# tangjiapeng/DiffuScene

Measured on AMD Instinct MI355X. Metric: denoiser steps/sec (train + 1000-step sample) at B=256, N=80 objects, higher is better.
Workload: dtype f32 (operands split 3xbf16, 6 products, f32 accumulate); 1 GPU; uncond living/dining rooms (config/uncond/diffusion_livingrooms_instancond_lat32_v.yaml scaled to N=80), B=256 scenes per GPU, N=80, C=65, T=1000, mode=both; global_batch=256, parallelism=single

## Files before the change

__graft_entry__.py:

```python
import os
import subprocess
import sys

ROOT = os.path.dirname(os.path.abspath(__file__))
CSRC = os.path.join(ROOT, "diffuscene_amd", "csrc")
LIB = os.path.join(ROOT, "diffuscene_amd", "libdiffuscene_hip.so")

SOURCES = [
    ("gemm_mfma.hip", []),
    ("gemm_split.hip", ["-fno-slp-vectorize"]),
    ("gemm_tn_split.hip", ["-fno-slp-vectorize"]),
    ("blocks.hip", []),
    ("diffusion.hip", ["-ffp-contract=off"]),
    ("train.hip", []),
    ("retrieval.hip", ["-ffp-contract=off"]),
    ("dataset.hip", ["-ffp-contract=off"]),
    ("chamfer.hip", ["-ffp-contract=off"]),
    ("optim.hip", ["-ffp-contract=off"]),
    ("foldingnet.hip", []),
]


def _hipcc():
    for c in (os.environ.get("HIPCC"), "/opt/rocm/bin/hipcc", "hipcc"):
        if c and (os.path.isabs(c) and os.path.exists(c) or not os.path.isabs(c)):
            return c
    raise RuntimeError("hipcc not found")


def _stale(target, deps):
    if not os.path.exists(target):
        return True
    t = os.path.getmtime(target)
    return any(os.path.getmtime(d) > t for d in deps)


def _stamp_git_head():
    try:
        head = subprocess.check_output(["git", "rev-parse", "--short", "HEAD"], cwd=ROOT, stderr=subprocess.DEVNULL, text=True).strip()
        dirty = subprocess.check_output(["git", "status", "--porcelain", "-uno"], cwd=ROOT, stderr=subprocess.DEVNULL, text=True).strip()
        with open(os.path.join(ROOT, "GIT_HEAD"), "w") as f:
            f.write(head + ("+" if dirty else "") + "\n")
    except Exception:
        pass


def build(force=False):
    hipcc = _hipcc()
    headers = [os.path.join(CSRC, "dsc_common.h"), os.path.join(CSRC, "gemm_core.h"), os.path.join(CSRC, "gemm_tn_split.h"),
               os.path.join(ROOT, "include", "diffuscene_hip.h")]
    objs = []
    for src, extra in SOURCES:
        s = os.path.join(CSRC, src)
        if not os.path.exists(s):
            continue
        o = os.path.join(CSRC, src.replace(".hip", ".o"))
        if force or _stale(o, [s] + headers):
            cmd = [hipcc, "--offload-arch=gfx950", "-O3", "-std=c++17", "-fPIC", "-c", s, "-o", o] + extra
            subprocess.check_call(cmd)
        objs.append(o)
    if force or _stale(LIB, objs):
        subprocess.check_call([hipcc, "--offload-arch=gfx950", "-shared", "-fPIC", "-o", LIB] + objs)
    gsrc = os.path.join(ROOT, "tools", "guard_alloc.cpp")
    gso = os.path.join(ROOT, "tools", "_build", "libdsc_guard_alloc.so")
    if os.path.exists(gsrc) and (force or _stale(gso, [gsrc])):
        os.makedirs(os.path.dirname(gso), exist_ok=True)
        try:
            subprocess.check_call([hipcc, "-O2", "-std=c++17", "-fPIC", "-shared", gsrc, "-o", gso])
        except (subprocess.CalledProcessError, OSError) as e:
            print("warning: guard allocator (tools/guard_alloc.cpp) not built: %s -- tests/test_gpu_guard.py will skip its allocator runs" % e,
                  file=sys.stderr)
    _stamp_git_head()
    if ROOT not in sys.path:
        sys.path.insert(0, ROOT)
    import diffuscene_amd
    from diffuscene_amd import _lib
    _lib.load()
    import oracle.ref_torch


def build_asan():
    hipcc = _hipcc()
    out = os.path.join(ROOT, "diffuscene_amd", "libdiffuscene_hip_asan.so")
    objs = []
    for src, extra in SOURCES:
        s = os.path.join(CSRC, src)
        o = os.path.join(CSRC, src.replace(".hip", ".asan.o"))
        subprocess.check_call([hipcc, "--offload-arch=gfx950", "-O1", "-g", "-std=c++17", "-fPIC", "-fsanitize=address", "-fno-gpu-sanitize",
                               "-shared-libsan", "-Wno-option-ignored", "-c", s, "-o", o] + extra)
        objs.append(o)
    subprocess.check_call([hipcc, "--offload-arch=gfx950", "-shared", "-fPIC", "-fsanitize=address", "-fno-gpu-sanitize", "-shared-libsan",
                           "-Wno-option-ignored", "-o", out] + objs)
    return out


def smoke():
    if ROOT not in sys.path:
        sys.path.insert(0, ROOT)
    import torch
    assert torch.cuda.is_available(), "smoke() needs a GPU"
    from diffuscene_amd.networks.denoise_net import Unet1D
    from diffuscene_amd.networks.diffusion_ddpm import DiffusionPoint
    from oracle import ref_torch as R
    from oracle import weights as W

    kw = dict(W.UNCOND_BEDROOM)
    B, N = 4, 12
    dev = torch.device("cuda:0")
    net = Unet1D(**kw)
    sd = W.synth_state_dict(kw)
    net.load_state_dict(sd)
    net.to(dev)
    cfg = dict(objectness_dim=0, class_dim=22, angle_dim=2, objfeat_dim=32)
    diff = DiffusionPoint(net, cfg, time_num=1000, model_mean_type="v")
    x = W.synth_scene_batch(B, N, 22, 32, 0)
    t = torch.tensor([3, 250, 600, 999], dtype=torch.int64)
    cond = W.synth_condition(B, N, 128, 0).contiguous()
    noise = W.synth_noise((B, N, 62), 7)
    with torch.no_grad():
        out = net(x.to(dev), t.to(dev), cond.to(dev), None).cpu()
        ref = R.unet1d_forward(sd, kw, x, t, cond, None)
        rel = float((out - ref).abs().max() / ref.abs().max())
        assert rel < 1e-4, "Unet1D forward mismatch vs oracle: %g" % rel
        tb = R.schedule_tables(1e-4, 0.02, 1000, "v")
        step = diff.diffusion.p_sample(diff._denoise, x.to(dev), t.to(dev), cond.to(dev), None,
                                       noise_fn=lambda size, dtype, device: noise.to(device), clip_denoised=True).cpu()
        ref_step = R.p_sample_step(tb, x, t, ref, noise, True, "v")
        rel2 = float((step - ref_step).abs().max() / ref_step.abs().max())
        assert rel2 < 1e-4, "p_sample mismatch vs oracle: %g" % rel2
    print("smoke ok: forward rel err %.3g, p_sample rel err %.3g" % (rel, rel2))


if __name__ == "__main__":
# ... 7 lines not shown
```

diffuscene_amd/_lib.py:

```python
import ctypes as C
import os

_HERE = os.path.dirname(os.path.abspath(__file__))
LIB_PATH = os.path.join(_HERE, "libdiffuscene_hip.so")
if os.environ.get("DSC_HIP_LIB"):
    LIB_PATH = os.path.abspath(os.environ["DSC_HIP_LIB"])

ACT_NONE, ACT_GELU, ACT_SILU, ACT_LEAKY01 = 0, 1, 2, 3
SS_NONE, SS_PER_TOKEN, SS_PER_SCENE, SS_PER_SLOT, SS_BY_INDEX = 0, 1, 2, 3, 4
MEAN_EPS, MEAN_X0, MEAN_V = 0, 1, 2
TILE_GN_80_W8, TILE_GN_80_W4, TILE_160x256, TILE_160x128_W4 = 1, 2, 5, 8
TILE_WAVE_GN, TILE_WAVE_DENSE, TILE_WAVE_GN_64 = 10, 11, 12
F32_TILE_160x256, F32_TILE_160x128, F32_TILE_128x128, F32_TILE_96x128, F32_TILE_64x64 = 0, 1, 2, 3, 4
DSC_PLANES_NONE = -100
GEMM_ROW_INVARIANT = 1
WS_MAX = 64
MAX_TOKENS_PER_SCENE = 160
STATS_MAX_OBJECTS, STATS_ONE_WAVE_MAX = 160, 32

_ERR = {-1: "DSC_EINVAL (bad shape / null pointer)", -2: "DSC_EALIGN (16-byte alignment required)",
        -3: "DSC_ERANGE (size outside kernel limits)"}

c_f32p = C.c_void_p
c_i64p = C.c_void_p


class GemmArgs(C.Structure):
    _fields_ = [
        ("a1", C.c_void_p), ("lda1", C.c_int64), ("k1", C.c_int32),
        ("a2", C.c_void_p), ("lda2", C.c_int64), ("k2", C.c_int32),
        ("w", C.c_void_p), ("ldw", C.c_int64),
        ("bias", C.c_void_p),
        ("residual", C.c_void_p), ("ldr", C.c_int64),
        ("y", C.c_void_p), ("ldy", C.c_int64),
        ("m", C.c_int32), ("n", C.c_int32),
        ("act_in", C.c_int32), ("act_out", C.c_int32),
        ("batch", C.c_int32),
        ("sa1", C.c_int64), ("sa2", C.c_int64), ("sw", C.c_int64), ("sbias", C.c_int64),
        ("sres", C.c_int64), ("sy", C.c_int64),
        ("gamma", C.c_void_p), ("beta", C.c_void_p), ("eps", C.c_float),
        ("tokens_per_scene", C.c_int32),
        ("scale_shift", C.c_void_p), ("ld_ss", C.c_int64), ("ss_mode", C.c_int32),
        ("preact", C.c_void_p), ("ld_preact", C.c_int64),
        ("ss_index", C.c_void_p),
        ("w_planes", C.c_void_p),
        ("actgrad_x", C.c_void_p), ("ld_actgrad", C.c_int64),
        ("ss_rows", C.c_int32),
        ("w_planes_layout", C.c_int32),
        ("gnb_z", C.c_void_p), ("ld_gnb_z", C.c_int64),
        ("gnb_dgamma", C.c_void_p), ("gnb_dbeta", C.c_void_p), ("gnb_dbias", C.c_void_p), ("gnb_pstride", C.c_int64),
        ("gnb_dss", C.c_void_p), ("ld_gnb_dss", C.c_int64),
        ("flags", C.c_int32),
    ]


class SplitItem(C.Structure):
    _fields_ = [("w", C.c_void_p), ("ldw", C.c_int64), ("rows", C.c_int32), ("cols", C.c_int32), ("planes", C.c_void_p),
                ("transpose", C.c_int32)]


class SmallKItem(C.Structure):
    _fields_ = [("x", C.c_void_p), ("ldx", C.c_int64), ("k_in", C.c_int32), ("w", C.c_void_p), ("ldw", C.c_int64), ("bias", C.c_void_p),
                ("y", C.c_void_p), ("ldy", C.c_int64)]


class ColSpan(C.Structure):
    _fields_ = [("src_col", C.c_int32), ("dst_col", C.c_int32), ("width", C.c_int32)]


SMALLK_MAX = 4


class WsItem(C.Structure):
    _fields_ = [("w", C.c_void_p), ("out", C.c_void_p), ("rows", C.c_int32), ("cols", C.c_int32)]


class TnGroup(C.Structure):
    _fields_ = [("a1", C.c_void_p), ("lda1", C.c_int64), ("k1", C.c_int32),
                ("a2", C.c_void_p), ("lda2", C.c_int64), ("k2", C.c_int32),
                ("dy", C.c_void_p), ("ldd", C.c_int64),
                ("out", C.c_void_p), ("ldo", C.c_int64),
                ("dbias", C.c_void_p),
                ("m", C.c_int32), ("n", C.c_int32), ("kvalid", C.c_int32),
                ("tile0", C.c_int32),
                ("ws_offset", C.c_int64),
                ("tile0s", C.c_int32)]


class ColsumItem(C.Structure):
    _fields_ = [("x", C.c_void_p), ("ldx", C.c_int64), ("m", C.c_int32), ("n", C.c_int32), ("out", C.c_void_p)]


class WsBwdItem(C.Structure):
    _fields_ = [("w", C.c_void_p), ("dw_std", C.c_void_p), ("dw", C.c_void_p), ("rows", C.c_int32), ("cols", C.c_int32)]


SIGNATURES = {
    "dsc_version": (C.c_int, []),
    "dsc_gemm_f32": (C.c_int, [C.POINTER(GemmArgs), C.c_void_p]),
    "dsc_gemm_gn_silu_f32": (C.c_int, [C.POINTER(GemmArgs), C.c_void_p]),
    "dsc_split_bf16x3_f32": (C.c_int, [C.POINTER(SplitItem), C.c_int32, C.c_void_p]),
    "dsc_gemm_arithmetic": (C.c_int, [C.POINTER(GemmArgs), C.c_int32]),
    "dsc_gemm_split_tile": (C.c_int, [C.POINTER(GemmArgs), C.c_int32]),
    "dsc_gemm_f32_tile": (C.c_int, [C.POINTER(GemmArgs)]),
    "dsc_gemm_planes_layout": (C.c_int, [C.POINTER(GemmArgs), C.c_int32]),
    "dsc_get_split_wave": (C.c_int, []),
    "dsc_set_split_wave": (C.c_int, [C.c_int32]),
    "dsc_gemm_skinny": (C.c_int, [C.POINTER(GemmArgs), C.c_int32]),
    "dsc_get_skinny": (C.c_int, []),
    "dsc_set_skinny": (C.c_int, [C.c_int32]),
    "dsc_get_gemm_arithmetic": (C.c_int, []),
    "dsc_set_gemm_arithmetic": (C.c_int, [C.c_int32]),
    "dsc_gemm_layernorm_f32": (C.c_int, [C.POINTER(GemmArgs), C.c_void_p]),
    "dsc_gemm_splitk_f32": (C.c_int, [C.POINTER(GemmArgs), C.c_int32, c_f32p, C.c_int64, C.c_void_p]),
    "dsc_linear_smallk_f32": (C.c_int, [c_f32p, C.c_int64, C.c_int32, c_f32p, C.c_int64, c_f32p, c_f32p, C.c_int64,
                                        C.c_int32, C.c_int32, C.c_int32, C.c_void_p]),
    "dsc_linear_smallk_grouped_f32": (C.c_int, [C.POINTER(SmallKItem), C.c_int32, C.c_int32, C.c_int32, C.c_int32, C.c_void_p]),
    "dsc_gather_columns_f32": (C.c_int, [c_f32p, C.c_int64, c_f32p, C.c_int64, C.c_int32, C.POINTER(ColSpan), C.c_int32, C.c_void_p]),
    "dsc_weight_standardize_f32": (C.c_int, [C.POINTER(WsItem), C.c_int32, C.c_float, C.c_void_p]),
    "dsc_layernorm_f32": (C.c_int, [c_f32p, C.c_int64, c_f32p, c_f32p, C.c_int64, c_f32p, C.c_int64, C.c_int32,
                                    C.c_int32, C.c_float, C.c_void_p]),
    "dsc_linear_attention_f32": (C.c_int, [c_f32p, C.c_int64, c_f32p, C.c_int64, c_f32p, C.c_int64, c_f32p, C.c_int64,
                                           C.c_int32, C.c_int32, C.c_int32, C.c_float, C.c_void_p]),
    "dsc_attention_f32": (C.c_int, [c_f32p, C.c_int64, c_f32p, C.c_int64, c_f32p, C.c_int64, c_f32p, C.c_int64,
                                    C.c_int32, C.c_int32, C.c_float, C.c_void_p]),
    "dsc_time_embedding_f32": (C.c_int, [c_i64p, C.c_int32, C.c_int32, c_f32p, C.c_int32, c_f32p, c_f32p, C.c_void_p]),
    "dsc_activation_f32": (C.c_int, [c_f32p, c_f32p, C.c_int64, C.c_int32, C.c_void_p]),
    "dsc_q_sample_f32": (C.c_int, [c_f32p, c_f32p, c_i64p, c_f32p, c_f32p, c_f32p, c_f32p, C.c_int32, C.c_int64, C.c_int32,
                                   C.c_void_p]),
    "dsc_p_sample_f32": (C.c_int, [c_f32p, c_f32p, c_f32p, c_i64p, c_f32p, c_f32p, c_f32p, c_f32p, c_f32p, c_f32p,
                                   c_f32p, C.c_int32, C.c_int32, C.c_int32, C.c_int64, C.c_int32, C.c_void_p]),
    "dsc_device_error_count": (C.c_int64, [C.c_int32]),
    "dsc_add_scalar_i64": (C.c_int, [c_i64p, C.c_int32, C.c_int64, C.c_void_p]),
    "dsc_ddim_step_f32": (C.c_int, [c_f32p, c_f32p, c_f32p, c_i64p, c_i64p, c_i64p, c_f32p, c_f32p, c_f32p, c_f32p, c_f32p,
                                    c_f32p, c_f32p, c_f32p, c_f32p, C.c_int32, C.c_int32, C.c_int64, C.c_int32, C.c_int32,
                                    C.c_void_p]),
    "dsc_ddim_advance_i64": (C.c_int, [c_i64p, c_i64p, c_i64p, C.c_int32, C.c_int32, C.c_void_p]),
    "dsc_knn16_f32": (C.c_int, [c_f32p, C.c_int64, C.c_int32, c_f32p, c_f32p, C.c_int32, C.c_int32, C.c_void_p, C.c_void_p]),
    "dsc_rowsq_f32": (C.c_int, [c_f32p, C.c_int64, C.c_int32, C.c_int64, c_f32p, C.c_void_p]),
    "dsc_knn_cov_f32": (C.c_int, [c_f32p, C.c_int64, C.c_void_p, C.c_int32, C.c_int32, c_f32p, C.c_int64, C.c_void_p]),
    "dsc_gather_max_f32": (C.c_int, [c_f32p, C.c_int64, C.c_void_p, C.c_int32, C.c_int32, C.c_int32, c_f32p, C.c_int64,
                                     C.c_void_p, C.c_void_p]),
    "dsc_gather_max_bwd_f32": (C.c_int, [c_f32p, C.c_int64, C.c_void_p, C.c_void_p, C.c_int32, C.c_int32, C.c_int32, c_f32p,
                                         C.c_int64, C.c_void_p]),
    "dsc_bn_workspace_floats": (C.c_int64, [C.c_int64, C.c_int32]),
    "dsc_batchnorm_fwd_f32": (C.c_int, [c_f32p, C.c_int64, c_f32p, c_f32p, C.c_int64, C.c_int32, C.c_float, C.c_float,
                                        C.c_int32, c_f32p, c_f32p, c_f32p, c_f32p, c_f32p, c_f32p, c_f32p, C.c_int64,
                                        C.c_void_p]),
    "dsc_batchnorm_eval_f32": (C.c_int, [c_f32p, C.c_int64, c_f32p, c_f32p, c_f32p, c_f32p, C.c_int64, C.c_int32, C.c_int32,
                                         c_f32p, C.c_void_p]),
    "dsc_batchnorm_bwd_f32": (C.c_int, [c_f32p, c_f32p, c_f32p, c_f32p, c_f32p, C.c_int64, C.c_int32, C.c_int32, c_f32p,
                                        c_f32p, c_f32p, c_f32p, C.c_int64, C.c_void_p]),
    "dsc_rowmax_f32": (C.c_int, [c_f32p, C.c_int64, C.c_int32, C.c_int32, C.c_int32, c_f32p, C.c_void_p, C.c_void_p]),
    "dsc_rowmax_bwd_f32": (C.c_int, [c_f32p, C.c_void_p, C.c_int32, C.c_int32, C.c_int32, c_f32p, C.c_void_p]),
    "dsc_point_affine_f32": (C.c_int, [c_f32p, C.c_int64, C.c_int32, c_f32p, C.c_int64, c_f32p, C.c_int32, C.c_int32,
                                       C.c_int32, C.c_int32, c_f32p, C.c_void_p]),
    "dsc_point_affine_bwd_f32": (C.c_int, [c_f32p, c_f32p, C.c_int64, C.c_int32, c_f32p, C.c_int64, C.c_int32, C.c_int32,
                                           C.c_int32, C.c_int32, c_f32p, C.c_int64, c_f32p, C.c_int64, c_f32p, c_f32p,
                                           C.c_int64, C.c_void_p]),
    "dsc_postfilter_compact_f32": (C.c_int, [c_f32p, C.c_int32, C.c_int32, C.c_int32, C.c_int32, C.c_int32, C.c_int32, c_f32p,
                                             C.c_void_p, C.c_void_p]),
    "dsc_gemm_tn_f32": (C.c_int, [c_f32p, C.c_int64, C.c_int32, c_f32p, C.c_int64, C.c_int32, c_f32p, C.c_int64, c_f32p,
                                  C.c_int64, c_f32p, C.c_int32, C.c_int32, C.c_int32, c_f32p, C.c_int64, C.c_void_p]),
    "dsc_gemm_tn_workspace_floats": (C.c_int64, [C.c_int32, C.c_int32, C.c_int32]),
    "dsc_gemm_tn_grouped_f32": (C.c_int, [C.c_void_p, C.c_int32, C.c_int32, C.c_int32, c_f32p, C.c_int64, C.c_int64,
                                          C.c_void_p]),
    "dsc_gemm_tn_grouped_split_f32": (C.c_int, [C.c_void_p, C.c_int32, C.c_int32, C.c_void_p, C.c_int32, C.c_int32, c_f32p, C.c_int64,
                                                C.c_int64, C.c_int32, C.c_void_p]),
    "dsc_set_tn_split_form": (C.c_int, [C.c_int32]),
    "dsc_get_tn_split_form": (C.c_int, []),
    "dsc_colsum_f32": (C.c_int, [c_f32p, C.c_int64, C.c_int32, C.c_int32, c_f32p, c_f32p, C.c_int64, C.c_void_p]),
    "dsc_colsum_grouped_f32": (C.c_int, [C.c_void_p, C.c_int32, C.c_int32, C.c_void_p]),
    "dsc_gn_silu_bwd_f32": (C.c_int, [c_f32p, C.c_int64, c_f32p, C.c_int64, c_f32p, c_f32p, c_f32p, C.c_int64, C.c_int32,
                                      c_f32p, C.c_int64, c_f32p, c_f32p, c_f32p, C.c_int64, c_f32p, C.c_int64, C.c_int32,
                                      C.c_int32, C.c_int32, C.c_float, C.c_void_p]),
    "dsc_weight_standardize_bwd_f32": (C.c_int, [C.POINTER(WsBwdItem), C.c_int32, C.c_float, C.c_void_p]),
    "dsc_layernorm_bwd_f32": (C.c_int, [c_f32p, C.c_int64, c_f32p, c_f32p, C.c_int64, c_f32p, C.c_int64, c_f32p, C.c_int64, c_f32p,
                                        C.c_int32, C.c_int32, C.c_int32, C.c_float, C.c_void_p]),
    "dsc_linear_attention_bwd_f32": (C.c_int, [c_f32p, C.c_int64] * 7 + [C.c_int32, C.c_int32, C.c_int32, C.c_float,
                                                                          C.c_void_p]),
    "dsc_attention_bwd_f32": (C.c_int, [c_f32p, C.c_int64] * 7 + [C.c_int32, C.c_int32, C.c_float, C.c_void_p]),
    "dsc_retrieve_nearest_f32": (C.c_int, [c_f32p, C.c_void_p, C.c_void_p, c_f32p, C.c_void_p, C.c_void_p, C.c_int32,
                                           C.c_int32, C.c_int32, C.c_void_p, c_f32p, C.c_void_p]),
    "dsc_box_bounds_f32": (C.c_int, [c_f32p, c_f32p, c_f32p, C.c_void_p, C.c_int32, C.c_int32, c_f32p, C.c_void_p]),
    "dsc_scene_stats_f32": (C.c_int, [c_f32p, c_f32p, C.c_void_p, C.c_void_p, C.c_int32, C.c_int32, C.c_int32, C.c_int32,
                                      C.c_void_p, C.c_void_p, C.c_void_p, C.c_void_p, C.c_void_p, C.c_void_p, c_f32p, C.c_void_p]),
    "dsc_encode_scene_batch_f32": (C.c_int, [c_i64p, c_f32p, c_f32p, c_f32p, c_f32p, c_f32p, C.c_int32, C.c_int32, c_i64p,
                                             C.c_void_p, C.c_void_p, C.c_void_p, C.c_int32, C.POINTER(C.c_double), c_f32p,
                                             C.c_int64, c_i64p, C.c_int32, C.c_int32, C.c_void_p]),
    "dsc_chamfer3d_forward_f32": (C.c_int, [c_f32p, c_f32p, c_f32p, c_f32p, C.c_void_p, C.c_void_p, C.c_int32, C.c_int32,
                                            C.c_int32, C.c_void_p]),
    "dsc_chamfer3d_backward_f32": (C.c_int, [c_f32p, c_f32p, c_f32p, c_f32p, C.c_void_p, C.c_void_p, c_f32p, c_f32p,
                                             C.c_int32, C.c_int32, C.c_int32, C.c_void_p]),
    "dsc_grad_sumsq_f32": (C.c_int, [C.c_void_p, C.c_int32, C.c_void_p, C.c_void_p]),
    "dsc_clip_coef_f32": (C.c_int, [C.c_void_p, C.c_int32, C.c_float, c_f32p, c_f32p, C.c_void_p]),
    "dsc_adam_step_f32": (C.c_int, [C.c_void_p, C.c_int32, C.c_float, C.c_float, C.c_float, C.c_float, C.c_float, C.c_float,
                                    c_f32p, C.c_void_p]),
    "dsc_ddpm_loss_f32": (C.c_int, [c_f32p, c_f32p, c_f32p, c_i64p, c_f32p, c_f32p, c_f32p, c_f32p, C.POINTER(C.c_float),
                                    c_f32p, c_f32p, c_f32p] + [C.c_int32] * 12 + [C.c_float, C.c_int32, C.c_void_p]),
    "dsc_copy2d_f32": (C.c_int, [c_f32p, C.c_int64, c_f32p, C.c_int64, C.c_int32, C.c_int32, C.c_void_p]),
    "dsc_add2d_f32": (C.c_int, [c_f32p, C.c_int64, c_f32p, C.c_int64, C.c_int32, C.c_int32, C.c_void_p]),
    "dsc_activation_bwd_f32": (C.c_int, [c_f32p, c_f32p, c_f32p, C.c_int64, C.c_int32, C.c_void_p]),
    "dsc_transpose_batched_f32": (C.c_int, [C.POINTER(WsItem), C.c_int32, C.c_void_p]),
    "dsc_transpose_f32": (C.c_int, [c_f32p, C.c_int64, c_f32p, C.c_int64, C.c_int32, C.c_int32, C.c_void_p]),
    "dsc_complete_overwrite_f32": (C.c_int, [c_f32p, c_f32p, c_f32p, c_i64p, c_f32p, c_f32p, C.c_int32, C.c_int32,
                                             C.c_int32, C.c_int32, C.c_int32, C.c_void_p]),
    "dsc_complete_overwrite_ragged_f32": (C.c_int, [c_f32p, c_f32p, c_f32p, c_i64p, c_i64p, c_f32p, c_f32p, C.c_int32, C.c_int32,
                                                    C.c_int32, C.c_int32, C.c_int32, C.c_void_p]),
    "dsc_p_sample_inpaint_f32": (C.c_int, [c_f32p, c_f32p, c_f32p, c_f32p, c_f32p, c_i64p, c_i64p, c_f32p, c_f32p, c_f32p, c_f32p,
                                           c_f32p, c_f32p, c_f32p, c_f32p] + [C.c_int32] * 7 + [C.c_void_p]),
    "dsc_ddim_inpaint_step_f32": (C.c_int, [c_f32p] * 5 + [c_i64p] * 4 + [c_f32p] * 10 + [C.c_int32] * 7 + [C.c_void_p]),
    "dsc_masked_overwrite_f32": (C.c_int, [c_f32p, c_f32p, c_f32p, C.c_void_p, c_i64p, c_f32p, c_f32p, C.c_int32, C.c_int64, C.c_int32,
                                           C.c_void_p]),
    "dsc_p_sample_masked_f32": (C.c_int, [c_f32p] * 5 + [C.c_void_p, c_i64p] + [c_f32p] * 8 + [C.c_int32] * 3 + [C.c_int64, C.c_int32,
                                                                                                                  C.c_void_p]),
    "dsc_ddim_masked_step_f32": (C.c_int, [c_f32p] * 5 + [C.c_void_p] + [c_i64p] * 3 + [c_f32p] * 10 + [C.c_int32] * 2 +
                                 [C.c_int64, C.c_int32, C.c_int32, C.c_void_p]),
    "dsc_cfg_combine_f32": (C.c_int, [c_f32p, c_f32p, c_f32p, C.c_int32, C.c_int64, C.c_void_p]),
    "dsc_scene_randn_f32": (C.c_int, [c_f32p, c_i64p, c_i64p, C.c_int64, C.c_int64, C.c_int64, C.c_void_p]),
    "dsc_scene_philox_u32": (C.c_int, [C.c_void_p, c_i64p, c_i64p, C.c_int64, C.c_int64, C.c_int64, C.c_void_p]),
    "dsc_p_sample_cfg_f32": (C.c_int, [c_f32p] * 4 + [c_i64p] + [c_f32p] * 8 + [C.c_int32] * 3 + [C.c_int64, C.c_int32, C.c_void_p]),
    "dsc_ddim_cfg_step_f32": (C.c_int, [c_f32p] * 4 + [c_i64p] * 3 + [c_f32p] * 10 + [C.c_int32] * 2 +
                              [C.c_int64, C.c_int32, C.c_int32, C.c_void_p]),
    "dsc_p_sample_masked_cfg_f32": (C.c_int, [c_f32p] * 6 + [C.c_void_p, c_i64p] + [c_f32p] * 9 + [C.c_int32] * 3 +
                                    [C.c_int64, C.c_int32, C.c_void_p]),
    "dsc_ddim_masked_cfg_step_f32": (C.c_int, [c_f32p] * 6 + [C.c_void_p] + [c_i64p] * 3 + [c_f32p] * 11 + [C.c_int32] * 2 +
                                     [C.c_int64, C.c_int32, C.c_int32, C.c_void_p]),
    "dsc_scene_gate_f32": (C.c_int, [c_f32p, C.c_void_p, c_f32p, C.c_int32, C.c_int64, C.c_void_p]),
}

_lib = None


class HipLibraryMissing(RuntimeError):
    pass


def load():
    global _lib
    if _lib is not None:
        return _lib
    if not os.path.exists(LIB_PATH):
        raise HipLibraryMissing(
            "%s not found: build it with `python __graft_entry__.py` (hipcc --offload-arch=gfx950). "
            "diffuscene_amd has no CPU or PyTorch fallback." % LIB_PATH)
    import torch
    lib = C.CDLL(LIB_PATH)
    for name, (res, args) in SIGNATURES.items():
        try:
            fn = getattr(lib, name)
        except AttributeError as e:
            raise HipLibraryMissing("symbol %s missing from %s" % (name, LIB_PATH)) from e
        fn.restype = res
        fn.argtypes = args
    if lib.dsc_get_gemm_arithmetic() < 0:
        raise ValueError("DSC_GEMM=%r: must be 'split' (default) or 'f32'" % os.environ.get("DSC_GEMM"))
    if lib.dsc_get_tn_split_form() < 0:
        raise ValueError("DSC_TN_FORM=%r: must be '2' (default), '1' or '0'" % os.environ.get("DSC_TN_FORM"))
    if lib.dsc_get_split_wave() < 0:
        raise ValueError("DSC_WAVE=%r: must be '1' / 'auto' (default) or '0'" % os.environ.get("DSC_WAVE"))
    _lib = lib
    return lib


def split_enabled():
    return load().dsc_get_gemm_arithmetic() == 1


def gemm_mode():
    lib = load()
    if lib.dsc_get_gemm_arithmetic() != 1:
        return 0
    return (2 if lib.dsc_get_split_wave() == 1 else 1) + 10 * lib.dsc_get_tn_split_form()


def set_split_wave(on):
    prev = load().dsc_get_split_wave() == 1
    check(load().dsc_set_split_wave(1 if on else 0), "dsc_set_split_wave")
    return prev


def set_gemm_arithmetic(name):
    if name not in ("split", "f32"):
        raise ValueError("gemm arithmetic must be 'split' or 'f32', got %r" % (name,))
    prev = "split" if split_enabled() else "f32"
    check(load().dsc_set_gemm_arithmetic(1 if name == "split" else 0), "dsc_set_gemm_arithmetic")
    return prev


def device_error_count(reset=False):
    n = load().dsc_device_error_count(1 if reset else 0)
    if n < 0:
        raise RuntimeError("dsc_device_error_count failed (HIP error)")
    return int(n)


def check_indices(where):
    if os.environ.get("DSC_CHECK_INDICES", "0") == "1":
        n = device_error_count(reset=True)
        if n:
            raise IndexError("%s: %d out-of-range device timestep(s) were clamped into the schedule tables" % (where, n))


def check(rc, what):
    if rc != 0:
        raise RuntimeError("%s failed: %s" % (what, _ERR.get(rc, "hipError_t %d" % rc)))


def fn(name):
    return getattr(load(), name)
```

diffuscene_amd/csrc/blocks.hip:

```cpp
#include "dsc_common.h"

namespace {

struct WsBatch { dsc_ws_item it[DSC_WS_MAX]; };

__device__ __forceinline__ float block_sum_256(float v, float* red) {
    v = wave_sum(v);
    const int lane = threadIdx.x & 63, wave = threadIdx.x >> 6;
    __syncthreads();
    if (lane == 0) red[wave] = v;
    __syncthreads();
    return red[0] + red[1] + red[2] + red[3];
}

__global__ __launch_bounds__(256) void ws_kernel(const WsBatch b, const float eps) {
    __shared__ float red[4];
    const dsc_ws_item it = b.it[blockIdx.y];
    const int row = blockIdx.x;
    if (row >= it.rows) return;
    const float* w = it.w + (int64_t)row * it.cols;
    float* o = it.out + (int64_t)row * it.cols;
    constexpr int MAXE = 8;
    float v[MAXE];
    float s = 0.f;
#pragma unroll
    for (int i = 0; i < MAXE; ++i) {
        const int c = threadIdx.x + 256 * i;
        v[i] = (c < it.cols) ? w[c] : 0.f;
        s += v[i];
    }
    const float mean = block_sum_256(s, red) / (float)it.cols;
    float s2 = 0.f;
#pragma unroll
    for (int i = 0; i < MAXE; ++i) {
        const int c = threadIdx.x + 256 * i;
        const float d = (c < it.cols) ? v[i] - mean : 0.f;
        s2 += d * d;
    }
    const float var = block_sum_256(s2, red) / (float)it.cols;
    const float rs = 1.0f / sqrtf(var + eps);
#pragma unroll
    for (int i = 0; i < MAXE; ++i) {
        const int c = threadIdx.x + 256 * i;
        if (c < it.cols) o[c] = (v[i] - mean) * rs;
    }
}

__global__ __launch_bounds__(256) void layernorm512_kernel(const float* __restrict__ x, int64_t ldx,
                                                          const float* __restrict__ g,
                                                          const float* __restrict__ res, int64_t ldr,
                                                          float* __restrict__ y, int64_t ldy, int m, float eps) {
    const int lane = threadIdx.x & 63;
    const int row = blockIdx.x * 4 + (threadIdx.x >> 6);
    if (row >= m) return;
    const float* xr = x + (int64_t)row * ldx;
    const f32x4 a = *reinterpret_cast<const f32x4*>(xr + lane * 4);
    const f32x4 b = *reinterpret_cast<const f32x4*>(xr + 256 + lane * 4);
    float s = (a[0] + a[1]) + (a[2] + a[3]) + (b[0] + b[1]) + (b[2] + b[3]);
    const float mean = wave_sum(s) * (1.0f / 512.0f);
    float s2 = 0.f;
#pragma unroll
    for (int e = 0; e < 4; ++e) {
        const float da = a[e] - mean, db = b[e] - mean;
        s2 += da * da + db * db;
    }
    const float var = wave_sum(s2) * (1.0f / 512.0f);
    const float rs = 1.0f / sqrtf(var + eps);
    const f32x4 ga = *reinterpret_cast<const f32x4*>(g + lane * 4);
    const f32x4 gb = *reinterpret_cast<const f32x4*>(g + 256 + lane * 4);
    f32x4 oa, ob;
#pragma unroll
    for (int e = 0; e < 4; ++e) {
        oa[e] = (a[e] - mean) * rs * ga[e];
        ob[e] = (b[e] - mean) * rs * gb[e];
    }
    if (res) {
        const float* rr = res + (int64_t)row * ldr;
        const f32x4 ra = *reinterpret_cast<const f32x4*>(rr + lane * 4);
        const f32x4 rb = *reinterpret_cast<const f32x4*>(rr + 256 + lane * 4);
#pragma unroll
        for (int e = 0; e < 4; ++e) { oa[e] += ra[e]; ob[e] += rb[e]; }
    }
    float* yr = y + (int64_t)row * ldy;
    *reinterpret_cast<f32x4*>(yr + lane * 4) = oa;
    *reinterpret_cast<f32x4*>(yr + 256 + lane * 4) = ob;
}

constexpr int MAXTOK = 160;
constexpr int HP = 33;
constexpr int LP = 36;

__global__ __launch_bounds__(256) void linear_attention_kernel(const float* __restrict__ q, int64_t ldq,
                                                               const float* __restrict__ k, int64_t ldk,
                                                               const float* __restrict__ v, int64_t ldv,
                                                               float* __restrict__ out, int64_t ldo,
                                                               int nq, int nk, float scale) {
    extern __shared__ __attribute__((aligned(16))) float lds[];
    float* Ks = lds;
    float* Vs = Ks + nk * LP;
    float* Qs = Vs + nk * LP;
    float* ctx = Qs + nq * LP;
    const int b = blockIdx.x >> 2, h = blockIdx.x & 3;
    const int tid = threadIdx.x;
    const float* kb = k + (int64_t)b * nk * ldk + h * 32;
    const float* vb = v + (int64_t)b * nk * ldv + h * 32;
    const float* qb = q + (int64_t)b * nq * ldq + h * 32;
    for (int f = tid; f < nk * 8; f += 256) {
        const int j = f >> 3, c4 = (f & 7) * 4;
        *reinterpret_cast<f32x4*>(Ks + j * LP + c4) = *reinterpret_cast<const f32x4*>(kb + (int64_t)j * ldk + c4);
        *reinterpret_cast<f32x4*>(Vs + j * LP + c4) = *reinterpret_cast<const f32x4*>(vb + (int64_t)j * ldv + c4);
    }
    for (int f = tid; f < nq * 8; f += 256) {
        const int i = f >> 3, c4 = (f & 7) * 4;
        *reinterpret_cast<f32x4*>(Qs + i * LP + c4) = *reinterpret_cast<const f32x4*>(qb + (int64_t)i * ldq + c4);
    }
    __syncthreads();
    {
        const int d = tid >> 3, part = tid & 7;
        float mx = -INFINITY;
        for (int j = part; j < nk; j += 8) mx = fmaxf(mx, Ks[j * LP + d]);
        mx = fmaxf(mx, __shfl_xor(mx, 1, 64));
        mx = fmaxf(mx, __shfl_xor(mx, 2, 64));
        mx = fmaxf(mx, __shfl_xor(mx, 4, 64));
        float sm = 0.f;
        for (int j = part; j < nk; j += 8) {
            const float e = expf(Ks[j * LP + d] - mx);
            Ks[j * LP + d] = e;
            sm += e;
        }
        sm += __shfl_xor(sm, 1, 64);
        sm += __shfl_xor(sm, 2, 64);
        sm += __shfl_xor(sm, 4, 64);
        const float inv = 1.0f / sm;
        for (int j = part; j < nk; j += 8) Ks[j * LP + d] *= inv;
    }
    __syncthreads();
    {
        const int d = tid >> 3, e0 = (tid & 7) * 4;
        f32x4 a = {0.f, 0.f, 0.f, 0.f};
        for (int j = 0; j < nk; ++j) {
            const float kd = Ks[j * LP + d];
            const f32x4 vv = *reinterpret_cast<const f32x4*>(Vs + j * LP + e0);
#pragma unroll
            for (int e = 0; e < 4; ++e) a[e] += kd * vv[e];
        }
        *reinterpret_cast<f32x4*>(ctx + d * LP + e0) = a;
    }
    __syncthreads();
    for (int i0 = 0; i0 < nq; i0 += 64) {
        const int i = i0 + (tid >> 2), part = tid & 3;
        const bool ok = i < nq;
        float qv[8];
        float mx = -INFINITY;
        if (ok) {
            const f32x4 a = *reinterpret_cast<const f32x4*>(Qs + i * LP + part * 8);
            const f32x4 c = *reinterpret_cast<const f32x4*>(Qs + i * LP + part * 8 + 4);
#pragma unroll
            for (int e = 0; e < 4; ++e) { qv[e] = a[e]; qv[4 + e] = c[e]; }
#pragma unroll
            for (int e = 0; e < 8; ++e) mx = fmaxf(mx, qv[e]);
        }
        mx = fmaxf(mx, __shfl_xor(mx, 1, 64));
        mx = fmaxf(mx, __shfl_xor(mx, 2, 64));
        float sm = 0.f;
        if (ok) {
#pragma unroll
            for (int e = 0; e < 8; ++e) { qv[e] = expf(qv[e] - mx); sm += qv[e]; }
        }
        sm += __shfl_xor(sm, 1, 64);
        sm += __shfl_xor(sm, 2, 64);
        if (ok) {
            const float inv = scale / sm;
            f32x4 a, c;
#pragma unroll
            for (int e = 0; e < 4; ++e) { a[e] = qv[e] * inv; c[e] = qv[4 + e] * inv; }
            *reinterpret_cast<f32x4*>(Qs + i * LP + part * 8) = a;
            *reinterpret_cast<f32x4*>(Qs + i * LP + part * 8 + 4) = c;
        }
        __builtin_amdgcn_wave_barrier();
        if (ok) {
            f32x4 o0 = {0.f, 0.f, 0.f, 0.f}, o1 = {0.f, 0.f, 0.f, 0.f};
#pragma unroll 8
            for (int d = 0; d < 32; ++d) {
                const float qd = Qs[i * LP + d];
                const f32x4 c0 = *reinterpret_cast<const f32x4*>(ctx + d * LP + part * 8);
                const f32x4 c1 = *reinterpret_cast<const f32x4*>(ctx + d * LP + part * 8 + 4);
#pragma unroll
                for (int e = 0; e < 4; ++e) { o0[e] += c0[e] * qd; o1[e] += c1[e] * qd; }
            }
            float* orow = out + ((int64_t)b * nq + i) * ldo + h * 32 + part * 8;
            *reinterpret_cast<f32x4*>(orow) = o0;
            *reinterpret_cast<f32x4*>(orow + 4) = o1;
        }
    }
}

__global__ __launch_bounds__(512) void attention_kernel(const float* __restrict__ q, int64_t ldq,
                                                        const float* __restrict__ k, int64_t ldk,
                                                        const float* __restrict__ v, int64_t ldv,
                                                        float* __restrict__ out, int64_t ldo, int n, float scale) {
    extern __shared__ __attribute__((aligned(16))) float att_lds[];
    float* Ks = att_lds;
    float* Vs = Ks + n * LP;
    const int b = blockIdx.x >> 2, h = blockIdx.x & 3;
    const int tid = threadIdx.x;
    const float* kb = k + (int64_t)b * n * ldk + h * 32;
    const float* vb = v + (int64_t)b * n * ldv + h * 32;
    const int nthr = blockDim.x, rows = nthr >> 2;
    for (int f = tid; f < n * 8; f += nthr) {
        const int j = f >> 3, c4 = (f & 7) * 4;
        *reinterpret_cast<f32x4*>(Ks + j * LP + c4) = *reinterpret_cast<const f32x4*>(kb + (int64_t)j * ldk + c4);
        *reinterpret_cast<f32x4*>(Vs + j * LP + c4) = *reinterpret_cast<const f32x4*>(vb + (int64_t)j * ldv + c4);
    }
    __syncthreads();
    const int part = tid & 3;
    for (int i0 = 0; i0 < n; i0 += rows) {
        const int i = i0 + (tid >> 2);
        const bool ok = i < n;
        const float* qr = q + ((int64_t)b * n + (ok ? i : 0)) * ldq + h * 32 + part * 8;
        const f32x4 qa = *reinterpret_cast<const f32x4*>(qr), qc = *reinterpret_cast<const f32x4*>(qr + 4);
        float qv[8];
#pragma unroll
        for (int e = 0; e < 4; ++e) { qv[e] = qa[e] * scale; qv[4 + e] = qc[e] * scale; }
        auto score = [&](int j) {
            const f32x4 ka = *reinterpret_cast<const f32x4*>(Ks + j * LP + part * 8);
            const f32x4 kc = *reinterpret_cast<const f32x4*>(Ks + j * LP + part * 8 + 4);
            float s = 0.f;
#pragma unroll
            for (int e = 0; e < 4; ++e) s += qv[e] * ka[e];
#pragma unroll
            for (int e = 0; e < 4; ++e) s += qv[4 + e] * kc[e];
            s += __shfl_xor(s, 1, 64);
            s += __shfl_xor(s, 2, 64);
            return s;
        };
        float mx = -INFINITY;
        for (int j = 0; j < n; ++j) mx = fmaxf(mx, score(j));
        float o[8] = {0.f, 0.f, 0.f, 0.f, 0.f, 0.f, 0.f, 0.f};
        float sm = 0.f;
        for (int j = 0; j < n; ++j) {
            const float pj = expf(score(j) - mx);
            sm += pj;
            const f32x4 va = *reinterpret_cast<const f32x4*>(Vs + j * LP + part * 8);
            const f32x4 vc = *reinterpret_cast<const f32x4*>(Vs + j * LP + part * 8 + 4);
#pragma unroll
            for (int e = 0; e < 4; ++e) { o[e] += pj * va[e]; o[4 + e] += pj * vc[e]; }
        }
        if (ok) {
            const float inv = 1.0f / sm;
            float* orow = out + ((int64_t)b * n + i) * ldo + h * 32 + part * 8;
            f32x4 t0, t1;
#pragma unroll
            for (int e = 0; e < 4; ++e) { t0[e] = o[e] * inv; t1[e] = o[4 + e] * inv; }
            *reinterpret_cast<f32x4*>(orow) = t0;
            *reinterpret_cast<f32x4*>(orow + 4) = t1;
        }
    }
}

constexpr int SK_TOK = 32;
constexpr int SK_MAXK = 64;

__device__ __forceinline__ void linear_smallk_block(const float* __restrict__ x, int64_t ldx, int kin,
                                                    const float* __restrict__ w, int64_t ldw,
                                                    const float* __restrict__ bias,
                                                    float* __restrict__ y, int64_t ldy, int m, int n, int act, float* xs) {
    const int tok0 = blockIdx.x * SK_TOK;
    const int ntok = (m - tok0) < SK_TOK ? (m - tok0) : SK_TOK;
    for (int f = threadIdx.x; f < SK_TOK * kin; f += 256) {
        const int t = f / kin, kk = f - t * kin;
        xs[kk * SK_TOK + t] = (t < ntok) ? x[(int64_t)(tok0 + t) * ldx + kk] : 0.f;
    }
    __syncthreads();
    for (int c = threadIdx.x; c < n; c += 256) {
        float acc[SK_TOK];
        const float b = bias ? bias[c] : 0.f;
// ... 219 lines not shown
```

diffuscene_amd/csrc/gemm_split.hip:

```cpp
#include "dsc_common.h"
#include "gemm_split_wave.h"
#include <atomic>
#include <cstring>

#ifndef DSC_SPLIT_DSPREAD
#define DSC_SPLIT_DSPREAD true
#endif

namespace dsc_split {

typedef unsigned u32x4 __attribute__((ext_vector_type(4)));
typedef __bf16 bf16x8 __attribute__((ext_vector_type(8)));
typedef __bf16 bf16x2 __attribute__((ext_vector_type(2)));

constexpr int BK = 32;

__device__ __forceinline__ unsigned cvt_pk_bf16(float a, float b) {
    f32x2 v = {a, b};
    return __builtin_bit_cast(unsigned, __builtin_convertvector(v, bf16x2));
}
__device__ __forceinline__ float bf_lo(unsigned p) { return __builtin_bit_cast(float, p << 16); }
__device__ __forceinline__ float bf_hi(unsigned p) { return __builtin_bit_cast(float, p & 0xffff0000u); }

__device__ __forceinline__ void split8(const f32x4 lo, const f32x4 hi, bf16x8& p1, bf16x8& p2, bf16x8& p3) {
// ... 316 lines not shown
            }
        }
        if (p.preact) {
            float* const pb = p.preact + (int64_t)(row0 + srow + l15) * p.ld_preact + cbase;
#pragma unroll
            for (int i = 0; i < RB; ++i)
                if (valid[i]) {
#pragma unroll
                    for (int j = 0; j < 4; ++j) *reinterpret_cast<f32x4*>(pb + (int64_t)i * 16 * p.ld_preact + j * 16) = acc[i][j];
                }
        }
        const float inv_cnt = 1.f / (float)(ntok * 64);
        float s0 = 0.f;
#pragma unroll
        for (int i = 0; i < RB; ++i)
#pragma unroll
            for (int j = 0; j < 4; ++j)
                s0 += valid[i] ? (acc[i][j][0] + acc[i][j][1]) + (acc[i][j][2] + acc[i][j][3]) : 0.f;
        const float mean = wave_sum_dpp(s0) * inv_cnt;
        float q0 = 0.f;
#pragma unroll
        for (int i = 0; i < RB; ++i)
#pragma unroll
            for (int j = 0; j < 4; ++j)
#pragma unroll
                for (int e = 0; e < 4; ++e) {
                    const float d = valid[i] ? acc[i][j][e] - mean : 0.f;
                    q0 = fmaf(d, d, q0);
                }
        const float rstd = 1.f / sqrtf(wave_sum_dpp(q0) * inv_cnt + p.eps);
#pragma unroll
        for (int j = 0; j < 4; ++j)
#pragma unroll
            for (int e = 0; e < 4; ++e) {
                const float a = rstd * ga[j][e], sp1 = sc[j][e] + 1.f;
                ga[j][e] = a * sp1;
                be[j][e] = fmaf(be[j][e] - mean * a, sp1, sh[j][e]);
            }
#pragma unroll
        for (int i = 0; i < RB; ++i) {
            if (valid[i]) {
#pragma unroll
                for (int j = 0; j < 4; ++j) {
                    f32x4 y, s1 = {1.f, 1.f, 1.f, 1.f}, s2 = {0.f, 0.f, 0.f, 0.f};
                    if (per_row) {
                        const int64_t row = p.ss_mode == DSC_SS_PER_TOKEN ? (int64_t)row0 + srow + i * 16 + l15 : (int64_t)i * 16 + l15;
                        const float* ssr = p.scale_shift + row * p.ld_ss + cbase + j * 16;
                        s1 = *reinterpret_cast<const f32x4*>(ssr) + 1.f;
                        s2 = *reinterpret_cast<const f32x4*>(ssr + p.n);
                    }
#pragma unroll
                    for (int e = 0; e < 4; ++e) {
                        float t = fmaf(acc[i][j][e], ga[j][e], be[j][e]);
                        if (per_row) t = fmaf(t, s1[e], s2[e]);
                        y[e] = dsc_silu_fast(t);
                    }
                    if (rbp) y += *reinterpret_cast<const f32x4*>(rbp + (int64_t)i * 16 * p.ldr + j * 16);
                    *reinterpret_cast<f32x4*>(ob + (int64_t)i * 16 * p.ldy + j * 16) = y;
                }
            }
        }
    }
}

template <bool GN, int WM, int WN, int RB, bool DSPREAD = DSC_SPLIT_DSPREAD>
__global__ __launch_bounds__(64 * WM * WN, 1) void gemm_split_kernel(const dsc_gemm_args p, const int ntok) {
    __shared__ __attribute__((aligned(16))) char smem[split_smem_bytes<WM, WN, RB>()];
    gemm_split_tile<GN, WM, WN, RB, DSPREAD>(p, ntok, blockIdx.x, blockIdx.y, smem);
}

template <bool GN, int WM, int WN, int RB>
int launch(const dsc_gemm_args* a, int ntok, hipStream_t s) {
    constexpr int BN = 64 * WN;
    const int scenes = (a->m + ntok - 1) / ntok;
    const unsigned grid = (unsigned)(((scenes + WM - 1) / WM) * (a->n / BN));
    DSC_CLEAR_STALE_ERROR();
    hipLaunchKernelGGL((gemm_split_kernel<GN, WM, WN, RB>), dim3(grid, (unsigned)a->batch), dim3(64 * WM * WN), 0, s, *a, ntok);
    DSC_LAUNCH_CHECK();
    return 0;
}

}

enum { T_GN_32 = 0, T_GN_80_W8, T_GN_80_W4, T_GN_48, T_GN_64, T_160x256, T_256x128, T_128x128, T_160x128_W4, T_64x256, T_WAVE_GN, T_WAVE_DENSE, T_WAVE_GN_64 };

static std::atomic<int> g_gemm_arith{-1000};

extern "C" int dsc_get_gemm_arithmetic(void) {
    int m = g_gemm_arith.load(std::memory_order_relaxed);
    if (m == -1000) {
        const char* e = getenv("DSC_GEMM");
        m = (!e || !e[0] || !strcmp(e, "split")) ? 1 : !strcmp(e, "f32") ? 0 : DSC_EINVAL;
        g_gemm_arith.store(m, std::memory_order_relaxed);
    }
    return m;
}

extern "C" int dsc_set_gemm_arithmetic(int32_t mode) {
    if (mode != 0 && mode != 1) return DSC_EINVAL;
    g_gemm_arith.store(mode, std::memory_order_relaxed);
    return 0;
}

static std::atomic<int> g_split_wave{-1000};

extern "C" int dsc_get_split_wave(void) {
    int m = g_split_wave.load(std::memory_order_relaxed);
    if (m == -1000) {
        const char* e = getenv("DSC_WAVE");
        m = (!e || !e[0] || !strcmp(e, "1") || !strcmp(e, "auto")) ? 1 : !strcmp(e, "0") ? 0 : DSC_EINVAL;
        g_split_wave.store(m, std::memory_order_relaxed);
    }
    return m;
}

extern "C" int dsc_set_split_wave(int32_t mode) {
    if (mode != 0 && mode != 1) return DSC_EINVAL;
    g_split_wave.store(mode, std::memory_order_relaxed);
    return 0;
}

static int select_wave(const dsc_gemm_args* a, bool gn) {
    if (dsc_get_split_wave() != 1) return -1;
    const int K = a->k1 + a->k2;
    if ((a->n % 128) || (a->k1 % 64) || (a->k2 % 64) || K < 256) return -1;
    if (a->batch != 1 && (gn || a->sw != (int64_t)a->n * K || a->ldw != K || (a->sy & 3) || (a->sres & 3) || (a->sbias & 3))) return -1;
    if (!dsc_aligned16(a->y) || (a->ldy & 3) || a->ldy < a->n) return -1;
    if (a->bias && !dsc_aligned16(a->bias)) return -1;
    if (a->residual && (!dsc_aligned16(a->residual) || (a->ldr & 3) || a->ldr < a->n)) return -1;
    if (a->preact && (!dsc_aligned16(a->preact) || (a->ld_preact & 3) || a->ld_preact < a->n || a->batch != 1)) return -1;
    if (a->actgrad_x && (gn || !dsc_aligned16(a->actgrad_x) || (a->ld_actgrad & 3) || a->ld_actgrad < a->n || a->batch != 1)) return -1;
    if (3LL * a->batch * a->n * K * 2 >= 0x7fffffffLL) return -1;
    const int64_t ld_max = a->lda1 > a->lda2 ? a->lda1 : a->lda2;
    if (ld_max * 4 * 96 >= 0x7fffffffLL) return -1;
    long waves;
    if (a->gnb_z) {
        const int N = a->tokens_per_scene;
        if (gn || a->batch != 1 || N <= 64 || N > 80 || (a->m % N) || a->bias || a->residual || a->preact || a->actgrad_x || a->act_out != DSC_ACT_NONE) return -1;
        if (!a->gamma || !a->beta || !a->gnb_dgamma || !a->gnb_dbeta || !a->gnb_dbias || (a->ss_mode != DSC_SS_NONE && a->ss_mode != DSC_SS_PER_SCENE)) return -1;
        if (!dsc_aligned16(a->gnb_z) || (a->ld_gnb_z & 3) || a->ld_gnb_z < a->n || !dsc_aligned16(a->gamma) || !dsc_aligned16(a->beta)) return -1;
        if (!dsc_aligned16(a->gnb_dgamma) || !dsc_aligned16(a->gnb_dbeta) || !dsc_aligned16(a->gnb_dbias) || (a->gnb_pstride & 3)) return -1;
        if (a->ss_mode == DSC_SS_PER_SCENE && (!a->scale_shift || !dsc_aligned16(a->scale_shift) || (a->ld_ss & 3))) return -1;
        if (a->gnb_dss && (!dsc_aligned16(a->gnb_dss) || (a->ld_gnb_dss & 3))) return -1;
        waves = (long)(a->m / N) * (a->n / 128);
        const long r = (waves + 1023) / 1024;
        return waves * 5 >= r * 1024 * 4 ? T_WAVE_DENSE : -1;
    }
    if (gn) {
        const int N = a->tokens_per_scene;
        if (N <= 16 || N > 80) return -1;
        const bool perrow = a->ss_mode == DSC_SS_PER_TOKEN || a->ss_mode == DSC_SS_PER_SLOT;
        if (perrow && a->ld_ss < 2 * (int64_t)a->n) return -1;
        waves = (long)(a->m / N) * (a->n / 128);
    } else {
        waves = (long)((a->m + 79) / 80) * (a->n / 128) * a->batch;
    }
    const long rounds = (waves + 1023) / 1024;
    if (waves * 5 >= rounds * 1024 * 4) return gn ? T_WAVE_GN : T_WAVE_DENSE;
    if (gn && a->tokens_per_scene > 64) {
        const long w4 = 2 * waves, r4 = (w4 + 1023) / 1024;
        if (r4 == 1 && w4 * 5 >= 1024 * 4) return T_WAVE_GN_64;
    }
    return -1;
}

static int select_block_tile(const dsc_gemm_args* a, bool gn);

static int select_tile(const dsc_gemm_args* a, bool gn, bool assume_planes = false) {
    if (dsc_get_gemm_arithmetic() != 1 || (!assume_planes && !a->w_planes)) return -1;
    if (a->flags & DSC_GEMM_ROW_INVARIANT) return -1;
    const int w = select_wave(a, gn);
    return w >= 0 ? w : select_block_tile(a, gn);
}

static int select_block_tile(const dsc_gemm_args* a, bool gn) {
    if (a->gnb_z) return -1;
    const int K = a->k1 + a->k2;
    if (a->batch != 1 && (gn || a->sw != (int64_t)a->n * K || a->ldw != K || (a->sy & 3) || (a->sres & 3) || (a->sbias & 3))) return -1;
    if ((a->n % 128) || (K % 32)) return -1;
    if (!dsc_aligned16(a->w_planes) || !dsc_aligned16(a->y) || (a->ldy & 3)) return -1;
    if (a->bias && !dsc_aligned16(a->bias)) return -1;
    if (a->residual && (!dsc_aligned16(a->residual) || (a->ldr & 3))) return -1;
    if (!gn && a->preact && (!dsc_aligned16(a->preact) || (a->ld_preact & 3) || a->batch != 1)) return -1;
    if (a->actgrad_x && (gn || !dsc_aligned16(a->actgrad_x) || (a->ld_actgrad & 3) || a->batch != 1)) return -1;
    if (3LL * a->batch * a->n * K * 2 >= 0x7fffffffLL) return -1;
    const int64_t ld_max = a->lda1 > a->lda2 ? a->lda1 : a->lda2;
    if (ld_max * 4 * 320 >= 0x7fffffffLL) return -1;
    const bool wide = (a->n % 256) == 0;
    constexpr long MIN_BLOCKS = 160;
    if (gn) {
        const int N = a->tokens_per_scene;
        if (N <= 16 || N > 80) return -1;
        const long S = a->m / N;
        if (N <= 32) return ((S + 3) / 4) * (a->n / 128) >= MIN_BLOCKS ? T_GN_32 : -1;
        const long b8 = wide ? ((S + 1) / 2) * (a->n / 256) : 0, b4 = ((S + 1) / 2) * (a->n / 128);
        if (N > 64) return b8 >= MIN_BLOCKS + 32 ? T_GN_80_W8 : b4 >= MIN_BLOCKS ? T_GN_80_W4 : -1;
        if (b8 < MIN_BLOCKS) return -1;
        return N <= 48 ? T_GN_48 : T_GN_64;
    }
    struct Cand { int bm, bn, id; };
    const Cand cands[5] = {{160, 256, T_160x256}, {256, 128, T_256x128}, {160, 128, T_160x128_W4}, {128, 128, T_128x128}, {64, 256, T_64x256}};
    int best = -1;
    long best_cost = 0, best_blk = 0;
    for (int i = 0; i < 5; ++i) {
        if (cands[i].bn == 256 && !wide) continue;
        const long nblk = (long)((a->m + cands[i].bm - 1) / cands[i].bm) * (a->n / cands[i].bn) * a->batch;
        const long c = ((nblk + 255) / 256) * (long)cands[i].bm * cands[i].bn;
        if (best < 0 || c < best_cost) { best = cands[i].id; best_cost = c; best_blk = nblk; }
    }
    return best_blk >= MIN_BLOCKS ? best : -1;
}

int dsc_gemm_try_split(const dsc_gemm_args* a, bool gn, hipStream_t s) {
    using namespace dsc_split;
    if (dsc_get_gemm_arithmetic() < 0 || dsc_get_split_wave() < 0) return DSC_EINVAL;
    const int N = a->tokens_per_scene;
    const int tile = select_tile(a, gn);
    if (tile < 0) return DSC_SPLIT_NOT_TAKEN;
    const int want = (tile == T_WAVE_GN || tile == T_WAVE_DENSE || tile == T_WAVE_GN_64) ? DSC_PLANES_FRAGMENT : DSC_PLANES_ROWMAJOR;
    if (a->w_planes_layout != want) return DSC_EINVAL;
    switch (tile) {
        case T_GN_32: return launch<true, 4, 2, 2>(a, N, s);
        case T_GN_80_W8: return launch<true, 2, 4, 5>(a, N, s);
        case T_GN_80_W4: return launch<true, 2, 2, 5>(a, N, s);
        case T_GN_48: return launch<true, 2, 4, 3>(a, N, s);
        case T_GN_64: return launch<true, 2, 4, 4>(a, N, s);
        case T_160x256: return launch<false, 2, 4, 5>(a, 80, s);
        case T_256x128: return launch<false, 4, 2, 4>(a, 64, s);
        case T_128x128: return launch<false, 4, 2, 2>(a, 32, s);
        case T_160x128_W4: return launch<false, 2, 2, 5>(a, 80, s);
        case T_64x256: return launch<false, 2, 4, 2>(a, 32, s);
        case T_WAVE_DENSE:
            if (a->gnb_z) return dsc_wave::launch<false, 5, false, 8, true>(a, a->w_planes, N, s);
            return dsc_wave::launch<false, 5>(a, a->w_planes, 80, s);
        case T_WAVE_GN_64:
            return (a->ss_mode == DSC_SS_PER_TOKEN || a->ss_mode == DSC_SS_PER_SLOT) ? dsc_wave::launch<true, 5, true, 4>(a, a->w_planes, N, s)
                                                                                     : dsc_wave::launch<true, 5, false, 4>(a, a->w_planes, N, s);
        case T_WAVE_GN: {
            const bool perrow = a->ss_mode == DSC_SS_PER_TOKEN || a->ss_mode == DSC_SS_PER_SLOT;
            const int rb = (N + 15) / 16;
            if (perrow) {
                return rb == 5 ? dsc_wave::launch<true, 5, true>(a, a->w_planes, N, s) : rb == 4 ? dsc_wave::launch<true, 4, true>(a, a->w_planes, N, s)
                     : rb == 3 ? dsc_wave::launch<true, 3, true>(a, a->w_planes, N, s) : dsc_wave::launch<true, 2, true>(a, a->w_planes, N, s);
            }
            return rb == 5 ? dsc_wave::launch<true, 5>(a, a->w_planes, N, s) : rb == 4 ? dsc_wave::launch<true, 4>(a, a->w_planes, N, s)
                 : rb == 3 ? dsc_wave::launch<true, 3>(a, a->w_planes, N, s) : dsc_wave::launch<true, 2>(a, a->w_planes, N, s);
        }
        default: return DSC_SPLIT_NOT_TAKEN;
    }
}

extern "C" int dsc_gemm_arithmetic(const dsc_gemm_args* a, int32_t gn) {
    if (!a || a->m <= 0 || a->n <= 0 || a->k1 <= 0) return DSC_EINVAL;
    return select_tile(a, gn != 0) >= 0 ? 1 : 0;
}

extern "C" int dsc_gemm_split_tile(const dsc_gemm_args* a, int32_t gn) {
    if (!a || a->m <= 0 || a->n <= 0 || a->k1 <= 0) return DSC_EINVAL;
    return select_tile(a, gn != 0);
}

extern "C" int dsc_gemm_planes_layout(const dsc_gemm_args* a, int32_t gn) {
    if (!a || a->m <= 0 || a->n <= 0 || a->k1 <= 0) return DSC_EINVAL;
    const int tile = select_tile(a, gn != 0, true);
    return tile < 0 ? DSC_PLANES_NONE : (tile == T_WAVE_GN || tile == T_WAVE_DENSE || tile == T_WAVE_GN_64) ? DSC_PLANES_FRAGMENT : DSC_PLANES_ROWMAJOR;
}

extern "C" int dsc_split_bf16x3_f32(const dsc_split_item* items, int32_t count, dsc_stream_t stream) {
    using namespace dsc_split;
    if (!items || count < 1 || count > DSC_WS_MAX) return DSC_EINVAL;
    SplitBatch b;
    long max_items = 0;
    for (int i = 0; i < count; ++i) {
        const dsc_split_item& it = items[i];
        if (!it.w || !it.planes || it.rows <= 0 || it.cols <= 0) return DSC_EINVAL;
        if (it.transpose & ~(DSC_SPLIT_TRANSPOSE | DSC_SPLIT_FRAGMENT)) return DSC_EINVAL;
        const bool tr = (it.transpose & DSC_SPLIT_TRANSPOSE) != 0;
        const int co = tr ? it.rows : it.cols, ro = tr ? it.cols : it.rows;
        if (co % 8) return DSC_EINVAL;
        if ((it.transpose & DSC_SPLIT_FRAGMENT) && ((ro % 16) || (co % 32))) return DSC_EINVAL;
        if (!dsc_aligned16(it.planes) || (!tr && (!dsc_aligned16(it.w) || (it.ldw & 3)))) return DSC_EALIGN;
        b.it[i] = it;
        const long n = (long)it.rows * it.cols / 8;
        if (n > max_items) max_items = n;
    }
    long bx = (max_items + 255) / 256;
    if (bx > 1024) bx = 1024;
    DSC_CLEAR_STALE_ERROR();
    hipLaunchKernelGGL(split_planes_kernel, dim3((unsigned)bx, (unsigned)count), dim3(256), 0, static_cast<hipStream_t>(stream), b);
    DSC_LAUNCH_CHECK();
    return 0;
}
```

diffuscene_amd/csrc/gemm_split_wave.h:

```cpp
#pragma once
#include "dsc_common.h"
#include <utility>

#ifndef DSC_WAVE_STAMP_ARGS
#define DSC_WAVE_STAMP_ARGS
#define DSC_WAVE_STAMP_PASS
#define DSC_WAVE_STAMP_DECL
#define DSC_WAVE_STAMP_KERNEL(id)
#define DSC_WAVE_STAMP_TILE(id)
#define DSC_WAVE_STAMP_FLUSH(kt)
#define DSC_WAVE_STAMP_END
#endif

namespace dsc_wave {

typedef unsigned u32x4 __attribute__((ext_vector_type(4)));
typedef __bf16 bf16x8 __attribute__((ext_vector_type(8)));
typedef __bf16 bf16x2 __attribute__((ext_vector_type(2)));

constexpr int BK = 32;
constexpr int WAVES = 4;

__device__ __forceinline__ unsigned cvt_pk_bf16(float a, float b) {
    f32x2 v = {a, b};
    return __builtin_bit_cast(unsigned, __builtin_convertvector(v, bf16x2));
}
__device__ __forceinline__ float bf_lo(unsigned p) { return __builtin_bit_cast(float, p << 16); }
__device__ __forceinline__ float bf_hi(unsigned p) { return __builtin_bit_cast(float, p & 0xffff0000u); }

__device__ __forceinline__ void split8(const f32x4 lo, const f32x4 hi, bf16x8& p1, bf16x8& p2, bf16x8& p3) {
    u32x4 a, b, c;
#pragma unroll
    for (int q = 0; q < 4; ++q) {
        const float x0 = q < 2 ? lo[2 * q] : hi[2 * q - 4], x1 = q < 2 ? lo[2 * q + 1] : hi[2 * q - 3];
        const unsigned u1 = cvt_pk_bf16(x0, x1);
        const float r0 = x0 - bf_lo(u1), r1 = x1 - bf_hi(u1);
        const unsigned u2 = cvt_pk_bf16(r0, r1);
        const float s0 = r0 - bf_lo(u2), s1 = r1 - bf_hi(u2);
        a[q] = u1;
        b[q] = u2;
        c[q] = cvt_pk_bf16(s0, s1);
    }
    p1 = __builtin_bit_cast(bf16x8, a);
    p2 = __builtin_bit_cast(bf16x8, b);
    p3 = __builtin_bit_cast(bf16x8, c);
}

template <int RB>
constexpr int wave_smem_bytes() { return WAVES * 2 * 3 * (16 * RB) * 64; }

template <bool GN, int RB, bool PERROW = false, int J = 8, bool GB = false>
__global__ __launch_bounds__(64 * WAVES, 1) void gemm_split_wave_kernel(const dsc_gemm_args p, const uint16_t* const planes_f, const int ntok DSC_WAVE_STAMP_ARGS) {
    static_assert(J == 8 || J == 4, "wave tile: 128 or 64 channels");
    static_assert(!GB || (!GN && J == 8), "the GroupNorm-backward epilogue rides on the dense 80 x 128 form");
    constexpr int NWF = 3 * J;
    constexpr int CW = 16 * J;
    constexpr int ROWS = 16 * RB, XP = ROWS * 64, STAGE = 3 * XP;
    constexpr int NWB = RB > 4 ? RB - 2 : RB > 3 ? RB - 1 : RB;
    constexpr int PERW = (NWF + NWB - 1) / NWB;
    __shared__ __attribute__((aligned(16))) char smem[wave_smem_bytes<RB>()];
    const int lane = threadIdx.x & 63;
    const int wave = __builtin_amdgcn_readfirstlane(threadIdx.x >> 6);
    const int K = p.k1 + p.k2, KT = K / BK;
    const int scenes = (p.m + ntok - 1) / ntok;
    const int sgs = (scenes + WAVES - 1) / WAVES, chunks = p.n / CW;
    const int bid = blockIdx.x;
    int sg, ch;
    if ((sgs & 7) == 0) {
        const int xcd = bid & 7, idx = bid >> 3;
        sg = xcd * (sgs >> 3) + idx / chunks;
        ch = idx % chunks;
    } else {
        sg = bid / chunks;
        ch = bid % chunks;
    }
    const int scene = sg * WAVES + wave;
    if (scene >= scenes) return;
    DSC_WAVE_STAMP_DECL
    DSC_WAVE_STAMP_KERNEL(0)
    const int z = blockIdx.y;
    const int row0 = scene * ntok, col0 = ch * CW;
    const int rows_here = min(ntok, p.m - row0);
    const float* const xb1 = p.a1 + (int64_t)z * p.sa1 + (int64_t)row0 * p.lda1;
    const float* const xb2 = p.a2 ? p.a2 + (int64_t)z * p.sa2 + (int64_t)row0 * p.lda2 : xb1;
    const float* const bias = p.bias ? p.bias + (int64_t)z * p.sbias : nullptr;
    const int64_t rec1 = ((int64_t)(p.m - row0 - 1) * p.lda1 + p.k1) * 4;
    const int64_t rec2 = p.a2 ? ((int64_t)(p.m - row0 - 1) * p.lda2 + p.k2) * 4 : rec1;
    const int64_t recw = (int64_t)3 * p.batch * p.n * K * 2;
    const int64_t rec1c = rec1 < 0x7fffffffLL ? rec1 : 0x7fffffffLL, rec2c = rec2 < 0x7fffffffLL ? rec2 : 0x7fffffffLL;
#if defined(__HIP_DEVICE_COMPILE__)
    const __amdgpu_buffer_rsrc_t r1 = __builtin_amdgcn_make_buffer_rsrc(const_cast<float*>(xb1), 0, (int)rec1c, 0x00020000);
    const __amdgpu_buffer_rsrc_t r2 = __builtin_amdgcn_make_buffer_rsrc(const_cast<float*>(xb2), 0, (int)rec2c, 0x00020000);
#endif
#if defined(__HIP_DEVICE_COMPILE__)
    const __amdgpu_buffer_rsrc_t rw = __builtin_amdgcn_make_buffer_rsrc(const_cast<uint16_t*>(planes_f), 0, (int)recw, 0x00020000);
#endif
    const int plane_bytes = p.batch * p.n * K * 2;
    const int nb0 = (z * p.n + col0) / 16;

    const int q4 = lane & 3, r16 = lane >> 2, g = lane >> 4, l15 = lane & 15;
    const int tvo1 = (r16 * (int)p.lda1 + q4 * 8) * 4, tvo2 = (r16 * (int)p.lda2 + q4 * 8) * 4;
    const int ildso = r16 * 64 + ((q4 ^ ((r16 >> 1) & 3)) << 4);
    const int xoff = l15 * 64 + ((g ^ ((l15 >> 1) & 3)) << 4);
    const int wvo = lane * 16;
    char* const wl = smem + wave * (2 * STAGE);

    f32x4 acc[RB][J];
#pragma unroll
    for (int j = 0; j < J; ++j) {
        f32x4 b4 = {0.f, 0.f, 0.f, 0.f};
        if (bias) b4 = *reinterpret_cast<const f32x4*>(bias + col0 + j * 16 + 4 * g);
#pragma unroll
        for (int i = 0; i < RB; ++i) acc[i][j] = b4;
    }

    f32x4 ld[RB][2];
    bf16x8 wf[2][J][3], xf[2][3];
    const int lda2e = p.a2 ? (int)p.lda2 : (int)p.lda1, kshift = p.a2 ? p.k1 : 0;
    const int tvo2e = p.a2 ? tvo2 : tvo1;
    auto load_tok = [&](int kt, int u, auto segc) {
#if defined(__HIP_DEVICE_COMPILE__)
        constexpr int SEG = decltype(segc)::value;
        const int k0 = kt * BK;
        if constexpr (SEG == 0) {
            const int so = (u * 16 * (int)p.lda1 + k0) * 4;
            ld[u][0] = __builtin_bit_cast(f32x4, __builtin_amdgcn_raw_buffer_load_b128(r1, tvo1, so, 0));
            ld[u][1] = __builtin_bit_cast(f32x4, __builtin_amdgcn_raw_buffer_load_b128(r1, tvo1 + 16, so, 0));
        } else {
            const int so = (u * 16 * lda2e + k0 - kshift) * 4;
            ld[u][0] = __builtin_bit_cast(f32x4, __builtin_amdgcn_raw_buffer_load_b128(r2, tvo2e, so, 0));
            ld[u][1] = __builtin_bit_cast(f32x4, __builtin_amdgcn_raw_buffer_load_b128(r2, tvo2e + 16, so, 0));
        }
#else
        (void)kt; (void)u;
#endif
    };
    auto load_w = [&](int kt, int j, int pl) -> bf16x8 {
#if defined(__HIP_DEVICE_COMPILE__)
        return __builtin_bit_cast(bf16x8, __builtin_amdgcn_raw_buffer_load_b128(rw, wvo, pl * plane_bytes + ((nb0 + j) * KT + kt) * 1024, 0));
#else
        (void)kt; (void)j; (void)pl;
        return bf16x8{};
#endif
    };
    constexpr int NMMA = 6 * J;

    auto tile = [&](const int kt, auto curc, auto segc) {
        constexpr int CUR = decltype(curc)::value, NXT = CUR ^ 1;
        char* const cur = wl + CUR * STAGE;
        char* const nxt = wl + NXT * STAGE;
        const int kn1 = min(kt + 1, KT - 1), kn2 = min(kt + 2, KT - 1);
        constexpr int X0 = CUR ? (RB & 1) : 0;
        DSC_WAVE_STAMP_TILE(0)
        auto block = [&](auto ic) {
            constexpr int i = decltype(ic)::value;
            constexpr int NR = 3;
            constexpr int W0 = i * PERW < NWF ? i * PERW : NWF, W1 = (i + 1) * PERW < NWF ? (i + 1) * PERW : NWF;
            constexpr int VPS = J == 8 ? 2 : 4, NVS = 44 / VPS;
            constexpr int S0 = NR + (W1 - W0), S1 = S0 + NVS, S2 = S1 + 3, S3 = S2 + 1;
            static_assert(S3 <= NMMA, "one MFMA per filler slot");
            unsigned su1[4], su2[4], su3[4];
            float sr0[4], sr1[4], st0[4], st1[4];
            auto xin = [&](int q, int h) -> float { return q < 2 ? ld[i][0][2 * q + h] : ld[i][1][2 * q - 4 + h]; };
            auto split_op = [&](auto nc) {
                constexpr int n = decltype(nc)::value;
                constexpr int q = 2 * (n / 22) + (n & 1), o = (n % 22) >> 1;
                if constexpr (o == 0) su1[q] = cvt_pk_bf16(xin(q, 0), xin(q, 1));
                if constexpr (o == 1) st0[q] = bf_lo(su1[q]);
                if constexpr (o == 2) st1[q] = bf_hi(su1[q]);
                if constexpr (o == 3) sr0[q] = xin(q, 0) - st0[q];
                if constexpr (o == 4) sr1[q] = xin(q, 1) - st1[q];
                if constexpr (o == 5) su2[q] = cvt_pk_bf16(sr0[q], sr1[q]);
                if constexpr (o == 6) st0[q] = bf_lo(su2[q]);
                if constexpr (o == 7) st1[q] = bf_hi(su2[q]);
                if constexpr (o == 8) sr0[q] = sr0[q] - st0[q];
                if constexpr (o == 9) sr1[q] = sr1[q] - st1[q];
                if constexpr (o == 10) su3[q] = cvt_pk_bf16(sr0[q], sr1[q]);
            };
            char* const d0 = nxt + i * 1024 + ildso;
            auto filler = [&](auto kc) {
                constexpr int k = decltype(kc)::value;
                if constexpr (k < NR) {
                    if constexpr (i + 1 < RB) xf[(X0 + i + 1) & 1][k] = *reinterpret_cast<const bf16x8*>(cur + k * XP + (i + 1) * 1024 + xoff);
                    else xf[(X0 + i + 1) & 1][k] = *reinterpret_cast<const bf16x8*>(nxt + k * XP + xoff);
                } else if constexpr (k < S0) {
                    constexpr int w = W0 + (k - NR);
                    wf[NXT][w / 3][w % 3] = load_w(kn1, w / 3, w % 3);
                } else if constexpr (k < S1) {
                    dsc_static_for<VPS>([&](auto vc) { split_op(std::integral_constant<int, VPS * (k - S0) + decltype(vc)::value>{}); });
                } else if constexpr (k < S2) {
                    constexpr int pl = k - S1;
                    const u32x4 v = pl == 0 ? u32x4{su1[0], su1[1], su1[2], su1[3]} : pl == 1 ? u32x4{su2[0], su2[1], su2[2], su2[3]}
                                                                                              : u32x4{su3[0], su3[1], su3[2], su3[3]};
                    *reinterpret_cast<u32x4*>(d0 + pl * XP) = v;
                } else if constexpr (k == S2) {
                    load_tok(kn2, i, segc);
                }
            };
            auto product = [&](auto pc) {
                constexpr int pr = decltype(pc)::value;
                constexpr int wp = pr == 0 ? 2 : (pr == 1 || pr >= 4) ? 0 : 1;
                constexpr int xp = pr == 0 ? 0 : pr == 1 ? 2 : pr == 2 ? 1 : pr == 3 ? 0 : pr == 4 ? 1 : 0;
                dsc_static_for<J>([&](auto jc) {
                    constexpr int j = decltype(jc)::value;
                    acc[i][j] = __builtin_amdgcn_mfma_f32_16x16x32_bf16(wf[CUR][j][wp], xf[(X0 + i) & 1][xp], acc[i][j], 0, 0, 0);
                    filler(std::integral_constant<int, pr * J + j>{});
                    __builtin_amdgcn_sched_barrier(0);
                });
            };
            dsc_static_for<6>(product);
            DSC_WAVE_STAMP_TILE(1 + i)
        };
        dsc_static_for<RB>(block);
        DSC_WAVE_STAMP_FLUSH(kt)
    };

    using std::integral_constant;
#pragma unroll
    for (int u = 0; u < RB; ++u) load_tok(0, u, integral_constant<int, 0>{});
#pragma unroll
    for (int w = 0; w < NWF; ++w) wf[0][w / 3][w % 3] = load_w(0, w / 3, w % 3);
#pragma unroll
    for (int u = 0; u < RB; ++u) {
        bf16x8 a, b, c;
        split8(ld[u][0], ld[u][1], a, b, c);
        char* d0 = wl + u * 1024 + ildso;
        *reinterpret_cast<bf16x8*>(d0) = a;
        *reinterpret_cast<bf16x8*>(d0 + XP) = b;
        *reinterpret_cast<bf16x8*>(d0 + 2 * XP) = c;
        load_tok(1, u, integral_constant<int, 0>{});
    }
#pragma unroll
    for (int pl = 0; pl < 3; ++pl) xf[0][pl] = *reinterpret_cast<const bf16x8*>(wl + pl * XP + xoff);
    const int KT1 = p.k1 / BK;
    int kt = 0;
    DSC_WAVE_STAMP_KERNEL(1)
    for (; kt + 2 < KT1; kt += 2) {
        tile(kt, integral_constant<int, 0>{}, integral_constant<int, 0>{});
        tile(kt + 1, integral_constant<int, 1>{}, integral_constant<int, 0>{});
    }
    f32x4 ep_ga[2], ep_be[2], ep_sc[2], ep_sh[2];
    if constexpr (GN) {
        const bool per_scene_e = p.ss_mode == DSC_SS_PER_SCENE || p.ss_mode == DSC_SS_BY_INDEX;
        int64_t ssrow_e = scene;
        if (p.ss_mode == DSC_SS_BY_INDEX) ssrow_e = dsc_clamp_index(p.ss_index[scene], p.ss_rows);
#pragma unroll
        for (int c2 = 0; c2 < J / 4; ++c2) {
            const int ch = col0 + 64 * c2 + 4 * (lane & 15);
            ep_ga[c2] = *reinterpret_cast<const f32x4*>(p.gamma + ch);
            ep_be[c2] = *reinterpret_cast<const f32x4*>(p.beta + ch);
            ep_sc[c2] = f32x4{0.f, 0.f, 0.f, 0.f};
            ep_sh[c2] = ep_sc[c2];
            if (per_scene_e) {
                const float* ssr = p.scale_shift + ssrow_e * p.ld_ss + ch;
                ep_sc[c2] = *reinterpret_cast<const f32x4*>(ssr);
                ep_sh[c2] = *reinterpret_cast<const f32x4*>(ssr + p.n);
            }
        }
    }
    for (; kt < KT; kt += 2) {
        tile(kt, integral_constant<int, 0>{}, integral_constant<int, 1>{});
        tile(kt + 1, integral_constant<int, 1>{}, integral_constant<int, 1>{});
    }

    DSC_WAVE_STAMP_KERNEL(2)
    constexpr int ERS = 64 * 4 + 16;
    static_assert(ROWS * ERS <= 2 * STAGE, "the transposed cell fits the wave's LDS image");
    const int er = lane >> 4, ec = lane & 15;
#if defined(__HIP_DEVICE_COMPILE__)
    auto row_rsrc = [&](const float* base, int64_t ld, int rows, int cols) {
        return __builtin_amdgcn_make_buffer_rsrc(const_cast<float*>(base), 0, rows > 0 ? (int)(((int64_t)(rows - 1) * ld + cols) * 4) : 0, 0x00020000);
    };
    const __amdgpu_buffer_rsrc_t ry = row_rsrc(p.y + (int64_t)z * p.sy + (int64_t)row0 * p.ldy, p.ldy, rows_here, p.n);
    const __amdgpu_buffer_rsrc_t rr = row_rsrc(p.residual ? p.residual + (int64_t)z * p.sres + (int64_t)row0 * p.ldr : p.y, p.ldr, p.residual ? rows_here : 0, p.n);
    const __amdgpu_buffer_rsrc_t rpa = row_rsrc(p.preact ? p.preact + (int64_t)z * p.sy + (int64_t)row0 * p.ld_preact : p.y, p.ld_preact, p.preact ? rows_here : 0, p.n);
    auto ld4 = [&](const __amdgpu_buffer_rsrc_t& r, int voff, int soff) { return __builtin_bit_cast(f32x4, __builtin_amdgcn_raw_buffer_load_b128(r, voff, soff, 0)); };
    auto st4 = [&](const f32x4 v, const __amdgpu_buffer_rsrc_t& r, int voff, int soff) { __builtin_amdgcn_raw_buffer_store_b128(__builtin_bit_cast(u32x4, v), r, voff, soff, 0); };
#else
    const int ry = 0, rr = 0, rpa = 0;
    auto ld4 = [&](int, int, int) { return f32x4{}; };
    auto st4 = [&](const f32x4, int, int, int) {};
#endif
    const bool has_res = p.residual != nullptr, has_pre = p.preact != nullptr;
    auto to_lds = [&](const int c2) {
#pragma unroll
        for (int i = 0; i < RB; ++i)
#pragma unroll
            for (int j = 0; j < 4; ++j) *reinterpret_cast<f32x4*>(wl + (i * 16 + l15) * ERS + (j * 16 + 4 * g) * 4) = acc[i][4 * c2 + j];
    };
    constexpr int NQ = ROWS / 4, QH = NQ % 10 == 0 ? 10 : NQ % 8 == 0 ? 8 : NQ % 6 == 0 ? 6 : 4;
    static_assert(NQ % QH == 0, "row groups per pass");
    if constexpr (GB) {
        const float inv_cnt = 1.f / (float)(ntok * 64);
        const bool per_scene = p.ss_mode == DSC_SS_PER_SCENE && p.scale_shift;
#if defined(__HIP_DEVICE_COMPILE__)
        const __amdgpu_buffer_rsrc_t rz = row_rsrc(p.gnb_z + (int64_t)row0 * p.ld_gnb_z, p.ld_gnb_z, rows_here, p.n);
#else
        const int rz = 0;
#endif
        dsc_static_for<2>([&](auto c2c) {
            constexpr int c2 = decltype(c2c)::value;
            const int ch = col0 + 64 * c2 + 4 * ec, cc = ch * 4;
            const int vy = er * (int)p.ldy * 4 + cc, vz = er * (int)p.ld_gnb_z * 4 + cc;
            f32x4 zv[NQ], dv[NQ];
#pragma unroll
            for (int q = 0; q < NQ; ++q) zv[q] = ld4(rz, vz, 4 * q * (int)p.ld_gnb_z * 4);
            const f32x4 ga = *reinterpret_cast<const f32x4*>(p.gamma + ch), be = *reinterpret_cast<const f32x4*>(p.beta + ch);
            f32x4 s1 = {1.f, 1.f, 1.f, 1.f}, sh = {0.f, 0.f, 0.f, 0.f};
            if (per_scene) {
                const float* ssr = p.scale_shift + (int64_t)scene * p.ld_ss + ch;
                s1 = *reinterpret_cast<const f32x4*>(ssr) + 1.f;
                sh = *reinterpret_cast<const f32x4*>(ssr + p.n);
            }
            to_lds(c2);
            float s = 0.f;
#pragma unroll
            for (int q = 0; q < NQ; ++q) {
                dv[q] = *reinterpret_cast<const f32x4*>(wl + (4 * q + er) * ERS + ec * 16);
                const bool ok = 4 * q + er < rows_here;
                if (!ok) dv[q] = f32x4{0.f, 0.f, 0.f, 0.f};
                s += ok ? (zv[q][0] + zv[q][1]) + (zv[q][2] + zv[q][3]) : 0.f;
            }
            const float mu = wave_sum_dpp(s) * inv_cnt;
            s = 0.f;
#pragma unroll
            for (int q = 0; q < NQ; ++q) {
                const bool ok = 4 * q + er < rows_here;
#pragma unroll
                for (int e = 0; e < 4; ++e) { const float d = ok ? zv[q][e] - mu : 0.f; s = fmaf(d, d, s); }
            }
            const float rs = 1.0f / sqrtf(wave_sum_dpp(s) * inv_cnt + p.eps);
            float S1 = 0.f, S2 = 0.f;
            f32x4 Gg = {0.f, 0.f, 0.f, 0.f}, Gb = Gg, Gsc = Gg, Gsh = Gg, Gz = Gg;
#pragma unroll
            for (int q = 0; q < NQ; ++q) {
#pragma unroll
                for (int e = 0; e < 4; ++e) {
                    const float xh = (zv[q][e] - mu) * rs;
                    const float gh = ga[e] * xh + be[e];
                    const float u = gh * s1[e] + sh[e];
                    const float sig = __builtin_amdgcn_rcpf(1.0f + __expf(-u));
                    const float du = dv[q][e] * (sig * (1.0f + u * (1.0f - sig)));
                    const float dgh = du * s1[e];
                    const float dxh = dgh * ga[e];
                    S1 += dxh; S2 += dxh * xh;
                    Gg[e] += dgh * xh; Gb[e] += dgh; Gsc[e] += du * gh; Gsh[e] += du;
                    zv[q][e] = xh;
                    dv[q][e] = dxh;
                }
            }
            const float m1 = wave_sum_dpp(S1) * inv_cnt, m2 = wave_sum_dpp(S2) * inv_cnt;
#pragma unroll
            for (int q = 0; q < NQ; ++q) {
                const bool ok = 4 * q + er < rows_here;
                f32x4 dzv;
#pragma unroll
                for (int e = 0; e < 4; ++e) { dzv[e] = rs * (dv[q][e] - m1 - zv[q][e] * m2); Gz[e] += ok ? dzv[e] : 0.f; }
                st4(dzv, ry, vy, 4 * q * (int)p.ldy * 4);
            }
            auto fold = [&](f32x4 v) {
#pragma unroll
                for (int e = 0; e < 4; ++e) { v[e] += __shfl_xor(v[e], 16, 64); v[e] += __shfl_xor(v[e], 32, 64); }
                return v;
            };
            Gg = fold(Gg); Gb = fold(Gb); Gz = fold(Gz);
            if (per_scene && p.gnb_dss) { Gsc = fold(Gsc); Gsh = fold(Gsh); }
            if (lane < 16) {
                const int64_t o = (int64_t)scene * p.gnb_pstride + ch;
                *reinterpret_cast<f32x4*>(p.gnb_dgamma + o) = Gg;
                *reinterpret_cast<f32x4*>(p.gnb_dbeta + o) = Gb;
                *reinterpret_cast<f32x4*>(p.gnb_dbias + o) = Gz;
                if (per_scene && p.gnb_dss) {
                    *reinterpret_cast<f32x4*>(p.gnb_dss + (int64_t)scene * p.ld_gnb_dss + ch) = Gsc;
                    *reinterpret_cast<f32x4*>(p.gnb_dss + (int64_t)scene * p.ld_gnb_dss + p.n + ch) = Gsh;
                }
// ... 55 lines not shown
    } else {
#if defined(__HIP_DEVICE_COMPILE__)
        const __amdgpu_buffer_rsrc_t rs = row_rsrc(PERROW ? p.scale_shift + (p.ss_mode == DSC_SS_PER_TOKEN ? (int64_t)row0 * p.ld_ss : 0) : p.y, p.ld_ss,
                                                   PERROW ? rows_here : 0, 2 * p.n);
#else
        const int rs = 0;
#endif
        const float inv_cnt = 1.f / (float)(ntok * 64);
        const bool vlast = (RB - 1) * 16 + l15 < rows_here;
#pragma unroll
        for (int c2 = 0; c2 < J / 4; ++c2) {
            const int ch = col0 + 64 * c2 + 4 * ec;
            const f32x4 ga = ep_ga[c2], be = ep_be[c2], sc = ep_sc[c2], sh = ep_sh[c2];
            to_lds(c2);
            float s0 = 0.f;
#pragma unroll
            for (int i = 0; i < RB; ++i)
#pragma unroll
                for (int j = 0; j < 4; ++j) {
                    const f32x4 a = acc[i][4 * c2 + j];
                    const float t = (a[0] + a[1]) + (a[2] + a[3]);
                    s0 += (i < RB - 1 || vlast) ? t : 0.f;
                }
            const float mean = wave_sum_dpp(s0) * inv_cnt;
            float q0 = 0.f;
#pragma unroll
            for (int i = 0; i < RB; ++i)
#pragma unroll
                for (int j = 0; j < 4; ++j)
#pragma unroll
                    for (int e = 0; e < 4; ++e) {
                        const float d = (i < RB - 1 || vlast) ? acc[i][4 * c2 + j][e] - mean : 0.f;
                        q0 = fmaf(d, d, q0);
                    }
            const float rstd = 1.f / sqrtf(wave_sum_dpp(q0) * inv_cnt + p.eps);
            if (c2 == 0) { DSC_WAVE_STAMP_KERNEL(3) }
            f32x4 A, B;
#pragma unroll
            for (int e = 0; e < 4; ++e) {
                const float a = rstd * ga[e], sp1 = sc[e] + 1.f;
                A[e] = a * sp1;
                B[e] = fmaf(be[e] - mean * a, sp1, sh[e]);
            }
            const int cc = ch * 4;
            const int vy = er * (int)p.ldy * 4 + cc, vr = er * (int)p.ldr * 4 + cc, vp = er * (int)p.ld_preact * 4 + cc, vs = er * (int)p.ld_ss * 4 + cc;
            if (c2 == 0) { DSC_WAVE_STAMP_KERNEL(4) }
#pragma unroll
            for (int h = 0; h < NQ; h += QH) {
                f32x4 rres[QH], s1[QH], s2[QH];
                if (has_res) {
#pragma unroll
                    for (int qq = 0; qq < QH; ++qq) rres[qq] = ld4(rr, vr, 4 * (h + qq) * (int)p.ldr * 4);
                }
                if constexpr (PERROW) {
#pragma unroll
                    for (int qq = 0; qq < QH; ++qq) {
                        s1[qq] = ld4(rs, vs, 4 * (h + qq) * (int)p.ld_ss * 4);
                        s2[qq] = ld4(rs, vs + p.n * 4, 4 * (h + qq) * (int)p.ld_ss * 4);
                    }
                }
#pragma unroll
                for (int qq = 0; qq < QH; ++qq) {
                    const f32x4 zv = *reinterpret_cast<const f32x4*>(wl + (4 * (h + qq) + er) * ERS + ec * 16);
                    if (has_pre) st4(zv, rpa, vp, 4 * (h + qq) * (int)p.ld_preact * 4);
                    f32x4 y;
#pragma unroll
                    for (int e = 0; e < 4; ++e) {
                        float t = fmaf(zv[e], A[e], B[e]);
                        if constexpr (PERROW) t = fmaf(t, s1[qq][e] + 1.f, s2[qq][e]);
                        y[e] = dsc_silu_fast(t);
                    }
                    if (has_res) y += rres[qq];
                    st4(y, ry, vy, 4 * (h + qq) * (int)p.ldy * 4);
                }
            }
            if (c2 == 0) { DSC_WAVE_STAMP_KERNEL(5) }
        }
    }
    DSC_WAVE_STAMP_END
}

template <bool GN, int RB, bool PERROW = false, int J = 8, bool GB = false>
int launch(const dsc_gemm_args* a, const uint16_t* planes_f, int ntok, hipStream_t s) {
    const int scenes = (a->m + ntok - 1) / ntok;
    const unsigned grid = (unsigned)(((scenes + WAVES - 1) / WAVES) * (a->n / (16 * J)));
    DSC_CLEAR_STALE_ERROR();
    hipLaunchKernelGGL((gemm_split_wave_kernel<GN, RB, PERROW, J, GB>), dim3(grid, (unsigned)a->batch), dim3(64 * WAVES), 0, s, *a, planes_f, ntok DSC_WAVE_STAMP_PASS);
    DSC_LAUNCH_CHECK();
    return 0;
}

}
```

diffuscene_amd/engine.py:

```python
import ctypes as C

import torch

from . import _lib, ops
from ._lib import ACT_GELU, ACT_NONE, ACT_SILU, SS_BY_INDEX, SS_NONE, SS_PER_SCENE, SS_PER_SLOT, SS_PER_TOKEN

D = 512
HID = 128
DEC_PAD = 32


def _own(t):
    if isinstance(t, torch.nn.Parameter):
        return t.detach()
    if isinstance(t, (tuple, list)):
        return tuple(_own(u) for u in t)
    return t


class StalePlanError(RuntimeError):
    pass


class _Pool:
    def __init__(self, device):
        self.device = device
        self.free_list = {}
        self.all = []
        self.bytes = 0

    def get(self, rows, cols):
        key = (rows, cols)
        lst = self.free_list.get(key)
        if lst:
            return lst.pop()
        t = torch.empty((rows, cols), device=self.device, dtype=torch.float32)
        self.all.append(t)
        self.bytes += t.numel() * 4
        return t

    def put(self, t):
        self.free_list.setdefault((t.shape[0], t.shape[1]), []).append(t)


class Plan:

    def __init__(self, eng, B, N, ctx_mode, ctx_dim, L, text_dim, time_table=False):
        self.eng, self.B, self.N, self.M = eng, B, N, B * N
        self.generation = eng.generation
        dev = eng.device
        self.pool = _Pool(dev)
        self.keep = []
        self.steps = []
        self.pre_steps = []
        net = eng.net
        C_in = net.channels
        self.x_in = torch.empty((self.M, C_in), device=dev, dtype=torch.float32)
        self.t_in = torch.empty((B,), device=dev, dtype=torch.int64)
        ctx_rows = {SS_NONE: 0, SS_PER_SLOT: N, SS_PER_TOKEN: self.M}[ctx_mode]
        self.ctx_in = torch.empty((ctx_rows, ctx_dim), device=dev, dtype=torch.float32) if ctx_rows else None
        self.cross_in = torch.empty((B * L, text_dim), device=dev, dtype=torch.float32) if L else None
        self.ctx_mode = ctx_mode
        self.L = L
        self.time_table = time_table
        self.out = torch.empty((self.M, net.out_dim), device=dev, dtype=torch.float32)
        self._build()
        self.tiled_steps = self.steps

    def gemm_args(self):
        kinds = {id(_lib.fn("dsc_gemm_gn_silu_f32")): "gn", id(_lib.fn("dsc_gemm_f32")): "plain"}
        out = []
        for f, a in self.steps:
            k = kinds.get(id(f))
            if k is not None:
                out.append((k, a[0]._obj))
        return out

    def gemm(self, a, w, out, bias=None, a2=None, residual=None, act_in=ACT_NONE, act_out=ACT_NONE, row_invariant=False):
        g = ops.make_gemm_args(a, w, out, bias, a2, residual, act_in, act_out, row_invariant=row_invariant)
        lay = ops.planes_layout(g)
        pl = self.eng.planes_of(w, lay) if lay >= 0 else None
        if pl is not None:
            ops.attach_planes(g, pl, layout=lay)
        self.keep.append(_own((g, a, w, out, bias, a2, residual, pl)))
        self.steps.append((_lib.fn("dsc_gemm_f32"), (C.byref(g),)))
        return out

    def gemm_batched(self, a, w, out, bias, batch, sa, sw, sy, sbias, act_out=ACT_NONE):
        stacked = w._base if w._base is not None else w
        g = ops.make_gemm_args(a, w, out, bias, None, None, ACT_NONE, act_out)
        g.batch, g.sa1, g.sw, g.sy, g.sbias = batch, sa, sw, sy, sbias
        whole = (stacked.dim() == 2 and stacked.is_contiguous() and w.data_ptr() == stacked.data_ptr()
                 and stacked.shape[0] == batch * w.shape[0] and stacked.shape[1] == w.shape[1] and sw == w.shape[0] * w.shape[1])
        lay = ops.planes_layout(g) if whole else -1
        pl = self.eng.planes_of(stacked, lay) if lay >= 0 else None
        if pl is not None:
            ops.attach_planes(g, pl, layout=lay)
        self.keep.append(_own((g, a, w, out, bias, pl)))
        self.steps.append((_lib.fn("dsc_gemm_f32"), (C.byref(g),)))
        return out

    def gemm_gn(self, a, w, out, bias, gamma, beta, a2=None, ss=None, ss_mode=SS_NONE, residual=None):
        g = ops.make_gemm_args(a, w, out, bias, a2, residual, gamma=gamma, beta=beta, eps=1e-5,
                               tokens_per_scene=self.N, scale_shift=ss, ss_mode=ss_mode if ss is not None else SS_NONE,
                               ss_index=self.t_in if (ss is not None and ss_mode == SS_BY_INDEX) else None)
        lay = ops.planes_layout(g, gn=True)
        pl = self.eng.planes_of(w, lay) if lay >= 0 else None
        if pl is not None:
            ops.attach_planes(g, pl, gn=True, layout=lay)
        self.keep.append(_own((g, a, w, out, bias, a2, residual, gamma, beta, ss, pl)))
        self.steps.append((_lib.fn("dsc_gemm_gn_silu_f32"), (C.byref(g),)))
        return out

    def call(self, name, *args, keep=()):
        self.keep.append(_own(keep))
        self.steps.append((_lib.fn(name), args))

    def hoist(self, first):
        if self.time_table:
            self.pre_steps += self.steps[first:]
            del self.steps[first:]
            return True
        return False

    def check_current(self):
        if self.generation != self.eng.generation:
            raise StalePlanError("diffuscene_amd: this launch plan was built for parameter storages the model no longer uses (flat storage "
                                 "of the first training step, module.to(), load into new tensors): rebuild it -- DenoiserEngine.prepare() / "
                                 "graph_sample_loop() do -- instead of running or replaying it")

    def run_pre(self):
        self.check_current()
        s = ops.stream_ptr()
        for f, a in self.pre_steps:
            rc = f(*a, s)
            if rc:
                _lib.check(rc, f.__name__)

    def layernorm(self, x, g, out, residual=None):
        self.call("dsc_layernorm_f32", x.data_ptr(), x.stride(0), g.data_ptr(),
                  residual.data_ptr() if residual is not None else None,
                  residual.stride(0) if residual is not None else 0,
                  out.data_ptr(), out.stride(0), x.shape[0], x.shape[1], 1e-5, keep=(x, g, out, residual))
        return out

    def out_proj_ln(self, a, conv, ln_gain, residual):
        M = self.M
        out = self.pool.get(M, D)
        if (M + 95) // 96 >= 160:
            g = ops.make_gemm_args(a, conv.weight, out, conv.bias, None, residual, gamma=ln_gain.view(-1), beta=ln_gain.view(-1),
                                   eps=1e-5)
            self.keep.append(_own((g, a, conv.weight, out, conv.bias, residual, ln_gain)))
            self.steps.append((_lib.fn("dsc_gemm_layernorm_f32"), (C.byref(g),)))
            return out
        o = self.gemm(a, conv.weight, self.pool.get(M, D), conv.bias)
        self.layernorm(o, ln_gain, out, residual=residual)
        self.pool.put(o)
        return out

    def resblock(self, rb, x, x2, ss, ss_mode):
        e, M = self.eng, self.M
        h = self.pool.get(M, D)
        self.gemm_gn(x, e.ws[id(rb.block1.proj)], h, rb.block1.proj.bias, rb.block1.norm.weight, rb.block1.norm.bias,
                     a2=x2, ss=ss, ss_mode=ss_mode)
        if rb.has_res_conv:
            r = self.pool.get(M, D)
            self.gemm(x, rb.res_conv.weight, r, rb.res_conv.bias, a2=x2)
        else:
            r = x
        out = self.pool.get(M, D)
        self.gemm_gn(h, e.ws[id(rb.block2.proj)], out, rb.block2.proj.bias, rb.block2.norm.weight, rb.block2.norm.bias,
                     residual=r)
        self.pool.put(h)
        if rb.has_res_conv:
            self.pool.put(r)
        return out

    def t_ss(self, rb):
        i = self.eng.t_index[id(rb)]
        return self.ss_t[:, i * 2 * D:(i + 1) * 2 * D], (SS_BY_INDEX if self.time_table else SS_PER_SCENE)

    def c_ss(self, rb):
        if self.ss_c is None:
            return None, SS_NONE
        i = self.eng.c_index[id(rb)]
        return self.ss_c[:, i * 2 * D:(i + 1) * 2 * D], self.ctx_mode

    def linattn(self, blk, x):
        M, B, N = self.M, self.B, self.N
        att = blk.fn.fn
        y = self.layernorm(x, blk.fn.norm.g, self.pool.get(M, D))
        qkv = self.gemm(y, att.to_qkv.weight, self.pool.get(M, 3 * HID))
        self.pool.put(y)
        a = self.pool.get(M, HID)
        self.call("dsc_linear_attention_f32", qkv.data_ptr(), 3 * HID, qkv.data_ptr() + 4 * HID, 3 * HID,
                  qkv.data_ptr() + 8 * HID, 3 * HID, a.data_ptr(), HID, B, N, N, float(att.scale), keep=(qkv, a))
        self.pool.put(qkv)
        out = self.out_proj_ln(a, att.to_out[0], att.to_out[1].g, x)
        self.pool.put(a)
        return out

    def crossattn(self, blk, x):
        M, B, N, L = self.M, self.B, self.N, self.L
        att = blk.fn.fn
        y = self.layernorm(x, blk.fn.norm.g, self.pool.get(M, D))
        q = self.gemm(y, att.to_q.weight, self.pool.get(M, HID))
        self.pool.put(y)
        first = len(self.steps)
        kv = self.gemm(self.cross_in, att.to_kv.weight, self.pool.get(B * L, 2 * HID))
        kv_is_invariant = self.hoist(first)
        a = self.pool.get(M, HID)
        self.call("dsc_linear_attention_f32", q.data_ptr(), HID, kv.data_ptr(), 2 * HID, kv.data_ptr() + 4 * HID,
                  2 * HID, a.data_ptr(), HID, B, N, L, float(att.scale), keep=(q, kv, a))
        self.pool.put(q)
        if not kv_is_invariant:
            self.pool.put(kv)
        out = self.out_proj_ln(a, att.to_out[0], att.to_out[1].g, x)
        self.pool.put(a)
        return out

    def fullattn(self, blk, x):
        M, B, N = self.M, self.B, self.N
        att = blk.fn.fn
        y = self.layernorm(x, blk.fn.norm.g, self.pool.get(M, D))
        qkv = self.gemm(y, att.to_qkv.weight, self.pool.get(M, 3 * HID))
        self.pool.put(y)
        a = self.pool.get(M, HID)
        self.call("dsc_attention_f32", qkv.data_ptr(), 3 * HID, qkv.data_ptr() + 4 * HID, 3 * HID,
                  qkv.data_ptr() + 8 * HID, 3 * HID, a.data_ptr(), HID, B, N, float(att.scale), keep=(qkv, a))
        self.pool.put(qkv)
        out = self.gemm(a, att.to_out.weight, self.pool.get(M, D), att.to_out.bias, residual=x)
        self.pool.put(a)
        return out

    def _build(self):
        e, net, M, B = self.eng, self.eng.net, self.M, self.B
        pool = self.pool
        if self.time_table:
            self.ss_t = e.ss_table()
        else:
            temb = pool.get(B, D)
            self.call("dsc_time_embedding_f32", self.t_in.data_ptr(), B, D, e.time_table.data_ptr(),
                      e.time_table.shape[0], e.time_freq.data_ptr(), temb.data_ptr(), keep=(temb,))
            t1 = self.gemm(temb, net.time_mlp[1].weight, pool.get(B, 4 * D), net.time_mlp[1].bias, act_out=ACT_GELU, row_invariant=True)
            t2 = self.gemm(t1, net.time_mlp[3].weight, pool.get(B, 4 * D), net.time_mlp[3].bias, act_out=ACT_SILU, row_invariant=True)
            self.ss_t = self.gemm(t2, e.t_pack_w, pool.get(B, e.t_pack_w.shape[0]), e.t_pack_b, row_invariant=True)
        if self.ctx_in is not None:
            first = len(self.steps)
            cact = pool.get(self.ctx_in.shape[0], self.ctx_in.shape[1])
            self.call("dsc_activation_f32", self.ctx_in.data_ptr(), cact.data_ptr(), self.ctx_in.numel(), ACT_SILU,
                      keep=(cact,))
            self.ss_c = self.gemm(cact, e.c_pack_w, pool.get(self.ctx_in.shape[0], e.c_pack_w.shape[0]), e.c_pack_b)
            self.hoist(first)
        else:
            self.ss_c = None
        if net.seperate_all:
            bb, nc, no, nf = net.bbox_dim, net.class_dim, net.objectness_dim, net.objfeat_dim
            emb = pool.get(M, D)
            H = len(e.enc_heads)
            h1 = pool.get(M, H * D)
            items = (_lib.SmallKItem * H)()
            for i, (seq, c0, k) in enumerate(e.enc_heads):
                xs = self.x_in[:, c0:c0 + k]
                items[i].x, items[i].ldx, items[i].k_in = xs.data_ptr(), self.x_in.stride(0), k
                items[i].w, items[i].ldw, items[i].bias = seq[0].weight.data_ptr(), k, seq[0].bias.data_ptr()
                items[i].y, items[i].ldy = h1.data_ptr() + 4 * i * D, H * D
            self.call("dsc_linear_smallk_grouped_f32", items, H, M, D, ACT_GELU,
                      keep=(items, h1, [(seq[0].weight, seq[0].bias) for seq, _, _ in e.enc_heads]))
            h2 = pool.get(M, H * 2 * D)
            self.gemm_batched(h1[:, :D], e.enc_w2[:2 * D], h2[:, :2 * D], e.enc_b2[:2 * D], H, D, 2 * D * D, 2 * D, 2 * D,
                              act_out=ACT_GELU)
            pool.put(h1)
            self.gemm(h2, e.enc_w3, emb, e.enc_b3)
            pool.put(h2)
            x = self.gemm(emb, net.init_conv.weight, pool.get(M, D), net.init_conv.bias)
            pool.put(emb)
        else:
            x = pool.get(M, D)
            k = net.channels
            self.call("dsc_linear_smallk_f32", self.x_in.data_ptr(), self.x_in.stride(0), k,
                      net.init_conv.weight.data_ptr(), k, net.init_conv.bias.data_ptr(), x.data_ptr(), D, M, D,
                      ACT_NONE, keep=(x, net.init_conv.weight, net.init_conv.bias))
        r = x
        skips = []
        text = net.text_condition

        def step(rb, xin, x2, ss_pair, free_in=True):
            out = self.resblock(rb, xin, x2, *ss_pair)
            if free_in and xin is not r and all(xin is not s for s in skips):
                pool.put(xin)
            return out

        for lvl in net.downs:
            b0, b1, ac, b2, la, down = lvl
            x = step(b0, x, None, self.c_ss(b0))
            x = step(b1, x, None, self.t_ss(b1))
            skips.append(x)
            if text:
                x = self.crossattn(ac, x)
            x = step(b2, x, None, self.t_ss(b2))
            xo = self.linattn(la, x)
            pool.put(x)
            x = xo
            skips.append(x)
            if isinstance(down, torch.nn.Conv1d):
                x = self.gemm(x, down.weight, pool.get(M, D), down.bias)
        x = step(net.mid_block0, x, None, self.c_ss(net.mid_block0))
        x = step(net.mid_block1, x, None, self.t_ss(net.mid_block1))
# ... 244 lines not shown
```

diffuscene_amd/ops.py:

```python
import ctypes as C
import numbers

import torch

from . import _lib
from ._lib import (ACT_GELU, ACT_NONE, ACT_SILU, MEAN_EPS, MEAN_V, MEAN_X0, SS_NONE, SS_PER_SCENE,
                   SS_PER_SLOT, SS_PER_TOKEN, GemmArgs, SplitItem, WsItem)


def stream_ptr():
    return torch.cuda.current_stream().cuda_stream


def _dev(t, name="tensor", dtype=torch.float32):
    if not isinstance(t, torch.Tensor) or not t.is_cuda:
        raise RuntimeError("diffuscene_amd: %s must live on a HIP device (no CPU fallback exists)" % name)
    if t.dtype != dtype:
        raise RuntimeError("diffuscene_amd: %s must be %s, got %s" % (name, dtype, t.dtype))
    return t


def _mat(t, name):
    _dev(t, name)
    if t.dim() != 2 or (t.shape[1] > 1 and t.stride(1) != 1):
        raise RuntimeError("diffuscene_amd: %s must be a 2-D tensor with contiguous rows, got shape %s strides %s"
                           % (name, tuple(t.shape), t.stride()))
    return t.data_ptr(), (t.stride(0) if t.shape[0] > 1 else t.shape[1])


def as2d(w):
    return w.view(w.shape[0], w.shape[1]) if w.dim() == 3 else w


def make_gemm_args(a, w, y, bias=None, a2=None, residual=None, act_in=ACT_NONE, act_out=ACT_NONE,
                   gamma=None, beta=None, eps=1e-5, tokens_per_scene=0, scale_shift=None, ss_mode=SS_NONE, preact=None,
                   ss_index=None, w_planes=None, actgrad_x=None, gnb=None, row_invariant=False):
    g = GemmArgs()
    g.a1, g.lda1 = _mat(a, "a")
    g.k1 = a.shape[1]
    if a2 is not None:
        g.a2, g.lda2 = _mat(a2, "a2")
        g.k2 = a2.shape[1]
        if a2.shape[0] != a.shape[0]:
            raise RuntimeError("a and a2 row mismatch")
    w2 = as2d(w)
    g.w, g.ldw = _mat(w2, "w")
    if w2.shape[1] != g.k1 + g.k2:
        raise RuntimeError("weight K (%d) != activation K (%d)" % (w2.shape[1], g.k1 + g.k2))
    g.m, g.n = a.shape[0], w2.shape[0]
    g.y, g.ldy = _mat(y, "y")
    if tuple(y.shape) != (g.m, g.n):
        raise RuntimeError("output shape %s != (%d, %d)" % (tuple(y.shape), g.m, g.n))
    if bias is not None:
        g.bias = _dev(bias, "bias").data_ptr()
    if residual is not None:
        g.residual, g.ldr = _mat(residual, "residual")
    g.act_in, g.act_out, g.batch = act_in, act_out, 1
    if row_invariant:
        g.flags |= _lib.GEMM_ROW_INVARIANT
    if gamma is not None:
        g.gamma, g.beta, g.eps = _dev(gamma).data_ptr(), _dev(beta).data_ptr(), eps
        g.tokens_per_scene = tokens_per_scene
    if scale_shift is not None:
        g.scale_shift, g.ld_ss = _mat(scale_shift, "scale_shift")
        g.ss_mode = ss_mode
    if preact is not None:
        g.preact, g.ld_preact = _mat(preact, "preact")
    if actgrad_x is not None:
        g.actgrad_x, g.ld_actgrad = _mat(actgrad_x, "actgrad_x")
        if tuple(actgrad_x.shape) != (g.m, g.n):
            raise RuntimeError("actgrad_x shape %s != (%d, %d)" % (tuple(actgrad_x.shape), g.m, g.n))
    if gnb is not None:
        g.gnb_z, g.ld_gnb_z = _mat(gnb["z"], "gnb z")
        g.gnb_dgamma, g.gnb_dbeta, g.gnb_dbias = gnb["dgamma"], gnb["dbeta"], gnb["dbias"]
        g.gnb_pstride = gnb["pstride"]
        if gnb.get("dss") is not None:
            g.gnb_dss, g.ld_gnb_dss = _mat(gnb["dss"], "gnb dss")
    if ss_index is not None:
        if scale_shift is None:
            raise RuntimeError("ss_index (DSC_SS_BY_INDEX) needs the scale_shift table it indexes")
        g.ss_index = _dev(ss_index, "ss_index", torch.int64).data_ptr()
        g.ss_rows = scale_shift.shape[0]
    if w_planes is not None:
        if (w_planes.dtype != torch.int16 or w_planes.dim() != 3 or w_planes.shape[0] != 3 or w_planes.shape[1] % g.n
                or w_planes.shape[2] != g.k1 + g.k2 or not w_planes.is_contiguous()):
            raise RuntimeError("w_planes must be a contiguous int16 tensor of shape (3, %d, %d)" % (g.n, g.k1 + g.k2))
        attach_planes(g, w_planes, gn=gamma is not None and gnb is None)
    return g


PLANES_ROWMAJOR, PLANES_FRAGMENT = 0, 1


def planes_layout(g, gn=False):
    r = _lib.fn("dsc_gemm_planes_layout")(C.byref(g), 1 if gn else 0)
    if r == _lib.DSC_PLANES_NONE:
        return -1
    if r < 0:
        _lib.check(r, "dsc_gemm_planes_layout")
    return r


def fragment_major(planes):
    _, n, k = planes.shape
    return planes.view(3, n // 16, 16, k // 32, 4, 8).permute(0, 1, 3, 4, 2, 5).contiguous().view(3, n, k)


def attach_planes(g, planes, gn=False, layout=None):
    want = planes_layout(g, gn)
    if layout is None:
        layout = getattr(planes, "_dsc_layout", PLANES_ROWMAJOR)
        if want == PLANES_FRAGMENT and layout == PLANES_ROWMAJOR:
            cached = getattr(planes, "_dsc_fragment", None)
            if cached is None or cached[0] != planes._version:
                cached = planes._dsc_fragment = (planes._version, fragment_major(planes))
            planes, layout = cached[1], PLANES_FRAGMENT
            g._planes_keep = planes
    g.w_planes = planes.data_ptr()
    g.w_planes_layout = layout
    return g


def planes_wanted(n, k):
    return n % 128 == 0 and k % 32 == 0 and 6 * n * k < 0x7fffffff


def split_planes(items, stream=None):
    out, batch = [], []
    for w, planes, tr in items:
        tr = int(tr)
        frag, tr = tr & 2, tr & 1
        w2 = as2d(_dev(w, "w"))
        ptr, ldw = _mat(w2, "w")
        r, c = w2.shape
        shape = (3, c, r) if tr else (3, r, c)
        if planes is None:
            planes = torch.empty(shape, device=w2.device, dtype=torch.int16)
        elif tuple(planes.shape) != shape or planes.dtype != torch.int16 or not planes.is_contiguous():
            raise RuntimeError("split_planes: planes must be contiguous int16 %s" % (shape,))
        planes._dsc_layout = PLANES_FRAGMENT if frag else PLANES_ROWMAJOR
        planes._dsc_fragment = None
        out.append(planes)
# ... 774 lines not shown
```

diffuscene_amd/train_plan.py:

```python
import ctypes as C
import os

import torch

from ._lib import ACT_GELU, ACT_NONE, ACT_SILU, SS_NONE, SS_PER_SCENE, SS_PER_SLOT, SS_PER_TOKEN

D = 512
HID = 128


def _as2d(w):
    return w.view(w.shape[0], w.shape[1]) if w.dim() == 3 else w


class H:
    __slots__ = ("t", "g", "ng", "act_of", "g_pre", "uses", "gn_of", "gn_part")

    def __init__(self, t, needs_grad=True):
        self.t, self.g, self.ng = t, None, needs_grad
        self.uses = 0
        self.act_of = None
        self.g_pre = None
        self.gn_of = None
        self.gn_part = None


def tn_token_slices(groups, tile_n, blocks_target, tile_k=128):
    def tiles(n, k):
        return ((n + tile_n - 1) // tile_n) * ((k + tile_k - 1) // tile_k)
    work = {}
    for m, n, k in groups:
        work[m] = work.get(m, 0) + tiles(n, k) * m
    m_ref = max(work, key=lambda m: (work[m], m))
    long_tiles = sum(tiles(n, k) for m, n, k in groups if 2 * m >= m_ref)
    return max(1, min(32, m_ref // 256, -(-blocks_target // max(long_tiles, 1)))), m_ref


def long_k_splits(K):
    return next((s for s in range(64, 1, -1) if K % (32 * s) == 0 and K // s >= 256), 0)


def tn_block_map(groups, n_xcd=8, tile_k=128):
    def tiles(n, k):
        return ((n + 255) // 256) * ((k + tile_k - 1) // tile_k)
    _, m_ref = tn_token_slices(groups, 256, 768)
    lists = [[] for _ in range(n_xcd)]
    work = [0] * n_xcd
    order = sorted(range(len(groups)), key=lambda i: (-groups[i][0], -tiles(groups[i][1], groups[i][2]), i))
    short = []
    for gi in order:
        m, n, k = groups[gi]
        nt = tiles(n, k)
        if 2 * m >= m_ref and nt <= 64:
            x = min(range(n_xcd), key=lambda j: (work[j], j))
            lists[x].extend((gi, t) for t in range(nt))
            work[x] += nt * m
        else:
            short.append(gi)
    for gi in short:
        m, n, k = groups[gi]
        for t in range(tiles(n, k)):
            x = min(range(n_xcd), key=lambda j: (len(lists[j]), j))
            lists[x].append((gi, t))
    depth = max(len(l) for l in lists)
    out = []
    for pos in range(depth):
        for x in range(n_xcd):
            out.append(lists[x][pos] if pos < len(lists[x]) else (-1, -1))
    return out


class HipBackend:

    name = "hip"

    def __init__(self, device):
        from . import _lib
        _lib.load()
        self.lib = _lib
        self.device = device
        self.keep = []
        self.scratch_floats = 0
        self.scratch = None
        self._scratch_users = []
        self.split = _lib.split_enabled()
        self._planes = {}
        self._planes_new = []
        self.plane_bytes = 0
        self.transposed_of = {}
        self.f32_reads = set()

    def planes_of(self, w, rows, layout=0):
        from . import ops
        if not self.split or rows < 256 or w.dim() != 2 or w.stride(1) != 1 or not ops.planes_wanted(w.shape[0], w.shape[1]):
            return None
        key = (w.data_ptr(), tuple(w.shape), w.stride(0), layout)
        ent = self._planes.get(key)
        if ent is None:
            planes = torch.empty((3,) + tuple(w.shape), device=self.device, dtype=torch.int16)
            self.plane_bytes += planes.numel() * 2
            src = self.transposed_of.get(w.data_ptr())
            if src is not None and (not w.is_contiguous() or tuple(src.shape) != (w.shape[1], w.shape[0])):
                src = None
            if src is None:
                self.f32_reads.add(w.untyped_storage().data_ptr())
            ent = self._planes[key] = (w, planes, src, 2 * layout)
            self._planes_new.append(ent)
        return ent[1]

    def split_steps(self):
        from . import ops
        ents, self._planes_new = self._planes_new, []
        steps = []
        for i in range(0, len(ents), self.lib.WS_MAX):
            part = ents[i:i + self.lib.WS_MAX]
            arr = (self.lib.SplitItem * len(part))()
            for j, (w, planes, src, frag) in enumerate(part):
                if src is not None:
                    ptr, ldw = ops._mat(src, "w")
                    arr[j].w, arr[j].ldw, arr[j].rows, arr[j].cols, arr[j].planes, arr[j].transpose = (
                        ptr, ldw, src.shape[0], src.shape[1], planes.data_ptr(), 1 | frag)
                    continue
                ptr, ldw = ops._mat(w, "w")
                arr[j].w, arr[j].ldw, arr[j].rows, arr[j].cols, arr[j].planes, arr[j].transpose = (
                    ptr, ldw, w.shape[0], w.shape[1], planes.data_ptr(), frag)
            steps.append(self._call("dsc_split_bf16x3_f32", arr, len(part), keep=(arr, part)))
        return steps

    def _mat(self, t):
        from .ops import _mat
        return _mat(t, "plan tensor")

    def _call(self, name, *args, keep=()):
        from .engine import _own
        self.keep.append(_own(keep))
        return (self.lib.fn(name), args, name)

    def finalize(self):
        self.scratch = torch.empty(max(self.scratch_floats, 1), device=self.device, dtype=torch.float32)
        for fix in self._scratch_users:
            fix(self.scratch)

    def _with_scratch(self, floats, build):
        self.scratch_floats = max(self.scratch_floats, int(floats))
        holder = {}

        def fix(scr):
            holder["step"] = build(scr.data_ptr(), scr.numel())
        self._scratch_users.append(fix)
        return holder

    def fuse_act_ok(self, a, w, out, a2=None, bias=None, preact=None, actgrad_x=None):
        from . import ops
        if not self.split or a.shape[0] < 256 or os.environ.get("DSC_FUSE_ACT", "1") == "0":
            return False
        g = ops.make_gemm_args(a, w, out, bias, a2, act_out=ACT_GELU if (preact is not None or actgrad_x is not None) else ACT_NONE,
                               preact=preact, actgrad_x=actgrad_x)
        lay = ops.planes_layout(g)
        return lay >= 0 and self.planes_of(w, a.shape[0], lay) is not None

    def gemm(self, a, w, out, bias=None, a2=None, residual=None, act_out=ACT_NONE, preact=None, actgrad_x=None):
        from . import ops
        m, K = a.shape
        if preact is not None or actgrad_x is not None:
            g = ops.make_gemm_args(a, w, out, bias, a2, residual, ACT_NONE, act_out, preact=preact, actgrad_x=actgrad_x)
            lay = ops.planes_layout(g)
            pl = self.planes_of(w, m, lay) if lay >= 0 else None
            if pl is None:
                raise RuntimeError("HipBackend.gemm: an activation epilogue was planned for a launch the split kernel does not take")
            ops.attach_planes(g, pl, layout=lay)
            return self._call("dsc_gemm_f32", C.byref(g), keep=(g, a, w, out, bias, a2, residual, pl, preact, actgrad_x))
        tiles = ((m + 63) // 64) * ((out.shape[1] + 63) // 64)
        if a2 is None and act_out == ACT_NONE and tiles < 256 and K >= 1024 and (m * out.shape[1]) % 4 == 0:
            splits = next((s for s in (8, 4, 2) if K % (32 * s) == 0 and K // s >= 128), 0)
            if splits:
                fn = self.lib.fn("dsc_gemm_splitk_f32")
                floats = splits * m * out.shape[1]
                g = ops.make_gemm_args(a, w, out, bias, a2, residual, ACT_NONE, act_out)
                from .engine import _own
                self.keep.append(_own((g, a, w, out, bias, residual)))
                self.f32_reads.add(w.untyped_storage().data_ptr())
                return self._with_scratch(floats, lambda wp, wn: (fn, (C.byref(g), splits, wp, wn), "dsc_gemm_splitk_f32"))
        g = ops.make_gemm_args(a, w, out, bias, a2, residual, ACT_NONE, act_out)
        lay = ops.planes_layout(g)
        pl = self.planes_of(w, m, lay) if lay >= 0 else None
        if pl is not None:
            ops.attach_planes(g, pl, layout=lay)
        else:
            self.f32_reads.add(w.untyped_storage().data_ptr())
        return self._call("dsc_gemm_f32", C.byref(g), keep=(g, a, w, out, bias, a2, residual, pl))

    def _gnbwd_args(self, dy, wt, dz, gn, part):
        from . import ops
        Cc = dz.shape[1]
        pp, ps = (part.data_ptr(), part.stride(0)) if part is not None else (0x100000, 3 * Cc)
        g = ops.make_gemm_args(dy, wt, dz, gamma=gn["gamma"], beta=gn["beta"], eps=1e-5, tokens_per_scene=gn["n_tok"],
                               scale_shift=gn["ss"], ss_mode=gn["ss_mode"] if gn["ss"] is not None else SS_NONE,
                               gnb=dict(z=gn["z"], dgamma=pp + 4 * Cc, dbeta=pp + 8 * Cc, dbias=pp, pstride=ps, dss=gn["dss"]))
        return g

    def fuse_gnbwd_ok(self, dy, wt, like, gn):
        from . import ops
        if not self.split or os.environ.get("DSC_FUSE_GNBWD", "1") == "0" or gn["ss_mode"] not in (SS_NONE, SS_PER_SCENE):
            return False
        g = self._gnbwd_args(dy, wt, like, gn, None)
        return ops.planes_layout(g) == ops.PLANES_FRAGMENT and self.planes_of(wt, dy.shape[0], ops.PLANES_FRAGMENT) is not None

    def gemm_gnbwd(self, dy, wt, dz, gn, part):
        from . import ops
        g = self._gnbwd_args(dy, wt, dz, gn, part)
        lay = ops.planes_layout(g)
        pl = self.planes_of(wt, dy.shape[0], lay) if lay >= 0 else None
        if pl is None:
            raise RuntimeError("HipBackend.gemm_gnbwd: planned for a launch the wave-autonomous kernel does not take")
        ops.attach_planes(g, pl, layout=lay)
        return self._call("dsc_gemm_f32", C.byref(g), keep=(g, dy, wt, dz, gn["z"], gn["gamma"], gn["beta"], gn["ss"], gn["dss"], part, pl))

    def gemm_long_k(self, a, w, out, residual=None):
        from . import ops
        m, K = a.shape
        n = out.shape[1]
        if (m * n) % 4 or K % 32:
            return None
        splits = long_k_splits(K)
        if not splits:
            return None
        fn = self.lib.fn("dsc_gemm_splitk_f32")
        g = ops.make_gemm_args(a, w, out, None, None, residual, ACT_NONE, ACT_NONE)
        from .engine import _own
        self.keep.append(_own((g, a, w, out, residual)))
        self.f32_reads.add(w.untyped_storage().data_ptr())
        floats = splits * m * n
        return self._with_scratch(floats, lambda wp, wn: (fn, (C.byref(g), splits, wp, wn), "dsc_gemm_splitk_f32"))

    def gemm_gn(self, a, w, out, bias, gamma, beta, n_tok, a2=None, ss=None, ss_mode=SS_NONE, residual=None, preact=None):
        from . import ops
        g = ops.make_gemm_args(a, w, out, bias, a2, residual, gamma=gamma, beta=beta, eps=1e-5, tokens_per_scene=n_tok,
                               scale_shift=ss, ss_mode=ss_mode if ss is not None else SS_NONE, preact=preact)
        lay = ops.planes_layout(g, gn=True)
        pl = self.planes_of(w, a.shape[0], lay) if lay >= 0 else None
        if pl is not None:
            ops.attach_planes(g, pl, gn=True, layout=lay)
        else:
            self.f32_reads.add(w.untyped_storage().data_ptr())
        return self._call("dsc_gemm_gn_silu_f32", C.byref(g), keep=(g, a, w, out, bias, gamma, beta, a2, ss, residual, preact, pl))

    def smallk(self, x, w, bias, out, act_out=ACT_NONE):
        xp, ldx = self._mat(x)
        wp, ldw = self._mat(w)
        yp, ldy = self._mat(out)
        return self._call("dsc_linear_smallk_f32", xp, ldx, x.shape[1], wp, ldw, bias.data_ptr() if bias is not None else None,
                          yp, ldy, x.shape[0], w.shape[0], act_out, keep=(x, w, bias, out))

    def ws(self, weights, outs):
        from . import ops
        steps = []
        for i in range(0, len(weights), self.lib.WS_MAX):
            arr = ops.make_ws_items(list(zip(weights[i:i + self.lib.WS_MAX], outs[i:i + self.lib.WS_MAX])))
            steps.append(self._call("dsc_weight_standardize_f32", arr, len(arr), 1e-5, keep=(arr, weights, outs)))
        return steps

    def time_embedding(self, t, table, freq, out):
        return self._call("dsc_time_embedding_f32", t.data_ptr(), t.shape[0], out.shape[1], table.data_ptr(), table.shape[0],
                          freq.data_ptr(), out.data_ptr(), keep=(t, table, freq, out))

    def act(self, x, out, kind):
# ... 406 lines not shown
            dst, acc = self.g_target(a)
            self._gemm_acc(dy, wt, dst, acc)
            return
        want1, want2 = a.ng, a2.ng
        if not (want1 or want2):
            return
        pair_fresh = a.g is None and a2.g is None and want1 and want2
        same_parent = (a.g is not None and a2.g is not None and a.g.stride(0) == K and a2.g.stride(0) == K
                       and a2.g.data_ptr() == a.g.data_ptr() + 4 * k1)
        if pair_fresh:
            buf = self.new(dy.shape[0], K)
            a.g, a2.g = buf[:, :k1], buf[:, k1:]
            self._gemm_acc(dy, wt, buf, False)
        elif same_parent:
            buf = torch.as_strided(a.g, (a.g.shape[0], K), (K, 1))
            self._guard(buf)
            self._gemm_acc(dy, wt, buf, True)
        else:
            tmp = self.new(dy.shape[0], K)
            self._gemm_acc(dy, wt, tmp, False)
            if want1:
                self.g_alias(a, tmp[:, :k1])
            if want2:
                self.g_alias(a2, tmp[:, k1:])

    def _gemm_acc(self, dy, wt, dst, acc):
        n = dy.shape[1]
        if n > 4096 and hasattr(self.be, "gemm_long_k"):
            step = self.be.gemm_long_k(dy, wt, dst, dst if acc else None)
            if step is not None:
                self.emit(step)
                return
        if n > 4096:
            for c0 in range(0, n, 2048):
                c1 = min(c0 + 2048, n)
                self.emit(self.be.gemm(dy[:, c0:c1], wt[:, c0:c1], dst, residual=dst if (acc or c0 > 0) else None))
        else:
            self.emit(self.be.gemm(dy, wt, dst, residual=dst if acc else None))

    def tn(self, a, dy, out, a2=None, kvalid=None, dbias=None, params=(), after=None):
        self._tn_pending.append({"a": a, "dy": dy, "out": out, "a2": a2, "kvalid": kvalid, "dbias": dbias,
                                 "params": tuple(p for p in params if p is not None), "after": after})
        if self.tn_flush_floats and sum(it["out"].numel() for it in self._tn_pending) >= self.tn_flush_floats:
            self.flush_tn()

    def colsum_later(self, x, out, params=(), after=None):
        if not hasattr(self.be, "colsum_grouped"):
            self.emit(self.be.colsum(x, out))
            if after is not None:
                after()
            self.wrote(*params)
            return
        self._cs_pending.append({"x": x, "out": out, "params": tuple(params), "after": after})

    def flush_tn(self):
        cs, self._cs_pending = self._cs_pending, []
        if cs:
            self.emit(self.be.colsum_grouped([(it["x"], it["out"]) for it in cs]))
            for it in cs:
                if it["after"] is not None:
                    it["after"]()
            self.wrote(*[p for it in cs for p in it["params"]])
        items, self._tn_pending = self._tn_pending, []
        if not items:
            return
        self.emit(self.be.gemm_tn_grouped(items))
        for it in items:
            if it["after"] is not None:
                it["after"]()
        self.wrote(*[p for it in items for p in it["params"]])

    def wT(self, w2d, npad=None):
        n, K = w2d.shape
        if npad is None or npad == n:
            buf = self.new(K, n)
            self._transposes.append((w2d, buf))
            if hasattr(self.be, "transposed_of"):
                self.be.transposed_of[buf.data_ptr()] = w2d
            return buf
        buf = self.zeros(K, npad)
        self._transposes.append((w2d, buf[:, :n]))
        return buf

    def linear(self, a, weight, bias, a2=None, residual=None, out=None, act_out=ACT_NONE, wt=None, act=None):
        w2 = _as2d(weight)
        n, K = w2.shape
        rows = a.t.shape[0]
        y = H(out if out is not None else self.new(rows, n))
        self._use(a, a2, residual)
        assert act_out == ACT_NONE, "training keeps the pre-activation (its backward needs it): use act="
        fused = (act is not None and residual is None and out is None and hasattr(self.be, "fuse_act_ok")
                 and self.be.fuse_act_ok(a.t, w2, y.t, a2.t if a2 is not None else None, bias=bias, preact=y.t))
        if fused:
            ya_t = self.new(rows, n)
            self.emit(self.be.gemm(a.t, w2, ya_t, bias, a2.t if a2 is not None else None, None, act, preact=y.t))
        else:
            self.emit(self.be.gemm(a.t, w2, y.t, bias, a2.t if a2 is not None else None,
                                   residual.t if residual is not None else None, act_out))

        def bw():
            dy = y.g
            if dy is None:
                return
            npad = (n + 31) // 32 * 32
            if npad != n:
                dyp = self.zeros(rows, npad)
                self.emit(self.be.copy(dyp[:, :n], dy))
            elif not self._dense_ok(dy):
                dyp = self.new(rows, n)
                self.emit(self.be.copy(dyp, dy))
            else:
                dyp = dy
            if a.ng or (a2 is not None and a2.ng):
                self.g_gemm(a, a2, dyp, wt if wt is not None else self.wT(w2, npad))
            gw = self.gview(weight)
            gb = self.flat.grad_view(bias) if bias is not None else None
            if npad != n:
                tw = self.new(npad, K)
                tb = self.new(1, npad) if bias is not None else None

                def unpad():
                    self.emit(self.be.copy(gw, tw[:n]))
                    if bias is not None:
                        self.emit(self.be.copy(gb.view(1, n), tb[:, :n]))
                self.tn(a.t, dyp, tw, a2.t if a2 is not None else None, dbias=tb.view(-1) if tb is not None else None,
                        params=(weight, bias), after=unpad)
            else:
                self.tn(a.t, dyp, gw, a2.t if a2 is not None else None, dbias=gb, params=(weight, bias))
            if residual is not None:
                self.g_alias(residual, dy)
        self._tape.append(bw)
        if act is None:
            return y
        return self.act(y, act, out=ya_t if fused else None)

    def smallk(self, x_slice, weight, bias):
        w2 = _as2d(weight)
        n, k = w2.shape
        rows = x_slice.shape[0]
        y = H(self.new(rows, n))
        self.emit(self.be.smallk(x_slice, w2, bias, y.t))
        xpad = self.zeros(rows, 32 if k <= 32 else 64)
        self.emit(self.be.copy(xpad[:, :k], x_slice))

        def bw():
            if y.g is None:
                return
            self.tn(xpad, y.g, self.gview(weight), kvalid=k, dbias=self.flat.grad_view(bias), params=(weight, bias))
        self._tape.append(bw)
        return y

    def act(self, x, kind, out=None):
        y = H(out if out is not None else self.new(*x.t.shape))
        if out is None:
            self.emit(self.be.act(x.t, y.t, kind))
        y.act_of = (x.t, kind)

        def bw():
            if y.g_pre is not None:
                self.g_alias(x, y.g_pre)
                if y.g is None:
                    return
            if y.g is None or not x.ng:
                return
            dy = y.g
            if not dy.is_contiguous():
                d = self.new(*dy.shape)
                self.emit(self.be.copy(d, dy))
                dy = d
            self.g_write(x, lambda dst: self.emit(self.be.act_bwd(x.t, dy, dst, kind)))
        self._tape.append(bw)
        return y

    def conv_gn(self, a, blk, a2=None, ss=None, ss_mode=SS_NONE, dss=None, residual=None):
        conv, norm = blk.proj, blk.norm
        w_std = self.ws_std[id(conv)]
        rows = a.t.shape[0]
        y, z = H(self.new(rows, D)), self.new(rows, D)
        self._use(a, a2, residual)
        self.emit(self.be.gemm_gn(a.t, w_std, y.t, conv.bias, norm.weight, norm.bias, self.N, a2.t if a2 is not None else None,
                                  ss, ss_mode, residual.t if residual is not None else None, z))

        if residual is None:
            y.gn_of = dict(z=z, gamma=norm.weight, beta=norm.bias, ss=ss, ss_mode=ss_mode if ss is not None else SS_NONE,
                           dss=dss if (ss is not None and ss_mode == SS_PER_SCENE) else None, n_tok=self.N)

        def bw():
            dy = y.g
            if dy is None and y.g_pre is None:
                return
            scenes = rows // self.N
            slot_tmp = None
            if y.g_pre is not None:
                dz, part = y.g_pre, y.gn_part
            else:
                dz = self.new(rows, D)
                part = self.new(scenes, 3 * D)
                dss_arg = dss
                if ss is not None and ss_mode == SS_PER_SLOT:
                    slot_tmp = self.new(rows, 2 * D)
                    dss_arg = slot_tmp
                self.emit(self.be.gn_bwd(z, dy, norm.weight, norm.bias, ss, ss_mode, dz, part, dss_arg, scenes, self.N))
            o_b, o_g, o_be = (self.flat.grad_range(p)[0] for p in (conv.bias, norm.weight, norm.bias))
            if o_g == o_b + D and o_be == o_g + D:
                self.colsum_later(part, self.flat.G[o_b:o_b + 3 * D], params=(conv.bias, norm.weight, norm.bias))
            else:
                tmp = self.new(1, 3 * D)

                def scatter(tmp=tmp):
                    for i, p in enumerate((conv.bias, norm.weight, norm.bias)):
                        self.emit(self.be.copy(self.flat.grad_view(p).view(1, D), tmp[:, i * D:(i + 1) * D]))
                self.colsum_later(part, tmp.view(-1), params=(conv.bias, norm.weight, norm.bias), after=scatter)
            if slot_tmp is not None:
                red = self.new(self.N, 2 * D)
                self.emit(self.be.colsum(slot_tmp.view(scenes, self.N * 2 * D), red.view(-1)))
                self.emit(self.be.copy(dss, red))
            self.g_gemm(a, a2, dz, self.ws_t[id(conv)])
            self.tn(a.t, dz, self.dws[id(conv)], a2.t if a2 is not None else None)
            self._ws_pending.append(conv)
            if residual is not None:
                self.g_alias(residual, dy)
        self._tape.append(bw)
        return y

    def resblock(self, rb, a, a2, ss_pair, post=None):
        if post is not None:
            self._tape.append(post)
        ss, mode, dss = ss_pair
        h = self.conv_gn(a, rb.block1, a2=a2, ss=ss, ss_mode=mode, dss=dss)
        r = self.linear(a, rb.res_conv.weight, rb.res_conv.bias, a2=a2) if rb.has_res_conv else a
        return self.conv_gn(h, rb.block2, residual=r)

    def layernorm(self, x, gain, residual=None):
        g = gain.view(-1)
        y = H(self.new(*x.t.shape))
        self._use(x, residual)
        self.emit(self.be.layernorm(x.t, g, y.t, residual.t if residual is not None else None))

        def bw():
            dy = y.g
            if dy is None:
                return
            M_ = x.t.shape[0]
            nblk = min((M_ + 3) // 4, 512)
            part = self.new(nblk, x.t.shape[1])
            self.g_write_add(x, lambda dst, addend: self.emit(self.be.layernorm_bwd(x.t, g, dy, dst, part, addend)))
            self.colsum_later(part, self.flat.grad_view(gain).view(-1), params=(gain,))
            if residual is not None:
                self.g_alias(residual, dy)
        self._tape.append(bw)
        return y

    def linattn(self, blk, a):
        att = blk.fn.fn
        B, N = self.B, self.N
        y = self.layernorm(a, blk.fn.norm.g)
        qkv = self.linear(y, att.to_qkv.weight, None)
        o = H(self.new(self.M, HID))
        q, k, v = qkv.t[:, :HID], qkv.t[:, HID:2 * HID], qkv.t[:, 2 * HID:]
        self.emit(self.be.linattn(q, k, v, o.t, B, N, N, float(att.scale)))

        def bw():
            if o.g is None:
                return
            d = self.new(self.M, 3 * HID)
            qkv.g = d
            self.emit(self.be.linattn_bwd(q, k, v, o.g, d[:, :HID], d[:, HID:2 * HID], d[:, 2 * HID:], B, N, N,
                                          float(att.scale)))
        self._tape.append(bw)
        p = self.linear(o, att.to_out[0].weight, att.to_out[0].bias)
        return self.layernorm(p, att.to_out[1].g, residual=a)

    def crossattn(self, blk, a):
        att = blk.fn.fn
        B, N, L = self.B, self.N, self.L
        y = self.layernorm(a, blk.fn.norm.g)
        qh = self.linear(y, att.to_q.weight, None)
        kv = self.linear(self.cross_in, att.to_kv.weight, None)
        o = H(self.new(self.M, HID))
        self.emit(self.be.linattn(qh.t, kv.t[:, :HID], kv.t[:, HID:], o.t, B, N, L, float(att.scale)))

        def bw():
            if o.g is None:
                return
            dq, dkv = self.new(self.M, HID), self.new(B * L, 2 * HID)
            qh.g, kv.g = dq, dkv
            self.emit(self.be.linattn_bwd(qh.t, kv.t[:, :HID], kv.t[:, HID:], o.g, dq, dkv[:, :HID], dkv[:, HID:], B, N, L,
                                          float(att.scale)))
        self._tape.append(bw)
        p = self.linear(o, att.to_out[0].weight, att.to_out[0].bias)
        return self.layernorm(p, att.to_out[1].g, residual=a)

    def fullattn(self, blk, a):
        att = blk.fn.fn
        B, N = self.B, self.N
        y = self.layernorm(a, blk.fn.norm.g)
        qkv = self.linear(y, att.to_qkv.weight, None)
        o = H(self.new(self.M, HID))
        q, k, v = qkv.t[:, :HID], qkv.t[:, HID:2 * HID], qkv.t[:, 2 * HID:]
        self.emit(self.be.attn(q, k, v, o.t, B, N, float(att.scale)))

        def bw():
            if o.g is None:
                return
            d = self.new(self.M, 3 * HID)
            qkv.g = d
            self.emit(self.be.attn_bwd(q, k, v, o.g, d[:, :HID], d[:, HID:2 * HID], d[:, 2 * HID:], B, N, float(att.scale)))
        self._tape.append(bw)
        return self.linear(o, att.to_out.weight, att.to_out.bias, residual=a)

    def encoder(self, seq, c0, k, acc):
        xf = self.x_t.view(self.M, -1)
        h = self.act(self.smallk(xf[:, c0:c0 + k], seq[0].weight, seq[0].bias), ACT_GELU)
        h = self.linear(h, seq[2].weight, seq[2].bias, act=ACT_GELU)
        return self.linear(h, seq[4].weight, seq[4].bias, residual=acc)

    def _build(self):
        net, be, B, N, M = self.net, self.be, self.B, self.N, self.M
        diff = self.diff
        tb = self._tables if self._tables is not None else diff.tables(self.device)
        self.tb = tb
        fl = self.flat
        want_v = diff.model_mean_type == "v"
        self.v_buf = self.new3(B, N, net.channels) if want_v else None
        self.emit(be.q_sample(self.x0, self.noise, self.t, tb["sqrt_alphas_cumprod"], tb["sqrt_one_minus_alphas_cumprod"],
                              self.x_t, self.v_buf))
        self.target = {"v": self.v_buf, "eps": self.noise, "x0": self.x0}[diff.model_mean_type]
        blocks = net.resblocks_in_order()
        ws_mods = []
        for rb, _ in blocks:
            ws_mods += [rb.block1.proj, rb.block2.proj]
        self.ws_mods = ws_mods
        self.ws_std = {id(m): self.new(*_as2d(m.weight).shape) for m in ws_mods}
        self.dws = {id(m): self.new(*_as2d(m.weight).shape) for m in ws_mods}
        self.ws_t = {id(m): self.new(_as2d(m.weight).shape[1], _as2d(m.weight).shape[0]) for m in ws_mods}
        self._ws_pending = []
        self.emit(be.ws([_as2d(m.weight) for m in ws_mods], [self.ws_std[id(m)] for m in ws_mods]))
        self._fwd_split_at = len(self.fwd)
        for m in ws_mods:
            self._transposes.append((self.ws_std[id(m)], self.ws_t[id(m)]))
            if hasattr(be, "transposed_of"):
                be.transposed_of[self.ws_t[id(m)].data_ptr()] = self.ws_std[id(m)]
        t_blocks = [rb for rb, kind in blocks if kind == "t"]
        c_blocks = [rb for rb, kind in blocks if kind == "c" and rb.mlp is not None]
        t_index = {id(rb): i for i, rb in enumerate(t_blocks)}
        c_index = {id(rb): i for i, rb in enumerate(c_blocks)}
        eng_table = net.time_table.to(self.device)
        eng_freq = net.time_freq.to(self.device)
        temb = H(self.new(B, D), needs_grad=False)
        self.emit(be.time_embedding(self.t, eng_table, eng_freq, temb.t))
        t1 = self.linear(temb, net.time_mlp[1].weight, net.time_mlp[1].bias, act=ACT_GELU)
        t2 = self.linear(t1, net.time_mlp[3].weight, net.time_mlp[3].bias, act=ACT_SILU)
        tw, tgw = fl.packed["t_w"]
        tbias, tgb = fl.packed["t_b"]
        ss_t = H(self.new(B, tw.shape[0]))
        self.emit(be.gemm(t2.t, tw, ss_t.t, tbias))
        dss_t = self.new(B, tw.shape[0])
        ss_t.g = dss_t
        tw_t = self.wT(tw)

        def bw_time_pack():
            self.g_gemm(t2, None, dss_t, tw_t)
            if self.per_block_grads:
                return
            self.tn(t2.t, dss_t, tgw, dbias=tgb, after=lambda: (self.wrote_range(*fl.pack_range["t_w"]),
                                                                 self.wrote_range(*fl.pack_range["t_b"])))
        self._tape.append(bw_time_pack)
        self._t_pack = (t2, dss_t, tgw, tgb)

        ss_c = dss_c = None
        if self.ctx_in is not None and c_blocks:
            cact = self.act(self.ctx_in, ACT_SILU)
            cw, cgw = fl.packed["c_w"]
            cb, cgb = fl.packed["c_b"]
            ss_c = H(self.new(self.ctx_in.t.shape[0], cw.shape[0]))
            self.emit(be.gemm(cact.t, cw, ss_c.t, cb))
            dss_c = self.new(self.ctx_in.t.shape[0], cw.shape[0])
            ss_c.g = dss_c
            cw_t = self.wT(cw)

# ... 202 lines not shown
```

include/diffuscene_hip.h:

```cpp
#ifndef DIFFUSCENE_HIP_H
#define DIFFUSCENE_HIP_H

#include <stdint.h>

#ifdef __cplusplus
extern "C" {
#endif

typedef void* dsc_stream_t;

#define DSC_EINVAL   (-1)
#define DSC_EALIGN   (-2)
#define DSC_ERANGE   (-3)

#define DSC_ACT_NONE 0
#define DSC_ACT_GELU 1
#define DSC_ACT_SILU 2
#define DSC_ACT_LEAKY01 3

#define DSC_SS_NONE      0
#define DSC_SS_PER_TOKEN 1
#define DSC_SS_PER_SCENE 2
#define DSC_SS_PER_SLOT  3
#define DSC_SS_BY_INDEX  4

#define DSC_HEADS    4
#define DSC_DIM_HEAD 32

int dsc_version(void);

typedef struct dsc_gemm_args {
    const float* a1; int64_t lda1; int32_t k1;
    const float* a2; int64_t lda2; int32_t k2;
    const float* w;  int64_t ldw;
    const float* bias;
    const float* residual; int64_t ldr;
    float* y; int64_t ldy;
    int32_t m, n;
    int32_t act_in;
    int32_t act_out;
    int32_t batch; int64_t sa1, sa2, sw, sbias, sres, sy;
    const float* gamma; const float* beta; float eps;
    int32_t tokens_per_scene;
    const float* scale_shift; int64_t ld_ss; int32_t ss_mode;
    float* preact; int64_t ld_preact;
    const int64_t* ss_index;
    const uint16_t* w_planes;
    const float* actgrad_x; int64_t ld_actgrad;
    int32_t ss_rows;
    int32_t w_planes_layout;
    const float* gnb_z; int64_t ld_gnb_z;
    float* gnb_dgamma; float* gnb_dbeta; float* gnb_dbias; int64_t gnb_pstride;
    float* gnb_dss; int64_t ld_gnb_dss;
    int32_t flags;
} dsc_gemm_args;
#define DSC_GEMM_ROW_INVARIANT 1
#define DSC_PLANES_ROWMAJOR 0
#define DSC_PLANES_FRAGMENT 1
#define DSC_PLANES_NONE (-100)

int dsc_gemm_f32(const dsc_gemm_args* args, dsc_stream_t stream);

int dsc_gemm_arithmetic(const dsc_gemm_args* args, int32_t gn);

#define DSC_TILE_GN_32       0
#define DSC_TILE_GN_80_W8    1
#define DSC_TILE_GN_80_W4    2
#define DSC_TILE_GN_48       3
#define DSC_TILE_GN_64       4
#define DSC_TILE_160x256     5
#define DSC_TILE_256x128     6
#define DSC_TILE_128x128     7
#define DSC_TILE_160x128_W4  8
#define DSC_TILE_64x256      9
#define DSC_TILE_WAVE_GN     10
#define DSC_TILE_WAVE_DENSE  11
#define DSC_TILE_WAVE_GN_64  12
int dsc_gemm_split_tile(const dsc_gemm_args* args, int32_t gn);

#define DSC_F32_TILE_160x256 0
#define DSC_F32_TILE_160x128 1
#define DSC_F32_TILE_128x128 2
#define DSC_F32_TILE_96x128  3
#define DSC_F32_TILE_64x64   4
int dsc_gemm_f32_tile(const dsc_gemm_args* args);

int dsc_gemm_planes_layout(const dsc_gemm_args* args, int32_t gn);

int dsc_get_split_wave(void);
int dsc_set_split_wave(int32_t mode);

int dsc_gemm_skinny(const dsc_gemm_args* args, int32_t gn);
int dsc_get_skinny(void);
int dsc_set_skinny(int32_t on);

int dsc_get_gemm_arithmetic(void);
int dsc_set_gemm_arithmetic(int32_t mode);

#define DSC_SPLIT_TRANSPOSE 1
#define DSC_SPLIT_FRAGMENT  2
typedef struct dsc_split_item { const float* w; int64_t ldw; int32_t rows, cols; uint16_t* planes; int32_t transpose; } dsc_split_item;
int dsc_split_bf16x3_f32(const dsc_split_item* items, int32_t count, dsc_stream_t stream);

int dsc_gemm_gn_silu_f32(const dsc_gemm_args* args, dsc_stream_t stream);

int dsc_gemm_splitk_f32(const dsc_gemm_args* a, int32_t splits, float* workspace, int64_t workspace_floats, dsc_stream_t stream);

int dsc_gemm_layernorm_f32(const dsc_gemm_args* a, dsc_stream_t stream);

int dsc_linear_smallk_f32(const float* x, int64_t ldx, int32_t k_in, const float* w, int64_t ldw,
                          const float* bias, float* y, int64_t ldy, int32_t m, int32_t n,
                          int32_t act_out, dsc_stream_t stream);
#define DSC_SMALLK_MAX 4
typedef struct dsc_smallk_item { const float* x; int64_t ldx; int32_t k_in; const float* w; int64_t ldw; const float* bias;
                                 float* y; int64_t ldy; } dsc_smallk_item;
int dsc_linear_smallk_grouped_f32(const dsc_smallk_item* items, int32_t count, int32_t m, int32_t n, int32_t act_out,
                                  dsc_stream_t stream);
typedef struct dsc_col_span { int32_t src_col, dst_col, width; } dsc_col_span;
int dsc_gather_columns_f32(float* dst, int64_t ldd, const float* src, int64_t lds, int32_t rows, const dsc_col_span* spans,
                           int32_t count, dsc_stream_t stream);

#define DSC_WS_MAX 64
typedef struct dsc_ws_item { const float* w; float* out; int32_t rows; int32_t cols; } dsc_ws_item;
int dsc_weight_standardize_f32(const dsc_ws_item* items, int32_t count, float eps, dsc_stream_t stream);

int dsc_layernorm_f32(const float* x, int64_t ldx, const float* g, const float* residual, int64_t ldr,
                      float* y, int64_t ldy, int32_t m, int32_t d, float eps, dsc_stream_t stream);

int dsc_linear_attention_f32(const float* q, int64_t ldq, const float* k, int64_t ldk,
                             const float* v, int64_t ldv, float* out, int64_t ldo,
                             int32_t scenes, int32_t nq, int32_t nk, float scale, dsc_stream_t stream);

int dsc_attention_f32(const float* q, int64_t ldq, const float* k, int64_t ldk,
                      const float* v, int64_t ldv, float* out, int64_t ldo,
                      int32_t scenes, int32_t n, float scale, dsc_stream_t stream);

int dsc_time_embedding_f32(const int64_t* t, int32_t b, int32_t dim, const float* table, int32_t table_rows,
                           const float* freq, float* out, dsc_stream_t stream);

int dsc_activation_f32(const float* x, float* y, int64_t count, int32_t act, dsc_stream_t stream);


int64_t dsc_device_error_count(int32_t reset);

int dsc_q_sample_f32(const float* x0, const float* noise, const int64_t* t,
                     const float* sqrt_ac, const float* sqrt_1mac,
                     float* x_t, float* v_out, int32_t b, int64_t inner, int32_t num_timesteps, dsc_stream_t stream);

#define DSC_MEAN_EPS 0
#define DSC_MEAN_X0  1
#define DSC_MEAN_V   2
int dsc_p_sample_f32(const float* x_t, const float* model_out, const float* noise, const int64_t* t,
                     const float* ca, const float* cb, const float* coef1, const float* coef2,
                     const float* sigma, float* out, float* x0_out ,
                     int32_t mean_type, int32_t clip, int32_t b, int64_t inner, int32_t num_timesteps,
                     dsc_stream_t stream);

int dsc_add_scalar_i64(int64_t* t, int32_t count, int64_t delta, dsc_stream_t stream);

int dsc_ddim_step_f32(const float* x_t, const float* model_out, const float* noise, const int64_t* step,
                      const int64_t* times, const int64_t* times_next, const float* sqrt_alpha_next,
                      const float* c_noise, const float* sigma, const float* ca, const float* cb,
                      const float* sqrt_recip_ac, const float* sqrt_recipm1_ac, float* out, float* x0_out,
                      int32_t mean_type, int32_t b, int64_t inner, int32_t num_steps, int32_t num_timesteps,
                      dsc_stream_t stream);

int dsc_ddim_advance_i64(int64_t* step, const int64_t* times, int64_t* t, int32_t count, int32_t num_steps,
                         dsc_stream_t stream);

int dsc_postfilter_compact_f32(const float* samples, int32_t b, int32_t n, int32_t c, int32_t empty_col, int32_t mode,
                               int32_t keep_empty, float* packed, int32_t* counts, dsc_stream_t stream);

int dsc_complete_overwrite_f32(float* x, const float* partial, const float* noise, const int64_t* t,
// ... 217 lines not shown
```

Baseline: 61.48 steps/s.

## Fuse QKV projection with linear attention in a per-head wave GEMM tile

Adds a head-aligned wave GEMM tile that computes one attention head's 96 Q/K/V channels per scene. For linear attention it can also run the softmax and context phases in the GEMM epilogue, writing the attention output directly. The goal is to drop the separate linear-attention kernel and the Q/K/V round trip through global memory in both the sampling and training forward passes. The shared softmax and context code moves into a common header. The cost is more shared memory per block and a tile that depends on shape and occupancy heuristics.

After: 61.89 steps/s (median of 6 runs). About the same (+0.7%).

```diff
diff --git a/__graft_entry__.py b/__graft_entry__.py
--- a/__graft_entry__.py
+++ b/__graft_entry__.py
@@ -47,8 +47,8 @@
 
 def build(force=False):
     hipcc = _hipcc()
-    headers = [os.path.join(CSRC, "dsc_common.h"), os.path.join(CSRC, "gemm_core.h"), os.path.join(CSRC, "gemm_tn_split.h"),
-               os.path.join(ROOT, "include", "diffuscene_hip.h")]
+    headers = [os.path.join(CSRC, h) for h in ("dsc_common.h", "gemm_core.h", "gemm_tn_split.h", "gemm_split_wave.h", "gemm_skinny.h",
+                                               "linattn_core.h")] + [os.path.join(ROOT, "include", "diffuscene_hip.h")]
     objs = []
     for src, extra in SOURCES:
         s = os.path.join(CSRC, src)
diff --git a/diffuscene_amd/_lib.py b/diffuscene_amd/_lib.py
--- a/diffuscene_amd/_lib.py
+++ b/diffuscene_amd/_lib.py
@@ -10,10 +10,12 @@
 SS_NONE, SS_PER_TOKEN, SS_PER_SCENE, SS_PER_SLOT, SS_BY_INDEX = 0, 1, 2, 3, 4
 MEAN_EPS, MEAN_X0, MEAN_V = 0, 1, 2
 TILE_GN_80_W8, TILE_GN_80_W4, TILE_160x256, TILE_160x128_W4 = 1, 2, 5, 8
-TILE_WAVE_GN, TILE_WAVE_DENSE, TILE_WAVE_GN_64 = 10, 11, 12
+TILE_WAVE_GN, TILE_WAVE_DENSE, TILE_WAVE_GN_64, TILE_WAVE_HEADS = 10, 11, 12, 13
 F32_TILE_160x256, F32_TILE_160x128, F32_TILE_128x128, F32_TILE_96x128, F32_TILE_64x64 = 0, 1, 2, 3, 4
 DSC_PLANES_NONE = -100
 GEMM_ROW_INVARIANT = 1
+GEMM_ATTN_HEADS = 2
+DSC_NOT_TAKEN = -101
 WS_MAX = 64
 MAX_TOKENS_PER_SCENE = 160
 STATS_MAX_OBJECTS, STATS_ONE_WAVE_MAX = 160, 32
@@ -106,6 +108,10 @@
     "dsc_gemm_planes_layout": (C.c_int, [C.POINTER(GemmArgs), C.c_int32]),
     "dsc_get_split_wave": (C.c_int, []),
     "dsc_set_split_wave": (C.c_int, [C.c_int32]),
+    "dsc_get_attn_heads": (C.c_int, []),
+    "dsc_set_attn_heads": (C.c_int, [C.c_int32]),
+    "dsc_qkv_linear_attention_f32": (C.c_int, [C.POINTER(GemmArgs), c_f32p, C.c_int64, C.c_int32, C.c_int32, C.c_int32, C.c_float,
+                                               C.c_int32, C.c_int32, C.c_void_p]),
     "dsc_gemm_skinny": (C.c_int, [C.POINTER(GemmArgs), C.c_int32]),
     "dsc_get_skinny": (C.c_int, []),
     "dsc_set_skinny": (C.c_int, [C.c_int32]),
@@ -259,6 +265,8 @@
         raise ValueError("DSC_TN_FORM=%r: must be '2' (default), '1' or '0'" % os.environ.get("DSC_TN_FORM"))
     if lib.dsc_get_split_wave() < 0:
         raise ValueError("DSC_WAVE=%r: must be '1' / 'auto' (default) or '0'" % os.environ.get("DSC_WAVE"))
+    if lib.dsc_get_attn_heads() < 0:
+        raise ValueError("DSC_ATTN_HEADS=%r: must be '1' (default) or '0'" % os.environ.get("DSC_ATTN_HEADS"))
     _lib = lib
     return lib
 
@@ -271,12 +279,19 @@
     lib = load()
     if lib.dsc_get_gemm_arithmetic() != 1:
         return 0
-    return (2 if lib.dsc_get_split_wave() == 1 else 1) + 10 * lib.dsc_get_tn_split_form()
+    wave = lib.dsc_get_split_wave() == 1
+    return (2 if wave else 1) + 10 * lib.dsc_get_tn_split_form() + (100 if wave and lib.dsc_get_attn_heads() == 1 else 0)
 
 
 def set_split_wave(on):
     prev = load().dsc_get_split_wave() == 1
     check(load().dsc_set_split_wave(1 if on else 0), "dsc_set_split_wave")
+    return prev
+
+
+def set_attn_heads(on):
+    prev = load().dsc_get_attn_heads() == 1
+    check(load().dsc_set_attn_heads(1 if on else 0), "dsc_set_attn_heads")
     return prev
 
 
diff --git a/diffuscene_amd/csrc/blocks.hip b/diffuscene_amd/csrc/blocks.hip
--- a/diffuscene_amd/csrc/blocks.hip
+++ b/diffuscene_amd/csrc/blocks.hip
@@ -1,4 +1,5 @@
 #include "dsc_common.h"
+#include "linattn_core.h"
 
 namespace {
 
@@ -88,7 +89,7 @@
 
 constexpr int MAXTOK = 160;
 constexpr int HP = 33;
-constexpr int LP = 36;
+constexpr int LP = dsc_la::LP;
 
 __global__ __launch_bounds__(256) void linear_attention_kernel(const float* __restrict__ q, int64_t ldq,
                                                                const float* __restrict__ k, int64_t ldk,
@@ -115,83 +116,15 @@
         *reinterpret_cast<f32x4*>(Qs + i * LP + c4) = *reinterpret_cast<const f32x4*>(qb + (int64_t)i * ldq + c4);
     }
     __syncthreads();
-    {
-        const int d = tid >> 3, part = tid & 7;
-        float mx = -INFINITY;
-        for (int j = part; j < nk; j += 8) mx = fmaxf(mx, Ks[j * LP + d]);
-        mx = fmaxf(mx, __shfl_xor(mx, 1, 64));
-        mx = fmaxf(mx, __shfl_xor(mx, 2, 64));
-        mx = fmaxf(mx, __shfl_xor(mx, 4, 64));
-        float sm = 0.f;
-        for (int j = part; j < nk; j += 8) {
-            const float e = expf(Ks[j * LP + d] - mx);
-            Ks[j * LP + d] = e;
-            sm += e;
-        }
-        sm += __shfl_xor(sm, 1, 64);
-        sm += __shfl_xor(sm, 2, 64);
-        sm += __shfl_xor(sm, 4, 64);
-        const float inv = 1.0f / sm;
-        for (int j = part; j < nk; j += 8) Ks[j * LP + d] *= inv;
-    }
-    __syncthreads();
-    {
-        const int d = tid >> 3, e0 = (tid & 7) * 4;
-        f32x4 a = {0.f, 0.f, 0.f, 0.f};
-        for (int j = 0; j < nk; ++j) {
-            const float kd = Ks[j * LP + d];
-            const f32x4 vv = *reinterpret_cast<const f32x4*>(Vs + j * LP + e0);
-#pragma unroll
-            for (int e = 0; e < 4; ++e) a[e] += kd * vv[e];
-        }
-        *reinterpret_cast<f32x4*>(ctx + d * LP + e0) = a;
-    }
+    dsc_la::phase1<1>(Ks, nk, tid);
+    __syncthreads();
+    dsc_la::phase2<1>(Ks, Vs, ctx, nk, tid >> 3, (tid & 7) * 4);
     __syncthreads();
     for (int i0 = 0; i0 < nq; i0 += 64) {
         const int i = i0 + (tid >> 2), part = tid & 3;
-        const bool ok = i < nq;
-        float qv[8];
-        float mx = -INFINITY;
-        if (ok) {
-            const f32x4 a = *reinterpret_cast<const f32x4*>(Qs + i * LP + part * 8);
-            const f32x4 c = *reinterpret_cast<const f32x4*>(Qs + i * LP + part * 8 + 4);
-#pragma unroll
-            for (int e = 0; e < 4; ++e) { qv[e] = a[e]; qv[4 + e] = c[e]; }
-#pragma unroll
-            for (int e = 0; e < 8; ++e) mx = fmaxf(mx, qv[e]);
-        }
-        mx = fmaxf(mx, __shfl_xor(mx, 1, 64));
-        mx = fmaxf(mx, __shfl_xor(mx, 2, 64));
-        float sm = 0.f;
-        if (ok) {
-#pragma unroll
-            for (int e = 0; e < 8; ++e) { qv[e] = expf(qv[e] - mx); sm += qv[e]; }
-        }
-        sm += __shfl_xor(sm, 1, 64);
-        sm += __shfl_xor(sm, 2, 64);
-        if (ok) {
-            const float inv = scale / sm;
-            f32x4 a, c;
-#pragma unroll
-            for (int e = 0; e < 4; ++e) { a[e] = qv[e] * inv; c[e] = qv[4 + e] * inv; }
-            *reinterpret_cast<f32x4*>(Qs + i * LP + part * 8) = a;
-            *reinterpret_cast<f32x4*>(Qs + i * LP + part * 8 + 4) = c;
-        }
+        dsc_la::phase3_softmax(Qs, nq, scale, i, part);
         __builtin_amdgcn_wave_barrier();
-        if (ok) {
-            f32x4 o0 = {0.f, 0.f, 0.f, 0.f}, o1 = {0.f, 0.f, 0.f, 0.f};
-#pragma unroll 8
-            for (int d = 0; d < 32; ++d) {
-                const float qd = Qs[i * LP + d];
-                const f32x4 c0 = *reinterpret_cast<const f32x4*>(ctx + d * LP + part * 8);
-                const f32x4 c1 = *reinterpret_cast<const f32x4*>(ctx + d * LP + part * 8 + 4);
-#pragma unroll
-                for (int e = 0; e < 4; ++e) { o0[e] += c0[e] * qd; o1[e] += c1[e] * qd; }
-            }
-            float* orow = out + ((int64_t)b * nq + i) * ldo + h * 32 + part * 8;
-            *reinterpret_cast<f32x4*>(orow) = o0;
-            *reinterpret_cast<f32x4*>(orow + 4) = o1;
-        }
+        dsc_la::phase3_out(Qs, ctx, out + ((int64_t)b * nq + i) * ldo + h * 32 + part * 8, nq, i, part);
     }
 }
 
diff --git a/diffuscene_amd/csrc/gemm_split.hip b/diffuscene_amd/csrc/gemm_split.hip
--- a/diffuscene_amd/csrc/gemm_split.hip
+++ b/diffuscene_amd/csrc/gemm_split.hip
@@ -422,7 +422,8 @@
 
 }
 
-enum { T_GN_32 = 0, T_GN_80_W8, T_GN_80_W4, T_GN_48, T_GN_64, T_160x256, T_256x128, T_128x128, T_160x128_W4, T_64x256, T_WAVE_GN, T_WAVE_DENSE, T_WAVE_GN_64 };
+enum { T_GN_32 = 0, T_GN_80_W8, T_GN_80_W4, T_GN_48, T_GN_64, T_160x256, T_256x128, T_128x128, T_160x128_W4, T_64x256, T_WAVE_GN, T_WAVE_DENSE, T_WAVE_GN_64, T_WAVE_HEADS };
+static inline bool is_wave_tile(int t) { return t == T_WAVE_GN || t == T_WAVE_DENSE || t == T_WAVE_GN_64 || t == T_WAVE_HEADS; }
 
 static std::atomic<int> g_gemm_arith{-1000};
 
@@ -458,6 +459,40 @@
     if (mode != 0 && mode != 1) return DSC_EINVAL;
     g_split_wave.store(mode, std::memory_order_relaxed);
     return 0;
+}
+
+static std::atomic<int> g_attn_heads{-1000};
+
+extern "C" int dsc_get_attn_heads(void) {
+    int m = g_attn_heads.load(std::memory_order_relaxed);
+    if (m == -1000) {
+        const char* e = getenv("DSC_ATTN_HEADS");
+        m = (!e || !e[0] || !strcmp(e, "1")) ? 1 : !strcmp(e, "0") ? 0 : DSC_EINVAL;
+        g_attn_heads.store(m, std::memory_order_relaxed);
+    }
+    return m;
+}
+
+extern "C" int dsc_set_attn_heads(int32_t mode) {
+    if (mode != 0 && mode != 1) return DSC_EINVAL;
+    g_attn_heads.store(mode, std::memory_order_relaxed);
+    return 0;
+}
+
+static bool heads_shape_ok(const dsc_gemm_args* a) {
+    const int K = a->k1 + a->k2, N = a->tokens_per_scene;
+    if (a->n != 3 * 128 || a->batch != 1 || (a->k1 % 64) || (a->k2 % 64) || K < 256) return false;
+    if (N <= 16 || N > 80 || (a->m % N)) return false;
+    if (a->residual || a->preact || a->actgrad_x || a->gnb_z || a->act_in != DSC_ACT_NONE || a->act_out != DSC_ACT_NONE) return false;
+    if (a->bias && !dsc_aligned16(a->bias)) return false;
+    if (3LL * a->n * K * 2 >= 0x7fffffffLL) return false;
+    const int64_t ld_max = a->lda1 > a->lda2 ? a->lda1 : a->lda2;
+    if (ld_max * 4 * 96 >= 0x7fffffffLL || a->ldy * 4 * 96 >= 0x7fffffffLL) return false;
+    return true;
+}
+static bool heads_fill(const dsc_gemm_args* a) {
+    const long w = (long)(a->m / a->tokens_per_scene) * 4, r = (w + 1023) / 1024;
+    return w * 5 >= r * 1024 * 4;
 }
 
 static int select_wave(const dsc_gemm_args* a, bool gn) {
@@ -473,6 +508,7 @@
     if (3LL * a->batch * a->n * K * 2 >= 0x7fffffffLL) return -1;
     const int64_t ld_max = a->lda1 > a->lda2 ? a->lda1 : a->lda2;
     if (ld_max * 4 * 96 >= 0x7fffffffLL) return -1;
+    if (!gn && (a->flags & DSC_GEMM_ATTN_HEADS) && dsc_get_attn_heads() == 1 && heads_shape_ok(a) && heads_fill(a)) return T_WAVE_HEADS;
     long waves;
     if (a->gnb_z) {
         const int N = a->tokens_per_scene;
@@ -551,13 +587,19 @@
     return best_blk >= MIN_BLOCKS ? best : -1;
 }
 
+static int launch_heads_rb(const dsc_gemm_args* a, const dsc_wave::head_args& ha, hipStream_t s) {
+    const int N = a->tokens_per_scene, rb = (N + 15) / 16;
+    return rb == 5 ? dsc_wave::launch_heads<5>(a, a->w_planes, N, ha, s) : rb == 4 ? dsc_wave::launch_heads<4>(a, a->w_planes, N, ha, s)
+         : rb == 3 ? dsc_wave::launch_heads<3>(a, a->w_planes, N, ha, s) : dsc_wave::launch_heads<2>(a, a->w_planes, N, ha, s);
+}
+
 int dsc_gemm_try_split(const dsc_gemm_args* a, bool gn, hipStream_t s) {
     using namespace dsc_split;
-    if (dsc_get_gemm_arithmetic() < 0 || dsc_get_split_wave() < 0) return DSC_EINVAL;
+    if (dsc_get_gemm_arithmetic() < 0 || dsc_get_split_wave() < 0 || dsc_get_attn_heads() < 0) return DSC_EINVAL;
     const int N = a->tokens_per_scene;
     const int tile = select_tile(a, gn);
     if (tile < 0) return DSC_SPLIT_NOT_TAKEN;
-    const int want = (tile == T_WAVE_GN || tile == T_WAVE_DENSE || tile == T_WAVE_GN_64) ? DSC_PLANES_FRAGMENT : DSC_PLANES_ROWMAJOR;
+    const int want = is_wave_tile(tile) ? DSC_PLANES_FRAGMENT : DSC_PLANES_ROWMAJOR;
     if (a->w_planes_layout != want) return DSC_EINVAL;
     switch (tile) {
         case T_GN_32: return launch<true, 4, 2, 2>(a, N, s);
@@ -586,8 +628,26 @@
             return rb == 5 ? dsc_wave::launch<true, 5>(a, a->w_planes, N, s) : rb == 4 ? dsc_wave::launch<true, 4>(a, a->w_planes, N, s)
                  : rb == 3 ? dsc_wave::launch<true, 3>(a, a->w_planes, N, s) : dsc_wave::launch<true, 2>(a, a->w_planes, N, s);
         }
+        case T_WAVE_HEADS: return launch_heads_rb(a, dsc_wave::head_args{nullptr, 0, 0.f, 1}, s);
         default: return DSC_SPLIT_NOT_TAKEN;
     }
+}
+
+extern "C" int dsc_qkv_linear_attention_f32(const dsc_gemm_args* a, float* out, int64_t ldo, int32_t scenes, int32_t nq, int32_t nk, float scale,
+                                            int32_t store_qkv, int32_t mode, dsc_stream_t stream) {
+    if (!a || !a->a1 || !out || scenes < 1 || nq < 1 || nk < 1 || (mode != 0 && mode != 1)) return DSC_EINVAL;
+    if (a->m <= 0 || a->n <= 0 || a->k1 <= 0 || a->k2 < 0 || (a->k2 > 0 && !a->a2) || (store_qkv && !a->y)) return DSC_EINVAL;
+    if (dsc_get_gemm_arithmetic() < 0 || dsc_get_split_wave() < 0 || dsc_get_attn_heads() < 0) return DSC_EINVAL;
+    if (nq != nk) return DSC_EINVAL;
+    if (a->tokens_per_scene != nq || (int64_t)scenes * nq != a->m) return DSC_EINVAL;
+    if (!dsc_aligned16(a->a1) || (a->lda1 & 3) || (a->k2 > 0 && (!dsc_aligned16(a->a2) || (a->lda2 & 3)))) return DSC_EALIGN;
+    if (!dsc_aligned16(out) || (ldo & 3) || ldo < 128) return DSC_EALIGN;
+    if (store_qkv && (!dsc_aligned16(a->y) || (a->ldy & 3) || a->ldy < a->n)) return DSC_EALIGN;
+    if ((a->flags & DSC_GEMM_ROW_INVARIANT) || !heads_shape_ok(a)) return DSC_NOT_TAKEN;
+    if (!a->w_planes || !dsc_aligned16(a->w_planes)) return DSC_NOT_TAKEN;
+    if (mode == 0 && (dsc_get_gemm_arithmetic() != 1 || dsc_get_split_wave() != 1 || dsc_get_attn_heads() != 1 || !heads_fill(a))) return DSC_NOT_TAKEN;
+    if (a->w_planes_layout != DSC_PLANES_FRAGMENT) return DSC_EINVAL;
+    return launch_heads_rb(a, dsc_wave::head_args{out, ldo, scale, store_qkv ? 1 : 0}, static_cast<hipStream_t>(stream));
 }
 
 extern "C" int dsc_gemm_arithmetic(const dsc_gemm_args* a, int32_t gn) {
@@ -603,7 +663,7 @@
 extern "C" int dsc_gemm_planes_layout(const dsc_gemm_args* a, int32_t gn) {
     if (!a || a->m <= 0 || a->n <= 0 || a->k1 <= 0) return DSC_EINVAL;
     const int tile = select_tile(a, gn != 0, true);
-    return tile < 0 ? DSC_PLANES_NONE : (tile == T_WAVE_GN || tile == T_WAVE_DENSE || tile == T_WAVE_GN_64) ? DSC_PLANES_FRAGMENT : DSC_PLANES_ROWMAJOR;
+    return tile < 0 ? DSC_PLANES_NONE : is_wave_tile(tile) ? DSC_PLANES_FRAGMENT : DSC_PLANES_ROWMAJOR;
 }
 
 extern "C" int dsc_split_bf16x3_f32(const dsc_split_item* items, int32_t count, dsc_stream_t stream) {
diff --git a/diffuscene_amd/csrc/gemm_split_wave.h b/diffuscene_amd/csrc/gemm_split_wave.h
--- a/diffuscene_amd/csrc/gemm_split_wave.h
+++ b/diffuscene_amd/csrc/gemm_split_wave.h
@@ -1,5 +1,6 @@
 #pragma once
 #include "dsc_common.h"
+#include "linattn_core.h"
 #include <utility>
 
 #ifndef DSC_WAVE_STAMP_ARGS
@@ -46,19 +47,33 @@
     p3 = __builtin_bit_cast(bf16x8, c);
 }
 
-template <int RB>
-constexpr int wave_smem_bytes() { return WAVES * 2 * 3 * (16 * RB) * 64; }
-
-template <bool GN, int RB, bool PERROW = false, int J = 8, bool GB = false>
-__global__ __launch_bounds__(64 * WAVES, 1) void gemm_split_wave_kernel(const dsc_gemm_args p, const uint16_t* const planes_f, const int ntok DSC_WAVE_STAMP_ARGS) {
-    static_assert(J == 8 || J == 4, "wave tile: 128 or 64 channels");
+struct head_args {
+    float* out;
+    int64_t ldo;
+    float scale;
+    int store_qkv;
+};
+
+template <int RB, bool HD = false>
+constexpr int wave_image_bytes() {
+    constexpr int kloop = 2 * 3 * (16 * RB) * 64, heads = (3 * 16 * RB + 32) * dsc_la::LP * 4;
+    return HD && heads > kloop ? heads : kloop;
+}
+template <int RB, bool HD = false>
+constexpr int wave_smem_bytes() { return WAVES * wave_image_bytes<RB, HD>(); }
+
+template <bool GN, int RB, bool PERROW = false, int J = 8, bool GB = false, bool HD = false>
+__global__ __launch_bounds__(64 * WAVES, 1) void gemm_split_wave_kernel(const dsc_gemm_args p, const uint16_t* const planes_f, const int ntok,
+                                                                        const head_args ha DSC_WAVE_STAMP_ARGS) {
+    static_assert(HD ? J == 6 : (J == 8 || J == 4), "wave tile: 128 or 64 channels, or the 96 channels of one head");
     static_assert(!GB || (!GN && J == 8), "the GroupNorm-backward epilogue rides on the dense 80 x 128 form");
+    static_assert(!HD || (!GN && !GB && !PERROW), "the head tile is a dense form");
     constexpr int NWF = 3 * J;
     constexpr int CW = 16 * J;
     constexpr int ROWS = 16 * RB, XP = ROWS * 64, STAGE = 3 * XP;
     constexpr int NWB = RB > 4 ? RB - 2 : RB > 3 ? RB - 1 : RB;
     constexpr int PERW = (NWF + NWB - 1) / NWB;
-    __shared__ __attribute__((aligned(16))) char smem[wave_smem_bytes<RB>()];
+    __shared__ __attribute__((aligned(16))) char smem[wave_smem_bytes<RB, HD>()];
     const int lane = threadIdx.x & 63;
     const int wave = __builtin_amdgcn_readfirstlane(threadIdx.x >> 6);
     const int K = p.k1 + p.k2, KT = K / BK;
@@ -96,20 +111,21 @@
     const __amdgpu_buffer_rsrc_t rw = __builtin_amdgcn_make_buffer_rsrc(const_cast<uint16_t*>(planes_f), 0, (int)recw, 0x00020000);
 #endif
     const int plane_bytes = p.batch * p.n * K * 2;
-    const int nb0 = (z * p.n + col0) / 16;
+    const int nbz = z * p.n / 16;
+    auto cblk = [&](const int j) { return HD ? (j >> 1) * 8 + 2 * ch + (j & 1) : ch * J + j; };
 
     const int q4 = lane & 3, r16 = lane >> 2, g = lane >> 4, l15 = lane & 15;
     const int tvo1 = (r16 * (int)p.lda1 + q4 * 8) * 4, tvo2 = (r16 * (int)p.lda2 + q4 * 8) * 4;
     const int ildso = r16 * 64 + ((q4 ^ ((r16 >> 1) & 3)) << 4);
     const int xoff = l15 * 64 + ((g ^ ((l15 >> 1) & 3)) << 4);
     const int wvo = lane * 16;
-    char* const wl = smem + wave * (2 * STAGE);
+    char* const wl = smem + wave * wave_image_bytes<RB, HD>();
 
     f32x4 acc[RB][J];
 #pragma unroll
     for (int j = 0; j < J; ++j) {
         f32x4 b4 = {0.f, 0.f, 0.f, 0.f};
-        if (bias) b4 = *reinterpret_cast<const f32x4*>(bias + col0 + j * 16 + 4 * g);
+        if (bias) b4 = *reinterpret_cast<const f32x4*>(bias + cblk(j) * 16 + 4 * g);
 #pragma unroll
         for (int i = 0; i < RB; ++i) acc[i][j] = b4;
     }
@@ -137,7 +153,7 @@
     };
     auto load_w = [&](int kt, int j, int pl) -> bf16x8 {
 #if defined(__HIP_DEVICE_COMPILE__)
-        return __builtin_bit_cast(bf16x8, __builtin_amdgcn_raw_buffer_load_b128(rw, wvo, pl * plane_bytes + ((nb0 + j) * KT + kt) * 1024, 0));
+        return __builtin_bit_cast(bf16x8, __builtin_amdgcn_raw_buffer_load_b128(rw, wvo, pl * plane_bytes + ((nbz + cblk(j)) * KT + kt) * 1024, 0));
 #else
         (void)kt; (void)j; (void)pl;
         return bf16x8{};
@@ -156,7 +172,7 @@
             constexpr int i = decltype(ic)::value;
             constexpr int NR = 3;
             constexpr int W0 = i * PERW < NWF ? i * PERW : NWF, W1 = (i + 1) * PERW < NWF ? (i + 1) * PERW : NWF;
-            constexpr int VPS = J == 8 ? 2 : 4, NVS = 44 / VPS;
+            constexpr int VPS = NR + PERW + 22 + 4 <= NMMA ? 2 : 4, NVS = 44 / VPS;
             constexpr int S0 = NR + (W1 - W0), S1 = S0 + NVS, S2 = S1 + 3, S3 = S2 + 1;
             static_assert(S3 <= NMMA, "one MFMA per filler slot");
             unsigned su1[4], su2[4], su3[4];
@@ -290,7 +306,48 @@
     };
     constexpr int NQ = ROWS / 4, QH = NQ % 10 == 0 ? 10 : NQ % 8 == 0 ? 8 : NQ % 6 == 0 ? 6 : 4;
     static_assert(NQ % QH == 0, "row groups per pass");
-    if constexpr (GB) {
+    if constexpr (HD) {
+        constexpr int LP = dsc_la::LP;
+        float* const Qs = reinterpret_cast<float*>(wl);
+        float* const Ks = Qs + ROWS * LP;
+        float* const Vs = Ks + ROWS * LP;
+        float* const ctx = Vs + ROWS * LP;
+        const int h = ch;
+#pragma unroll
+        for (int i = 0; i < RB; ++i)
+#pragma unroll
+            for (int j = 0; j < J; ++j) *reinterpret_cast<f32x4*>(Qs + (j >> 1) * (ROWS * LP) + (i * 16 + l15) * LP + (j & 1) * 16 + 4 * g) = acc[i][j];
+        auto wave_sync = [&]() {
+            __builtin_amdgcn_fence(__ATOMIC_SEQ_CST, "wavefront");
+            __builtin_amdgcn_wave_barrier();
+        };
+        wave_sync();
+        if (ha.store_qkv) {
+            const int er8 = lane >> 3, ec8 = lane & 7;
+#pragma unroll
+            for (int sgm = 0; sgm < 3; ++sgm) {
+                const int vy = (er8 * (int)p.ldy + sgm * 128 + h * 32 + ec8 * 4) * 4;
+#pragma unroll
+                for (int q = 0; q < ROWS / 8; ++q) {
+                    const f32x4 v = *reinterpret_cast<const f32x4*>(Qs + sgm * (ROWS * LP) + (8 * q + er8) * LP + ec8 * 4);
+                    st4(v, ry, vy, 8 * q * (int)p.ldy * 4);
+                }
+            }
+        }
+        if (ha.out) {
+            const int nk = rows_here;
+            wave_sync();
+            dsc_la::phase1<4>(Ks, nk, lane);
+            wave_sync();
+            dsc_la::phase2<4>(Ks, Vs, ctx, nk, lane >> 1, (lane & 1) * 16);
+            wave_sync();
+            const int i0 = lane >> 2, part = lane & 3;
+#pragma unroll
+            for (int r = 0; r < RB; ++r) dsc_la::phase3_softmax(Qs, nk, ha.scale, i0 + 16 * r, part);
+            wave_sync();
+            dsc_la::phase3_out_jam<RB>(Qs, ctx, ha.out + ((int64_t)row0 + i0) * ha.ldo + h * 32 + part * 8, 16 * ha.ldo, nk, i0, part);
+        }
+    } else if constexpr (GB) {
         const float inv_cnt = 1.f / (float)(ntok * 64);
         const bool per_scene = p.ss_mode == DSC_SS_PER_SCENE && p.scale_shift;
 #if defined(__HIP_DEVICE_COMPILE__)
@@ -512,12 +569,23 @@
 
 template <bool GN, int RB, bool PERROW = false, int J = 8, bool GB = false>
 int launch(const dsc_gemm_args* a, const uint16_t* planes_f, int ntok, hipStream_t s) {
+    static_assert(J != 6, "the head tile has its own launcher");
     const int scenes = (a->m + ntok - 1) / ntok;
     const unsigned grid = (unsigned)(((scenes + WAVES - 1) / WAVES) * (a->n / (16 * J)));
     DSC_CLEAR_STALE_ERROR();
-    hipLaunchKernelGGL((gemm_split_wave_kernel<GN, RB, PERROW, J, GB>), dim3(grid, (unsigned)a->batch), dim3(64 * WAVES), 0, s, *a, planes_f, ntok DSC_WAVE_STAMP_PASS);
+    hipLaunchKernelGGL((gemm_split_wave_kernel<GN, RB, PERROW, J, GB>), dim3(grid, (unsigned)a->batch), dim3(64 * WAVES), 0, s, *a, planes_f, ntok, head_args{nullptr, 0, 0.f, 0} DSC_WAVE_STAMP_PASS);
     DSC_LAUNCH_CHECK();
     return 0;
 }
 
-}
+template <int RB>
+int launch_heads(const dsc_gemm_args* a, const uint16_t* planes_f, int ntok, const head_args& ha, hipStream_t s) {
+    const int scenes = (a->m + ntok - 1) / ntok;
+    const unsigned grid = (unsigned)(((scenes + WAVES - 1) / WAVES) * 4);
+    DSC_CLEAR_STALE_ERROR();
+    hipLaunchKernelGGL((gemm_split_wave_kernel<false, RB, false, 6, false, true>), dim3(grid, 1u), dim3(64 * WAVES), 0, s, *a, planes_f, ntok, ha DSC_WAVE_STAMP_PASS);
+    DSC_LAUNCH_CHECK();
+    return 0;
+}
+
+}
diff --git a/diffuscene_amd/csrc/linattn_core.h b/diffuscene_amd/csrc/linattn_core.h
--- /dev/null
+++ b/diffuscene_amd/csrc/linattn_core.h
@@ -0,0 +1,142 @@
+#pragma once
+#include "dsc_common.h"
+
+namespace dsc_la {
+
+constexpr int LP = 36;
+
+
+template <int V>
+__device__ __forceinline__ void phase1(float* Ks, const int nk, const int tid0) {
+    const int d0 = tid0 >> 3, part = tid0 & 7;
+    float mx[V], sm[V], inv[V];
+#pragma unroll
+    for (int v = 0; v < V; ++v) mx[v] = -INFINITY;
+    for (int j = part; j < nk; j += 8) {
+#pragma unroll
+        for (int v = 0; v < V; ++v) mx[v] = fmaxf(mx[v], Ks[j * LP + d0 + 8 * v]);
+    }
+#pragma unroll
+    for (int v = 0; v < V; ++v) {
+        mx[v] = fmaxf(mx[v], __shfl_xor(mx[v], 1, 64));
+        mx[v] = fmaxf(mx[v], __shfl_xor(mx[v], 2, 64));
+        mx[v] = fmaxf(mx[v], __shfl_xor(mx[v], 4, 64));
+        sm[v] = 0.f;
+    }
+    for (int j = part; j < nk; j += 8) {
+#pragma unroll
+        for (int v = 0; v < V; ++v) {
+            const float e = expf(Ks[j * LP + d0 + 8 * v] - mx[v]);
+            Ks[j * LP + d0 + 8 * v] = e;
+            sm[v] += e;
+        }
+    }
+#pragma unroll
+    for (int v = 0; v < V; ++v) {
+        sm[v] += __shfl_xor(sm[v], 1, 64);
+        sm[v] += __shfl_xor(sm[v], 2, 64);
+        sm[v] += __shfl_xor(sm[v], 4, 64);
+        inv[v] = 1.0f / sm[v];
+    }
+    for (int j = part; j < nk; j += 8) {
+#pragma unroll
+        for (int v = 0; v < V; ++v) Ks[j * LP + d0 + 8 * v] *= inv[v];
+    }
+}
+
+template <int V>
+__device__ __forceinline__ void phase2(const float* Ks, const float* Vs, float* ctx, const int nk, const int d, const int e0) {
+    f32x4 a[V];
+#pragma unroll
+    for (int v = 0; v < V; ++v) a[v] = f32x4{0.f, 0.f, 0.f, 0.f};
+    auto step = [&](const int j) {
+        const float kd = Ks[j * LP + d];
+#pragma unroll
+        for (int v = 0; v < V; ++v) {
+            const f32x4 vv = *reinterpret_cast<const f32x4*>(Vs + j * LP + e0 + 4 * v);
+#pragma unroll
+            for (int e = 0; e < 4; ++e) a[v][e] += kd * vv[e];
+        }
+    };
+    if constexpr (V == 1) {
+        for (int j = 0; j < nk; ++j) step(j);
+    } else {
+#pragma unroll 4
+        for (int j = 0; j < nk; ++j) step(j);
+    }
+#pragma unroll
+    for (int v = 0; v < V; ++v) *reinterpret_cast<f32x4*>(ctx + d * LP + e0 + 4 * v) = a[v];
+}
+
+__device__ __forceinline__ void phase3_softmax(float* Qs, const int nq, const float scale, const int i, const int part) {
+    const bool ok = i < nq;
+    float qv[8];
+    float mx = -INFINITY;
+    if (ok) {
+        const f32x4 a = *reinterpret_cast<const f32x4*>(Qs + i * LP + part * 8);
+        const f32x4 c = *reinterpret_cast<const f32x4*>(Qs + i * LP + part * 8 + 4);
+#pragma unroll
+        for (int e = 0; e < 4; ++e) { qv[e] = a[e]; qv[4 + e] = c[e]; }
+#pragma unroll
+        for (int e = 0; e < 8; ++e) mx = fmaxf(mx, qv[e]);
+    }
+    mx = fmaxf(mx, __shfl_xor(mx, 1, 64));
+    mx = fmaxf(mx, __shfl_xor(mx, 2, 64));
+    float sm = 0.f;
+    if (ok) {
+#pragma unroll
+        for (int e = 0; e < 8; ++e) { qv[e] = expf(qv[e] - mx); sm += qv[e]; }
+    }
+    sm += __shfl_xor(sm, 1, 64);
+    sm += __shfl_xor(sm, 2, 64);
+    if (ok) {
+        const float inv = scale / sm;
+        f32x4 a, c;
+#pragma unroll
+        for (int e = 0; e < 4; ++e) { a[e] = qv[e] * inv; c[e] = qv[4 + e] * inv; }
+        *reinterpret_cast<f32x4*>(Qs + i * LP + part * 8) = a;
+        *reinterpret_cast<f32x4*>(Qs + i * LP + part * 8 + 4) = c;
+    }
+}
+
+__device__ __forceinline__ void phase3_out(const float* Qs, const float* ctx, float* orow, const int nq, const int i, const int part) {
+    if (i < nq) {
+        f32x4 o0 = {0.f, 0.f, 0.f, 0.f}, o1 = {0.f, 0.f, 0.f, 0.f};
+#pragma unroll 8
+        for (int d = 0; d < 32; ++d) {
+            const float qd = Qs[i * LP + d];
+            const f32x4 c0 = *reinterpret_cast<const f32x4*>(ctx + d * LP + part * 8);
+            const f32x4 c1 = *reinterpret_cast<const f32x4*>(ctx + d * LP + part * 8 + 4);
+#pragma unroll
+            for (int e = 0; e < 4; ++e) { o0[e] += c0[e] * qd; o1[e] += c1[e] * qd; }
+        }
+        *reinterpret_cast<f32x4*>(orow) = o0;
+        *reinterpret_cast<f32x4*>(orow + 4) = o1;
+    }
+}
+
+template <int V>
+__device__ __forceinline__ void phase3_out_jam(const float* Qs, const float* ctx, float* orow0, const int64_t ldo16, const int nq, const int i0, const int part) {
+    f32x4 o0[V], o1[V];
+#pragma unroll
+    for (int v = 0; v < V; ++v) { o0[v] = f32x4{0.f, 0.f, 0.f, 0.f}; o1[v] = o0[v]; }
+#pragma unroll 8
+    for (int d = 0; d < 32; ++d) {
+        const f32x4 c0 = *reinterpret_cast<const f32x4*>(ctx + d * LP + part * 8);
+        const f32x4 c1 = *reinterpret_cast<const f32x4*>(ctx + d * LP + part * 8 + 4);
+#pragma unroll
+        for (int v = 0; v < V; ++v) {
+            const float qd = Qs[(i0 + 16 * v) * LP + d];
+#pragma unroll
+            for (int e = 0; e < 4; ++e) { o0[v][e] += c0[e] * qd; o1[v][e] += c1[e] * qd; }
+        }
+    }
+#pragma unroll
+    for (int v = 0; v < V; ++v)
+        if (i0 + 16 * v < nq) {
+            *reinterpret_cast<f32x4*>(orow0 + v * ldo16) = o0[v];
+            *reinterpret_cast<f32x4*>(orow0 + v * ldo16 + 4) = o1[v];
+        }
+}
+
+}
diff --git a/diffuscene_amd/engine.py b/diffuscene_amd/engine.py
--- a/diffuscene_amd/engine.py
+++ b/diffuscene_amd/engine.py
@@ -68,7 +68,8 @@
         self.tiled_steps = self.steps
 
     def gemm_args(self):
-        kinds = {id(_lib.fn("dsc_gemm_gn_silu_f32")): "gn", id(_lib.fn("dsc_gemm_f32")): "plain"}
+        kinds = {id(_lib.fn("dsc_gemm_gn_silu_f32")): "gn", id(_lib.fn("dsc_gemm_f32")): "plain",
+                 id(_lib.fn("dsc_qkv_linear_attention_f32")): "plain"}
         out = []
         for f, a in self.steps:
             k = kinds.get(id(f))
@@ -76,15 +77,22 @@
                 out.append((k, a[0]._obj))
         return out
 
-    def gemm(self, a, w, out, bias=None, a2=None, residual=None, act_in=ACT_NONE, act_out=ACT_NONE, row_invariant=False):
-        g = ops.make_gemm_args(a, w, out, bias, a2, residual, act_in, act_out, row_invariant=row_invariant)
+    def gemm(self, a, w, out, bias=None, a2=None, residual=None, act_in=ACT_NONE, act_out=ACT_NONE, row_invariant=False, attn_heads=0,
+             attn_core=None):
+        g = ops.make_gemm_args(a, w, out, bias, a2, residual, act_in, act_out, row_invariant=row_invariant, attn_heads=attn_heads)
         lay = ops.planes_layout(g)
         pl = self.eng.planes_of(w, lay) if lay >= 0 else None
         if pl is not None:
             ops.attach_planes(g, pl, layout=lay)
         self.keep.append(_own((g, a, w, out, bias, a2, residual, pl)))
+        if attn_core is not None and pl is not None and _lib.fn("dsc_gemm_split_tile")(C.byref(g), 0) == _lib.TILE_WAVE_HEADS:
+            o, scale = attn_core
+            self.keep.append(_own((o,)))
+            self.steps.append((_lib.fn("dsc_qkv_linear_attention_f32"),
+                               (C.byref(g), o.data_ptr(), o.stride(0), self.B, attn_heads, attn_heads, scale, 0, 0)))
+            return True
         self.steps.append((_lib.fn("dsc_gemm_f32"), (C.byref(g),)))
-        return out
+        return False if attn_core is not None else out
 
     def gemm_batched(self, a, w, out, bias, batch, sa, sw, sy, sbias, act_out=ACT_NONE):
         stacked = w._base if w._base is not None else w
@@ -190,11 +198,12 @@
         M, B, N = self.M, self.B, self.N
         att = blk.fn.fn
         y = self.layernorm(x, blk.fn.norm.g, self.pool.get(M, D))
-        qkv = self.gemm(y, att.to_qkv.weight, self.pool.get(M, 3 * HID))
+        qkv, a = self.pool.get(M, 3 * HID), self.pool.get(M, HID)
+        fused = self.gemm(y, att.to_qkv.weight, qkv, attn_heads=N, attn_core=(a, float(att.scale)))
         self.pool.put(y)
-        a = self.pool.get(M, HID)
-        self.call("dsc_linear_attention_f32", qkv.data_ptr(), 3 * HID, qkv.data_ptr() + 4 * HID, 3 * HID,
-                  qkv.data_ptr() + 8 * HID, 3 * HID, a.data_ptr(), HID, B, N, N, float(att.scale), keep=(qkv, a))
+        if not fused:
+            self.call("dsc_linear_attention_f32", qkv.data_ptr(), 3 * HID, qkv.data_ptr() + 4 * HID, 3 * HID,
+                      qkv.data_ptr() + 8 * HID, 3 * HID, a.data_ptr(), HID, B, N, N, float(att.scale), keep=(qkv, a))
         self.pool.put(qkv)
         out = self.out_proj_ln(a, att.to_out[0], att.to_out[1].g, x)
         self.pool.put(a)
@@ -223,7 +232,7 @@
         M, B, N = self.M, self.B, self.N
         att = blk.fn.fn
         y = self.layernorm(x, blk.fn.norm.g, self.pool.get(M, D))
-        qkv = self.gemm(y, att.to_qkv.weight, self.pool.get(M, 3 * HID))
+        qkv = self.gemm(y, att.to_qkv.weight, self.pool.get(M, 3 * HID), attn_heads=N)
         self.pool.put(y)
         a = self.pool.get(M, HID)
         self.call("dsc_attention_f32", qkv.data_ptr(), 3 * HID, qkv.data_ptr() + 4 * HID, 3 * HID,
diff --git a/diffuscene_amd/ops.py b/diffuscene_amd/ops.py
--- a/diffuscene_amd/ops.py
+++ b/diffuscene_amd/ops.py
@@ -34,7 +34,7 @@
 
 def make_gemm_args(a, w, y, bias=None, a2=None, residual=None, act_in=ACT_NONE, act_out=ACT_NONE,
                    gamma=None, beta=None, eps=1e-5, tokens_per_scene=0, scale_shift=None, ss_mode=SS_NONE, preact=None,
-                   ss_index=None, w_planes=None, actgrad_x=None, gnb=None, row_invariant=False):
+                   ss_index=None, w_planes=None, actgrad_x=None, gnb=None, row_invariant=False, attn_heads=0):
     g = GemmArgs()
     g.a1, g.lda1 = _mat(a, "a")
     g.k1 = a.shape[1]
@@ -58,6 +58,9 @@
     g.act_in, g.act_out, g.batch = act_in, act_out, 1
     if row_invariant:
         g.flags |= _lib.GEMM_ROW_INVARIANT
+    if attn_heads:
+        g.flags |= _lib.GEMM_ATTN_HEADS
+        g.tokens_per_scene = attn_heads
     if gamma is not None:
         g.gamma, g.beta, g.eps = _dev(gamma).data_ptr(), _dev(beta).data_ptr(), eps
         g.tokens_per_scene = tokens_per_scene
diff --git a/diffuscene_amd/train_plan.py b/diffuscene_amd/train_plan.py
--- a/diffuscene_amd/train_plan.py
+++ b/diffuscene_amd/train_plan.py
@@ -14,7 +14,7 @@
 
 
 class H:
-    __slots__ = ("t", "g", "ng", "act_of", "g_pre", "uses", "gn_of", "gn_part")
+    __slots__ = ("t", "g", "ng", "act_of", "g_pre", "uses", "gn_of", "gn_part", "attn_fused")
 
     def __init__(self, t, needs_grad=True):
         self.t, self.g, self.ng = t, None, needs_grad
@@ -23,6 +23,7 @@
         self.g_pre = None
         self.gn_of = None
         self.gn_part = None
+        self.attn_fused = False
 
 
 def tn_token_slices(groups, tile_n, blocks_target, tile_k=128):
@@ -159,7 +160,20 @@
         lay = ops.planes_layout(g)
         return lay >= 0 and self.planes_of(w, a.shape[0], lay) is not None
 
-    def gemm(self, a, w, out, bias=None, a2=None, residual=None, act_out=ACT_NONE, preact=None, actgrad_x=None):
+    def qkv_linattn(self, a, w, qkv, out, scenes, n, scale):
+        from . import ops
+        g = ops.make_gemm_args(a, w, qkv, attn_heads=n)
+        lay = ops.planes_layout(g)
+        pl = self.planes_of(w, a.shape[0], lay) if lay >= 0 else None
+        if pl is None:
+            return None
+        ops.attach_planes(g, pl, layout=lay)
+        if self.lib.fn("dsc_gemm_split_tile")(C.byref(g), 0) != self.lib.TILE_WAVE_HEADS:
+            return None
+        op, ldo = self._mat(out)
+        return self._call("dsc_qkv_linear_attention_f32", C.byref(g), op, ldo, scenes, n, n, scale, 1, 0, keep=(g, a, w, qkv, out, pl))
+
+    def gemm(self, a, w, out, bias=None, a2=None, residual=None, act_out=ACT_NONE, preact=None, actgrad_x=None, attn_heads=0):
         from . import ops
         m, K = a.shape
         if preact is not None or actgrad_x is not None:
@@ -181,7 +195,7 @@
                 self.keep.append(_own((g, a, w, out, bias, residual)))
                 self.f32_reads.add(w.untyped_storage().data_ptr())
                 return self._with_scratch(floats, lambda wp, wn: (fn, (C.byref(g), splits, wp, wn), "dsc_gemm_splitk_f32"))
-        g = ops.make_gemm_args(a, w, out, bias, a2, residual, ACT_NONE, act_out)
+        g = ops.make_gemm_args(a, w, out, bias, a2, residual, ACT_NONE, act_out, attn_heads=attn_heads)
         lay = ops.planes_layout(g)
         pl = self.planes_of(w, m, lay) if lay >= 0 else None
         if pl is not None:
@@ -754,7 +768,7 @@
         self._transposes.append((w2d, buf[:, :n]))
         return buf
 
-    def linear(self, a, weight, bias, a2=None, residual=None, out=None, act_out=ACT_NONE, wt=None, act=None):
+    def linear(self, a, weight, bias, a2=None, residual=None, out=None, act_out=ACT_NONE, wt=None, act=None, attn_heads=0, attn_core=None):
         w2 = _as2d(weight)
         n, K = w2.shape
         rows = a.t.shape[0]
@@ -766,6 +780,11 @@
         if fused:
             ya_t = self.new(rows, n)
             self.emit(self.be.gemm(a.t, w2, ya_t, bias, a2.t if a2 is not None else None, None, act, preact=y.t))
+        elif attn_heads and hasattr(self.be, "qkv_linattn"):
+            assert bias is None and a2 is None and residual is None and act_out == ACT_NONE
+            step = self.be.qkv_linattn(a.t, w2, y.t, attn_core[0], rows // attn_heads, attn_heads, attn_core[1]) if attn_core is not None else None
+            y.attn_fused = step is not None
+            self.emit(step if step is not None else self.be.gemm(a.t, w2, y.t, attn_heads=attn_heads))
         else:
             self.emit(self.be.gemm(a.t, w2, y.t, bias, a2.t if a2 is not None else None,
                                    residual.t if residual is not None else None, act_out))
@@ -927,10 +946,11 @@
         att = blk.fn.fn
         B, N = self.B, self.N
         y = self.layernorm(a, blk.fn.norm.g)
-        qkv = self.linear(y, att.to_qkv.weight, None)
         o = H(self.new(self.M, HID))
+        qkv = self.linear(y, att.to_qkv.weight, None, attn_heads=N, attn_core=(o.t, float(att.scale)))
         q, k, v = qkv.t[:, :HID], qkv.t[:, HID:2 * HID], qkv.t[:, 2 * HID:]
-        self.emit(self.be.linattn(q, k, v, o.t, B, N, N, float(att.scale)))
+        if not qkv.attn_fused:
+            self.emit(self.be.linattn(q, k, v, o.t, B, N, N, float(att.scale)))
 
         def bw():
             if o.g is None:
@@ -967,7 +987,7 @@
         att = blk.fn.fn
         B, N = self.B, self.N
         y = self.layernorm(a, blk.fn.norm.g)
-        qkv = self.linear(y, att.to_qkv.weight, None)
+        qkv = self.linear(y, att.to_qkv.weight, None, attn_heads=N)
         o = H(self.new(self.M, HID))
         q, k, v = qkv.t[:, :HID], qkv.t[:, HID:2 * HID], qkv.t[:, 2 * HID:]
         self.emit(self.be.attn(q, k, v, o.t, B, N, float(att.scale)))
diff --git a/include/diffuscene_hip.h b/include/diffuscene_hip.h
--- a/include/diffuscene_hip.h
+++ b/include/diffuscene_hip.h
@@ -55,6 +55,7 @@
     int32_t flags;
 } dsc_gemm_args;
 #define DSC_GEMM_ROW_INVARIANT 1
+#define DSC_GEMM_ATTN_HEADS 2
 #define DSC_PLANES_ROWMAJOR 0
 #define DSC_PLANES_FRAGMENT 1
 #define DSC_PLANES_NONE (-100)
@@ -76,6 +77,7 @@
 #define DSC_TILE_WAVE_GN     10
 #define DSC_TILE_WAVE_DENSE  11
 #define DSC_TILE_WAVE_GN_64  12
+#define DSC_TILE_WAVE_HEADS  13
 int dsc_gemm_split_tile(const dsc_gemm_args* args, int32_t gn);
 
 #define DSC_F32_TILE_160x256 0
@@ -89,6 +91,12 @@
 
 int dsc_get_split_wave(void);
 int dsc_set_split_wave(int32_t mode);
+int dsc_get_attn_heads(void);
+int dsc_set_attn_heads(int32_t mode);
+
+#define DSC_NOT_TAKEN (-101)
+int dsc_qkv_linear_attention_f32(const dsc_gemm_args* args, float* out, int64_t ldo, int32_t scenes, int32_t nq, int32_t nk, float scale,
+                                 int32_t store_qkv, int32_t mode, dsc_stream_t stream);
 
 int dsc_gemm_skinny(const dsc_gemm_args* args, int32_t gn);
 int dsc_get_skinny(void);
```
